# YoungSeng/QPGesture

Hardware: AMD Instinct MI355X
Metric: matched gesture frames/sec (GestureKNN) (higher is better)
Workload: dtype split-f16 products / f64 block sums + f64 re-evaluation; 1 GPU; 1 x 24 s clip (M=6 windows, Q=48 steps, 1440 frames each) per job vs speaker-10-class DB N_db=2048 windows (53248 candidates), shipped mode wavlm_feat(f32-bounded/f64-exact)+text(f32)+phase; n_db=2048, windows_per_clip=6, clips=1, clips_per_gpu=1, feature_dtype=f32, audio_precision=mixed, encode_batch=0, clips_in_flight=1, parallelism=single GPU, unsharded DB

## Files before the change

include/qpg.h:

```cpp
#ifndef QPG_H
#define QPG_H

#include <stddef.h>
#include <stdint.h>

#ifdef __cplusplus
extern "C" {
#endif

#define QPG_OK 0
#define QPG_EINVAL (-1)
#define QPG_EHIP (-2)
#define QPG_EUNSUP (-3)

typedef struct qpg_ctx qpg_ctx;

int qpg_version(void);
const char* qpg_build_id(void);
int qpg_ctx_create(int device, qpg_ctx** out);
int qpg_dev_kernarg(void);
int qpg_ctx_destroy(qpg_ctx* ctx);
#define QPG_OPT_GATE_DEDUP_FROM_CHAINS 0
#define QPG_OPT_TAKES_STAGES 1
#define QPG_OPT_COUNT 4
int qpg_ctx_set_option(qpg_ctx* ctx, int option, int value);
int qpg_ctx_get_option(qpg_ctx* ctx, int option, int* value);
int qpg_last_error(char* buf, size_t n);
int qpg_signal_i32(qpg_ctx*, void* stream, int32_t* dst, int32_t value);
int qpg_doorbell_wait(qpg_ctx*, void* stream, int32_t* counter, const int32_t* go, int32_t timeout_ms);


int qpg_wavlm_resample_f32(qpg_ctx*, void* stream, const float* x, int64_t N, int Tin, int F, int Tout, float* out);

int qpg_frame_norm2_f64(qpg_ctx*, void* stream, const float* x, int64_t rows, int F, double* out);

int qpg_audio_cand_norm2(qpg_ctx*, void* stream, const double* fn2, int N, int T, const int32_t* cand_t,
                         int G, int n_taps, int tap_stride, double* cn2);

int qpg_l2_normalize_rows_f32(qpg_ctx*, void* stream, const float* x, int64_t rows, int D, float* out);
int qpg_text_pack_queries_f32(qpg_ctx*, void* stream, const float* x, int M, int R, int D, const int32_t* q_win,
                              const int32_t* q_row, int Q, float* out);


int qpg_audio_pack_queries(qpg_ctx*, void* stream, const float* qbase, int M, int T, int F,
                           const int32_t* q_win, const int32_t* q_t, int Q, int n_taps, int tap_stride,
                           float* q32, double* qn2);

int qpg_audio_cosine_f64(qpg_ctx*, void* stream, const float* base, int N, int T, int F,
                         const int32_t* cand_t, int G, int n_taps, int tap_stride, const double* cn2,
                         const float* q32, const double* qn2, int Q, double* D, int64_t ldD);
int qpg_audio_cosine_f64_h(qpg_ctx*, void* stream, const void* base_f16, int N, int T, int F,
                           const int32_t* cand_t, int G, int n_taps, int tap_stride, const double* cn2,
                           const float* q32, const double* qn2, int Q, double* D, int64_t ldD);

#define QPG_AUDIO_MX_ERR 2.05e-6
int qpg_audio_cosine_mx(qpg_ctx*, void* stream, const float* base, int N, int T, int F, const int32_t* cand_t, int G,
                        int n_taps, int tap_stride, const double* cn2, const float* q32, const double* qn2, int Q,
                        void* D, int d_is_f32, int64_t ldD, int32_t* stats);

int qpg_audio_cosine_mx_h(qpg_ctx*, void* stream, const void* base_f16, int N, int T, int F, const int32_t* cand_t, int G,
                          int n_taps, int tap_stride, const double* cn2, const float* q32, const double* qn2, int Q,
                          void* D, int d_is_f32, int64_t ldD, int32_t* stats);

#define QPG_AUDIO_HL_ERR 1.3e-6
int qpg_audio_hl_supported(int T, int F, int G, int n_taps, int tap_stride, int cand_step);
int qpg_audio_pack_queries_hl(qpg_ctx*, void* stream, const float* qbase, int M, int T, int F, const int32_t* q_win,
                              const int32_t* q_t, int Q, int n_taps, int tap_stride, float* q32, double* qn2, void* image,
                              int64_t image_bytes);
int64_t qpg_audio_hl_db_bytes(int N, int F);
int64_t qpg_audio_hl_query_bytes(int Q, int F);
int qpg_audio_hl_pack_db(qpg_ctx*, void* stream, const float* base, int N, int T, int F, int G, int n_taps, int tap_stride,
                         int cand_step, void* image, int64_t image_bytes);
int qpg_audio_hl_pack_queries(qpg_ctx*, void* stream, const float* q32, int Q, int F, void* image, int64_t image_bytes);
int qpg_clip_pack_hl(qpg_ctx*, void* stream, const float* qbase, int M, int T, int F, const int32_t* q_win,
                     const int32_t* q_t, int Q, int n_taps, int tap_stride, float* q32, double* qn2, void* image,
                     int64_t image_bytes, const float* text_ctx, int Mt, int R, int Dt, const int32_t* tq_win,
                     const int32_t* tq_row, int Qt, float* qn_out, void* cols_image, int64_t cols_bytes);
int qpg_audio_cosine_hl(qpg_ctx*, void* stream, const void* db_image, int N, int F, int G, const double* cn2,
                        const void* q_image, const double* qn2, int Q, void* D, int d_is_f32, int64_t ldD, int32_t* stats);
int qpg_audio_hl1_supported(int T, int F, int G, int n_taps, int tap_stride, int cand_step);
int64_t qpg_audio_hl1_db_bytes(int N, int F);
int qpg_audio_hl1_pack_db(qpg_ctx*, void* stream, const void* base_f16, int N, int T, int F, int G, int n_taps,
                          int tap_stride, int cand_step, void* image, int64_t image_bytes);
int qpg_audio_cosine_hl1(qpg_ctx*, void* stream, const void* db_image, int N, int F, int G, const double* cn2,
                         const void* q_image, const double* qn2, int Q, void* D, int d_is_f32, int64_t ldD, int32_t* stats);
int qpg_probe_mfma_f16_tile(qpg_ctx*, void* stream, const void* a, const void* b, const float* c, int tiles, float* out);

int qpg_text_pack_candidates_f32(qpg_ctx*, void* stream, const float* x, int N, int R, int Dm,
                                 const int32_t* cand_r, int G, float* xt);

int qpg_text_cosine_f32(qpg_ctx*, void* stream, const float* xt, int64_t C, int Dm, const float* qn, int Q,
                        float* D, int64_t ldD);

int64_t qpg_text_percode_ws_bytes(int64_t C, int Q, int K, int tiles_per_chunk);
int qpg_text_percode_f32(qpg_ctx*, void* stream, const float* xt, int64_t C, int Dm, const int16_t* cand_code, int K,
                         const float* qn, int Q, int tiles_per_chunk, int32_t idx_base, float absent, void* ws,
                         int64_t ws_bytes, float* out_dist, int32_t* out_idx, int16_t* out_rank, int32_t* out_nn);
int qpg_text_pack_candidates_f16(qpg_ctx*, void* stream, const float* x, int N, int R, int Dm, const int32_t* cand_r,
                                 int G, void* xh, float* nrm);
int qpg_text_percode_f16(qpg_ctx*, void* stream, const void* xh, const float* nrm, int64_t C, int Dm,
                         const int16_t* cand_code, int K, const float* qn, int Q, int32_t idx_base, float absent,
                         void* ws, int64_t ws_bytes, float* out_dist, int32_t* out_idx, int16_t* out_rank,
                         int32_t* out_nn);

int64_t qpg_hl_rows_bytes(int64_t R, int D);
int64_t qpg_hl_cols_bytes(int Q, int D);
int qpg_hl_pack_rows(qpg_ctx*, void* stream, const float* xs, int64_t R, int D, void* image, int64_t image_bytes);
int qpg_hl_pack_cols(qpg_ctx*, void* stream, const float* qn, int Q, int D, void* image, int64_t image_bytes);
int qpg_hl_prepare_queries(qpg_ctx*, void* stream, const float* q, int Q, int D, float* qn_out, void* cols_image,
                           int64_t image_bytes, float* qperm_out);
int qpg_hl_gemm_distance(qpg_ctx*, void* stream, const void* rows_image, int64_t R, int D, const void* cols_image, int Q,
                         float* Dm, int64_t ldD, float* tile_min, int64_t ldT);
int qpg_hl_gemm_tilemin(qpg_ctx*, void* stream, const void* rows_image, int64_t R, int D, const void* cols_image, int Q,
                        float band, float* tile_min, uint16_t* tile_mask, int64_t ldT);
int qpg_hl_gemm_tilemin_h(qpg_ctx*, void* stream, const void* rows_image, int64_t R, int D, const void* cols_image, int Q,
                          float band, float* tile_min_t, uint16_t* tile_mask_t, int64_t ldQ);
int qpg_perm32_rows_f32(qpg_ctx*, void* stream, const float* x, int64_t R, int D, float* y);
int qpg_percode_select_bycode_f32(qpg_ctx*, void* stream, const float* tile_min_t, const uint16_t* tile_mask_t, int64_t ldQ,
                                  int Q, int64_t R, const int16_t* row_code, const int32_t* row_index,
                                  const int32_t* zero_row, const int32_t* code_tile, int K, float band,
                                  const float* qn_perm, const float* xs_perm, int D, float absent, float* out_dist,
                                  int32_t* out_idx, int16_t* out_rank, int32_t* out_nn, int32_t* stats, int32_t idx_base);
int qpg_percode_select_sorted_f32(qpg_ctx*, void* stream, const float* Dm, int64_t ldD, const float* tile_min,
                                  const uint16_t* tile_mask , int64_t ldT,
                                  int Q, int64_t R, const int16_t* row_code, const int32_t* row_index,
                                  const int32_t* zero_row, const int32_t* code_tile, int K, float band, const float* qn,
                                  const float* xs, int D, float absent, float* out_dist, int32_t* out_idx,
                                  int16_t* out_rank, int32_t* out_nn, int32_t* stats, int32_t idx_base, int q_block,
                                  int64_t block_stride);

int qpg_wavvq_lev_f32(qpg_ctx*, void* stream, const int32_t* sym_db, int N, int T, const int32_t* cand_t, int G,
                      const int32_t* tap_off, int n_taps, const int32_t* sym_q, int Mq, int Tq,
                      const int32_t* q_win, const int32_t* q_t, int Q, float* D, int64_t ldD);

int qpg_percode_select_f64(qpg_ctx*, void* stream, const double* D, int64_t ldD, int Q, const int16_t* cand_code,
                           int64_t C, int K, double absent, int32_t idx_base, double* out_dist, int32_t* out_idx,
                           int16_t* out_rank, int q_block, int64_t block_stride);
int qpg_percode_select_f32(qpg_ctx*, void* stream, const float* D, int64_t ldD, int Q, const int16_t* cand_code,
                           int64_t C, int K, float absent, int32_t idx_base, float* out_dist, int32_t* out_idx,
                           int16_t* out_rank, int q_block, int64_t block_stride);

int qpg_percode_select_guarded_f64(qpg_ctx*, void* stream, const double* D, int64_t ldD, int Q, const int16_t* cand_code,
                                   int64_t C, int K, double absent, int32_t idx_base, double* out_dist, int32_t* out_idx,
                                   int16_t* out_rank, int q_block, int64_t block_stride, const float* base, int T, int F,
                                   const int32_t* cand_t, int G, int n_taps, int tap_stride, const float* q32, double eps,
                                   int32_t* stats, int base_is_f16);

int64_t qpg_percode_select_exact_ws_bytes(int Q, int64_t C, int K);
int qpg_percode_select_exact_f64(qpg_ctx*, void* stream, const double* D, int64_t ldD, int Q, const int16_t* cand_code,
                                 int64_t C, int K, double absent, int32_t idx_base, double* out_dist, int32_t* out_idx,
                                 int16_t* out_rank, int q_block, int64_t block_stride, const float* base, int T, int F,
                                 const int32_t* cand_t, int G, int n_taps, int tap_stride, const float* q32, double eps,
                                 int32_t* stats, int base_is_f16, void* ws, int64_t ws_bytes);

int qpg_percode_select_mixed_f64(qpg_ctx*, void* stream, const void* D, int d_is_f32, int64_t ldD, int Q, const int16_t* cand_code,
                                 int64_t C, int K, double absent, int32_t idx_base, double* out_dist, int32_t* out_idx,
                                 int16_t* out_rank, int q_block, int64_t block_stride, const float* base, int T, int F,
                                 const int32_t* cand_t, int G, int n_taps, int tap_stride, const float* q32,
                                 const double* qn2, const double* cn2, double eps1, double eps2, int32_t* stats,
                                 void* ws, int64_t ws_bytes, int base_is_f16);
int64_t qpg_percode_select_mixed_ws_bytes(int Q, int K);
int64_t qpg_percode_select_mixed_ws_stride(int K);
int qpg_percode_select_mixed_f64_cut(qpg_ctx*, void* stream, const void* D, int d_is_f32, int64_t ldD, int Q,
                                     const int16_t* cand_code, int64_t C, int K, double absent, int32_t idx_base,
                                     double* out_dist, int32_t* out_idx, int16_t* out_rank, int q_block, int64_t block_stride,
                                     const float* base, int T, int F, const int32_t* cand_t, int G, int n_taps,
                                     int tap_stride, const float* q32, const double* qn2, const double* cn2, double eps1,
                                     double eps2, int32_t* stats, void* ws, int64_t ws_bytes, int base_is_f16,
                                     const int16_t* pos_rank_t, const int16_t* freq_rank, int top_n, int probe);

int64_t qpg_merge_mixed_ws_bytes(int Q, int K, int fl_cap);
int qpg_merge_mixed_phase1_f64(qpg_ctx*, void* stream, const void* recv, int W, int64_t src_stride, int64_t dist_off,
                               int64_t idx_off, int Q, int K, double absent, double eps1, int R, void* req,
                               int64_t req_stride, void* ws, int64_t ws_bytes, int32_t* stats, int fl_cap,
                               int64_t flag_off);
int qpg_shard_refine_f64(qpg_ctx*, void* stream, const void* req_recv, int W, int64_t req_stride, int R, int q_stride,
                         int64_t cand_base, const float* base, int base_is_f16, int T, int F, const int32_t* cand_t, int G,
                         int n_taps, int tap_stride, const float* q32, const double* qn2, const double* cn2, void* resp,
                         int64_t resp_stride, int reference_arithmetic, int32_t* stats, int Rq);
int qpg_flags_stamp(qpg_ctx*, void* stream, void* buf, int nblk, int64_t stride, int64_t off, const int32_t* stats);
int qpg_flags_gather(qpg_ctx*, void* stream, const void* buf, int nblk, int64_t stride, int64_t off, int32_t* stats);
int qpg_merge_mixed_phase2_f64(qpg_ctx*, void* stream, const void* recv, int W, int64_t src_stride, int64_t idx_off, int Q,
                               int K, double absent, const void* ws, int64_t ws_bytes, const void* resp_recv,
                               int64_t resp_stride, double* out_dist, int32_t* out_idx, int16_t* out_rank, int32_t* stats,
                               int fl_cap, double eps2);

int qpg_merge_select_f64(qpg_ctx*, void* stream, const void* recv, int W, int64_t src_stride, int64_t dist_off,
                         int64_t idx_off, int Q, int K, double absent, double* out_dist, int32_t* out_idx,
                         int16_t* out_rank, double eps2, int32_t* stats);
int qpg_merge_select_f32(qpg_ctx*, void* stream, const void* recv, int W, int64_t src_stride, int64_t dist_off,
                         int64_t idx_off, int Q, int K, float absent, float* out_dist, int32_t* out_idx,
                         int16_t* out_rank);

int qpg_rank_rows_f64(qpg_ctx*, void* stream, const double* d, int Q, int K, int16_t* out);
int qpg_rank_rows_f32(qpg_ctx*, void* stream, const float* d, int Q, int K, int16_t* out);


int qpg_l2_table_f32(qpg_ctx*, void* stream, const float* sig, int K, int Dm, float* out);

#define QPG_MODE_AUD_TXT 0
#define QPG_MODE_AUD 1
#define QPG_MODE_TXT 2
#define QPG_MODE_SERIAL_WALK 0x100
#define QPG_MODE_PREFUSED 0x200

int qpg_match_steps(qpg_ctx*, void* stream, const int16_t* aud_rank, const int32_t* aud_idx,
                    const int16_t* txt_rank, const int32_t* txt_idx, const int16_t* pos_rank,
                    const int16_t* freq_rank, const int32_t* code, int code_ld, const int32_t* aud_cidx,
                    const int32_t* aud_pslot, int Ga, const int32_t* txt_cidx, const int32_t* txt_pslot, int Gt,
                    const float* phase, int Tp, int mode, int M, int steps, int K, int seed_code,
                    const float* seed_phase, int32_t* gate_tables, int32_t* out_codes, float* out_phase,
                    int32_t* out_vote, int32_t* out_status, const int32_t* guard_flags);
int qpg_match_steps_batch(qpg_ctx*, void* stream, const int16_t* aud_rank, const int32_t* aud_idx, const int16_t* txt_rank,
                          const int32_t* txt_idx, const int16_t* pos_rank, const int16_t* freq_rank, const int32_t* code,
                          int code_ld, const int32_t* aud_cidx, const int32_t* aud_pslot, int Ga, const int32_t* txt_cidx,
                          const int32_t* txt_pslot, int Gt, const float* phase, int Tp, int mode, int M, int steps, int K,
                          int n_chains, const int32_t* seed_codes, const float* seed_phase, int32_t* gate_tables,
                          int32_t* out_codes, float* out_phase, int32_t* out_vote, int32_t* out_status,
                          int64_t status_stride, const int32_t* guard_flags);
#define QPG_TAKES_MAX 65536
size_t qpg_match_steps_takes_ws_bytes(int n_takes, int M, int steps);
int qpg_match_steps_takes(qpg_ctx*, void* stream, const int16_t* aud_rank, const int32_t* aud_idx, const int16_t* txt_rank,
// ... 187 lines not shown
```

qpgesture_amd/code_knn.py:

```python
import ctypes
from collections import namedtuple
from typing import NamedTuple, Optional

import numpy as np
import torch

from . import _lib
from .parallel import allreduce_max_, allreduce_min_index, exchange_bytes, shard_rows
from .sorted_rows import SortedRows

from .constant import (ABSENT_DIST, NUM_AUDIO_FEAT_FRAMES, STEP_SZ, WAVVQ_GROUP_SIZE, codebook_size, num_frames,
                       num_frames_code)

MODE_AUD_TXT, MODE_AUD, MODE_TXT = _lib.QPG_MODE_AUD_TXT, _lib.QPG_MODE_AUD, _lib.QPG_MODE_TXT
AUDIO_MX_ERR = _lib.QPG_AUDIO_MX_ERR
AUDIO_MX_BAND = 2.1 * AUDIO_MX_ERR
AUDIO_HL_ERR = _lib.QPG_AUDIO_HL_ERR
AUDIO_HL_BAND = 2.1 * AUDIO_HL_ERR

FLAG_LIST_OVERFLOW, FLAG_SMALL_NORMS, FLAG_REQUEST_OVERFLOW, FLAG_CROSS_SHARD_TIE = 1, 2, 4, 8
FLAG_TEXT_OVERFLOW = 16


_PIN_SENTINEL = -1234567
# ... 207 lines not shown
            pd = torch.empty((self.K, self.K), dtype=torch.float32, device=dev)
            _lib.call("qpg_l2_table_f32", dev, sig, self.K, sig.shape[1], pd)
            self.pos_dist = pd
            self.pos_rank = torch.empty((self.K, self.K), dtype=torch.int16, device=dev)
            _lib.call("qpg_rank_rows_f32", dev, pd, self.K, self.K, self.pos_rank)
        else:
            self.pos_rank = torch.as_tensor(np.asarray(pos_rank, np.int16), device=dev).contiguous()

        cnt = np.bincount(code.reshape(-1), minlength=self.K)[:self.K]
        self.freq_dist = np.where(cnt > 0, 1 - cnt / cnt.sum(), 1.0)
        self.pos_rank_t = self.pos_rank.t().contiguous()
        if freq_rank is None:
            fd = torch.from_numpy(self.freq_dist[None].copy()).to(dev)
            self.freq_rank = torch.empty((1, self.K), dtype=torch.int16, device=dev)
            _lib.call("qpg_rank_rows_f64", dev, fd, 1, self.K, self.freq_rank)
            self.freq_rank = self.freq_rank[0].contiguous()
        else:
            self.freq_rank = torch.as_tensor(np.asarray(freq_rank, np.int16), device=dev).contiguous()

    def save(self, path, key="", sources=None):
        from . import db_cache
        return db_cache.save(self, path, key, sources=sources)

    @classmethod
    def load(cls, path, device="cuda:0", key=None):
        from . import db_cache
        dev = torch.device(device)
        if dev.type != "cuda":
            raise RuntimeError("GestureDB needs a HIP device (got %s); there is no CPU path" % dev)
        _lib.load()
        db = db_cache.load(path, dev, key)
        if db is None:
            return None
        if db.hl_image is not None or db.txt_sorted is not None:
            from .selfcheck import mfma_bound_ok
            db.hl_bound_ok, db.hl_bound_report = mfma_bound_ok(dev)
            if not db.hl_bound_ok:
                db.hl_image = db.txt_sorted = None
        return db

    @staticmethod
    def _cand_code(code_local, cidx, dev):
        cc = np.ascontiguousarray(code_local[:, np.asarray(cidx, np.int64)].reshape(-1))
        cc = np.where((cc >= 0) & (cc < 32767), cc, -1).astype(np.int16)
        return torch.from_numpy(cc if cc.size else np.zeros((1,), np.int16)).to(dev)

    @property
    def idx_base(self):
        return self.lo


Knobs = namedtuple("Knobs", "audio_precision audio_kernel text_kernel tie_eps mixed_single_launch sharded_mixed "
                   "sharded_mixed_min_gflop force_sharded overlap_sweeps text_after_sweep audio_first fused_pack rank_cut "
                   "split_fuse split_fuse_max_steps host_ranks use_wavvq",
                   defaults=("mixed", "hl", "mfma", 1e-12, False, True, 20.0, False, True, True, None, True, True, True,
                             256, False, False))
DBFacts = namedtuple("DBFacts", "n_local N world K Ga F Dt feature_dtype hl_bound_ok has_hl_image has_txt_sorted hl_planes",
                     defaults=("f32", True, True, True, 2))


class AudioPlan(NamedTuple):
    path: str
    kernel: str
    band: float
    cut_top_n: int
    fused_rank: bool


class StepPlan(NamedTuple):
    audio: Optional[AudioPlan]
    text: Optional[str]
    sharded: bool
    exchange: Optional[str]
    clip_pack: bool
    split_fuse: bool
    overlap: bool
    order: Optional[str]


def plan_audio(kn, db, Q, want_rank=False, reduce=True, out_given=False, cut_top_n=0):
    C = db.n_local * db.Ga
    fused_rank = want_rank and db.world == 1
    local_final = fused_rank and reduce and not out_given
    shard_part = (db.world > 1 or kn.force_sharded) and not reduce and out_given
    gflop = 2e-9 * Q * (-(-db.N // db.world) * db.Ga) * NUM_AUDIO_FEAT_FRAMES * db.F
    guard = kn.tie_eps > 0 and C > 0
    half = db.feature_dtype == "f16"
    if (kn.audio_precision == "mixed" and guard and db.K <= 512 and db.hl_bound_ok and
            (local_final or (shard_part and kn.sharded_mixed and gflop >= kn.sharded_mixed_min_gflop))):
        hl = kn.audio_kernel == "hl" and db.has_hl_image
        kernel = ("hl" if db.hl_planes == 2 else "hl1") if hl else ("mx_h" if half else "mx")
        cut = cut_top_n if (cut_top_n in (1, 2) and local_final and not kn.mixed_single_launch) else 0
        return AudioPlan("mixed", kernel, AUDIO_HL_BAND if hl else AUDIO_MX_BAND, cut, fused_rank)
    path = "exact" if (kn.audio_precision == "exact" and guard) else ("guarded" if guard else "plain")
    return AudioPlan(path, "f64_h" if half else "f64", 0.0, 0, fused_rank)


def plan_text(kn, db, Q, reduce=True, out_given=False):
    mfma = (kn.text_kernel == "mfma" and db.has_txt_sorted and Q > 0 and kn.audio_precision != "exact" and
            ((not out_given and reduce and db.world == 1) or (out_given and not reduce)))
    return "mfma" if mfma else "valu"


def plan_step(kn, db, M, steps, mode=MODE_AUD_TXT, for_walk=False, owner_blocks=False):
    Q = M * steps
    sharded = db.world > 1 or kn.force_sharded
    audio = text = None
    if mode != MODE_TXT and not kn.use_wavvq:
        cut = 0
        if for_walk and kn.rank_cut and not sharded and not kn.host_ranks:
            cut = 1 if mode == MODE_AUD_TXT else 2
        audio = plan_audio(kn, db, Q, want_rank=not sharded, reduce=not sharded, out_given=sharded, cut_top_n=cut)
    if mode != MODE_AUD:
        text = plan_text(kn, db, Q, reduce=not sharded, out_given=sharded)
    split = (for_walk and mode == MODE_AUD_TXT and not sharded and not kn.host_ranks and kn.split_fuse and
             db.K % 16 == 0 and db.K <= 4096 and Q <= kn.split_fuse_max_steps)
    overlap = mode == MODE_AUD_TXT and kn.overlap_sweeps
    mfma_text = kn.text_kernel == "mfma" and db.has_txt_sorted and kn.audio_precision != "exact"
    clip_pack = (overlap and not kn.use_wavvq and mfma_text and audio.kernel in ("hl", "hl1") and db.Dt % 128 == 0 and
                 kn.fused_pack)
    audio_first = mfma_text if kn.audio_first is None else bool(kn.audio_first)
    after = overlap and kn.text_after_sweep and not audio_first and not kn.use_wavvq
    order = None
    if overlap:
        order = "audio_first" if audio_first else ("text_after_sweep" if after else "text_first")
    exchange = ("all_to_all" if owner_blocks else "all_gather") if sharded else None
    return StepPlan(audio, text, sharded, exchange, clip_pack, split, overlap, order)


class TakesPlan(NamedTuple):
    path: str
    reason: str


def plan_takes(kn, db, M, steps, n_takes, serial_walk=False):
    if db.world > 1 or kn.force_sharded:
        return TakesPlan("unsupported", "takes of a row-sharded database are not implemented (the merged tables would serve; "
                                        "nothing tests them)")
    if serial_walk:
        return TakesPlan("per_take", "the one-wave sequential walk was asked for (serial_walk)")
    K = db.K
    last_idx = min(steps * 4, num_frames_code) - 1
    if (last_idx // 4 != steps - 1 or M * steps > 2048 or 2 * steps * 2 * K * 2 > 64 * 1024 or (steps * 2 * K) % 8 or
            2 * K > 65536):
        return TakesPlan("per_take", "the tabulated walk does not take this geometry (steps = %d, K = %d, %d steps per clip)"
                         % (steps, K, M * steps))
    if not 1 <= n_takes <= _lib.QPG_TAKES_MAX:
        return TakesPlan("per_take", "n_takes outside [1, %d]" % _lib.QPG_TAKES_MAX)
    return TakesPlan("kernel", "")


AudioResult = namedtuple("AudioResult", "dist idx rank D q32 qn2 plan")


def _grown(buf, nbytes, dev, zero=False):
    if buf is not None and buf.numel() >= nbytes:
        return buf
    return (torch.zeros if zero else torch.empty)((nbytes,), dtype=torch.uint8, device=dev)


class CodeKNN:

    def __init__(self, db, use_wavlm=True, use_wavvq=False, use_phase=True, use_txt=True, rng=None):
        if use_wavlm == use_wavvq:
            raise ValueError("exactly one of use_wavlm / use_wavvq (GestureKNN.py:431-438)")
        if use_wavvq and not db.has_wavvq:
            raise ValueError("GestureDB was built without a wavvq track")
        self.db = db
        self.use_wavvq = use_wavvq
        if use_wavvq:
            self.step_sz, self.n_db_frm = db.vq_step, db.Tv
        else:
            self.step_sz, self.n_db_frm = db.step_sz, db.T
        self.n_db_seq = db.N
        self.use_phase, self.use_txt = use_phase, use_txt
        self.rng = rng if rng is not None else np.random
        self.overlap_sweeps = True
        self.text_after_sweep = True
        self.audio_first = None
        self.serial_walk = False
        self.tie_eps = 1e-12
        self._guard_stats = torch.zeros((4,), dtype=torch.int32, device=db.device)
        self.audio_precision = "mixed"
        self.audio_kernel = "hl"
        self.text_kernel = "mfma"
        self._txt_scratch = {}
        self.fallbacks = 0
        import os as _os
        self.fused_pack = _os.environ.get("QPG_FUSED_PACK", "1") != "0"
        self.rank_cut = _os.environ.get("QPG_RANK_CUT", "1") != "0"
        self.rank_cut_probe = 64
        self.mixed_single_launch = False
        self.split_fuse = True
        self.split_fuse_max_steps = 256
        self.sharded_mixed = True
        self.force_sharded = False
        self.sharded_mixed_min_gflop = 20.0
        self.mixed_requests = None
        self.host_ranks = False

        self._qpos, self._qcache, self._layouts, self._mm_cache, self._pinned_ints, self._plans = None, {}, {}, {}, {}, {}
        self._side_stream = self._side_gate = self._side_done = self._sweep_event = None
        self._mix_ws = self._exact_ws = self._hl_qimage = self._takes_ws = None
        self.kernel_events, self.kernel_events_every, self.kernel_event_pool, self._ev_calls = None, 1, None, 0
        self.text_fallbacks, self.tables, self._last_mix_Q = 0, None, 0
        self._last_audio_mixed = self._last_audio_exact = self._last_audio_hl = False
        self._last_text_mfma = self._last_rank_cut = False
        self._last_D_aud = self._last_q32 = self._last_qn2 = self._last_ints = self._last_gate_tables = None

    def _knobs(self):
        return Knobs(self.audio_precision, self.audio_kernel, self.text_kernel, self.tie_eps, self.mixed_single_launch,
                     self.sharded_mixed, self.sharded_mixed_min_gflop, self.force_sharded, self.overlap_sweeps,
                     self.text_after_sweep, self.audio_first, self.fused_pack, self.rank_cut, self.split_fuse,
                     self.split_fuse_max_steps, self.host_ranks, self.use_wavvq)

    def _facts(self):
        db = self.db
        return DBFacts(db.n_local, db.N, db.world, db.K, db.Ga, db.F, db.Dt, db.feature_dtype, db.hl_bound_ok,
                       db.hl_image is not None, db.txt_sorted is not None, db.hl_planes)

    def _audio_grid(self):
        db = self.db
        if self.use_wavvq:
            return db.vq_cidx, db.vq_pslot, db.Gv
        return db.aud_cidx, db.aud_pslot, db.Ga

    def query_positions(self):
        key = (self.n_db_frm, self.step_sz)
        if self._qpos is not None and self._qpos[0] == key:
            return self._qpos[1]
        pos, i = [], 0
        while i < self.n_db_frm:
            pos.append(i)
            i += STEP_SZ * self.step_sz
        self._qpos = (key, pos)
        return pos

    def init_code_phase(self):
        db = self.db
        i = self.rng.randint(0, self.n_db_seq)
        j = self.rng.randint(0, self.n_db_frm - int(num_frames / num_frames_code))
        code = int(db.code_host[i, j // num_frames_code])
        P = db.phase_host[i, j:j + 8]
        if P.shape[0] != 8:
            raise ValueError("init_code_phase drew frame %d: phase slice has %d rows, not 8 "
                             "(the reference fails on this draw too); use another seed" % (j, P.shape[0]))
        return code, np.concatenate((P[:, 0], P[:, 1]), axis=1).astype(np.float32)

    def _tables_out(self, Q, dtype, out, with_rank):
        K, dev = self.db.K, self.db.device
        dist, idx, qb, bs = out if out is not None else (torch.empty((Q, K), dtype=dtype, device=dev),
                                                         torch.empty((Q, K), dtype=torch.int32, device=dev), 0, 0)
        return dist, idx, (torch.empty((Q, K), dtype=torch.int16, device=dev) if with_rank else None), qb, bs

    def _select_plain(self, D, cand_code, C, G, out, with_rank):
        db, Q = self.db, D.shape[0]
        dist, idx, rank, qb, bs = self._tables_out(Q, D.dtype, out, with_rank)
        _lib.call("qpg_percode_select_f64" if D.dtype == torch.float64 else "qpg_percode_select_f32", db.device, D,
                  D.stride(0), Q, cand_code, C, db.K, float(ABSENT_DIST), db.idx_base * G, dist, idx, rank, qb, bs)
        return dist, idx, rank

    def _finish(self, dist, idx, rank, want_rank, reduce):
        if not reduce:
            return dist, idx
        dist, idx = self._reduce_min(dist, idx)
        if want_rank:
            return dist, idx, (rank if rank is not None else self.rank_rows(dist))
        return dist, idx

    def _sweep_timer(self):
        if self.kernel_events is None:
            return None
        if self.kernel_events_every > 1:
            self._ev_calls += 1
            if self._ev_calls % self.kernel_events_every:
                return None
        return (self.kernel_event_pool.pop() if self.kernel_event_pool else
                (torch.cuda.Event(enable_timing=True), torch.cuda.Event(enable_timing=True)))

    def sweep_audio(self, qbase, q_win, q_t, tap_stride=None, want_rank=False, reduce=True, out=None, prepacked=None,
                    cut_top_n=None):
        Q = int(q_win.shape[0]) if isinstance(q_win, torch.Tensor) else len(q_win)
        plan = plan_audio(self._knobs(), self._facts(), Q, want_rank, reduce, out is not None, cut_top_n or 0)
        r = self._sweep_audio(plan, qbase, q_win, q_t, tap_stride, out, prepacked)
        return self._finish(r.dist, r.idx, r.rank, want_rank, reduce)

    def _sweep_audio(self, plan, qbase, q_win, q_t, tap_stride=None, out=None, prepacked=None, sweep_event=None,
                     after_sweep=None):
        db, dev = self.db, self.db.device
        Q = int(q_win.shape[0]) if isinstance(q_win, torch.Tensor) else len(q_win)
        qbase = qbase.contiguous()
        M, T, F = qbase.shape
        ts = db.tap_stride if tap_stride is None else tap_stride
        if prepacked is not None:
            q32, qn2 = prepacked[0], prepacked[1]
        else:
            q32 = torch.empty((Q, NUM_AUDIO_FEAT_FRAMES * F), dtype=torch.float32, device=dev)
            qn2 = torch.empty((Q,), dtype=torch.float64, device=dev)
        C = db.n_local * db.Ga
        mixed, use_hl, half = plan.path == "mixed", plan.kernel in ("hl", "hl1"), db.feature_dtype == "f16"
        D = torch.empty((Q, max(C, 1)), dtype=torch.float32 if mixed else torch.float64, device=dev)
        timer = self._sweep_timer()
        sweep_fn = "qpg_audio_cosine_" + plan.kernel
        if use_hl:
            qi = self._hl_qimage = _grown(self._hl_qimage, int(_lib.load().qpg_audio_hl_query_bytes(Q, db.F)), dev)
            sweep_launch = _lib.prepare(sweep_fn, dev, db.hl_image, db.n_local, db.F, db.Ga, db.cn2, qi,
                                        qn2, Q, D, 1, D.stride(0), self._guard_stats)
            if prepacked is None:
                _lib.call("qpg_audio_pack_queries_hl", dev, qbase, M, T, F, _i32(q_win, dev), _i32(q_t, dev), Q,
                          NUM_AUDIO_FEAT_FRAMES, ts, q32, qn2, qi, qi.numel())
        else:
            assert prepacked is None, "the one-launch clip pack feeds the split-f16 sweep only"
            _lib.call("qpg_audio_pack_queries", dev, qbase, M, T, F, _i32(q_win, dev), _i32(q_t, dev), Q,
                      NUM_AUDIO_FEAT_FRAMES, ts, q32, qn2)
        if timer is not None:
            timer[0].record(torch.cuda.current_stream(dev))
        if use_hl:
            sweep_launch()
        else:
            strides = (1, D.stride(0), self._guard_stats) if mixed else (D.stride(0),)
            _lib.call(sweep_fn, dev, db.base, db.n_local, db.T, db.F, db.aud_t, db.Ga, NUM_AUDIO_FEAT_FRAMES,
                      db.tap_stride, db.cn2, q32, qn2, Q, D, *strides)
        if timer is not None:
            timer[1].record(torch.cuda.current_stream(dev))
            self.kernel_events.append(timer)
        if after_sweep is not None:
            after_sweep()
        if sweep_event is not None:
            sweep_event.record(torch.cuda.current_stream(dev))
        if plan.path == "plain":
            dist, idx, rank = self._select_plain(D, db.aud_cand_code, C, db.Ga, out, plan.fused_rank)
        else:
            dist, idx, rank, qb, bs = self._tables_out(Q, torch.float64, out, plan.fused_rank)
            tables = (Q, db.aud_cand_code, C, db.K, float(ABSENT_DIST), db.idx_base * db.Ga, dist, idx, rank, qb, bs)
            track = (db.base, db.T, db.F, db.aud_t, db.Ga, NUM_AUDIO_FEAT_FRAMES, db.tap_stride, q32)
        if mixed:
            ws = self._mix_ws = _grown(self._mix_ws, int(_lib.load().qpg_percode_select_mixed_ws_bytes(Q, db.K)), dev,
                                       zero=True)
            single = self.mixed_single_launch
            sel_args = (D, 1, D.stride(0), *tables, *track, qn2, db.cn2, plan.band, float(self.tie_eps),
                        self._guard_stats, None if single else ws, 0 if single else ws.numel(), int(half))
            try:
                if plan.cut_top_n:
                    _lib.call("qpg_percode_select_mixed_f64_cut", dev, *sel_args, db.pos_rank_t, db.freq_rank,
                              int(plan.cut_top_n), int(self.rank_cut_probe))
                else:
                    _lib.call("qpg_percode_select_mixed_f64", dev, *sel_args)
            except Exception:
                self._mix_ws = None
                raise
        elif plan.path == "exact":
            ws = self._exact_ws = _grown(self._exact_ws, int(_lib.load().qpg_percode_select_exact_ws_bytes(Q, C, db.K)),
                                         dev)
            _lib.call("qpg_percode_select_exact_f64", dev, D, D.stride(0), *tables, *track, float(self.tie_eps),
                      self._guard_stats, int(half), ws, ws.numel())
        elif plan.path == "guarded":
            _lib.call("qpg_percode_select_guarded_f64", dev, D, D.stride(0), *tables, *track, float(self.tie_eps),
                      self._guard_stats, int(half))
        self._last_audio_mixed, self._last_audio_exact, self._last_audio_hl = mixed, plan.path == "exact", use_hl
        self._last_rank_cut, self._last_D_aud, self._last_q32, self._last_qn2 = plan.cut_top_n > 0, D, q32, qn2
        if mixed:
            self._last_mix_Q = Q
        return AudioResult(dist, idx, rank, D, q32, qn2, plan)

    def sweep_text(self, queries, want_rank=False, reduce=True, normalised=False, out=None, cols_packed=False, kind=None):
        db, dev = self.db, self.db.device
        Q = queries.shape[0]
        if normalised:
            qn = queries
        else:
            qn = torch.empty_like(queries)
            _lib.call("qpg_l2_normalize_rows_f32", dev, queries, Q, db.Dt, qn)
        if kind is None:
            kind = plan_text(self._knobs(), self._facts(), Q, reduce, out is not None)
        self._last_text_mfma = kind == "mfma"
        if kind == "mfma":
            dist, idx, rank, qb, bs = self._tables_out(Q, torch.float32, out, want_rank and out is None)
            db.txt_sorted.select(qn, float(ABSENT_DIST), self._guard_stats, dist=dist, idx=idx, rank=rank,
                                 idx_base=db.idx_base * db.Gt, q_block=qb, block_stride=bs, scratch=self._txt_scratch,
                                 cols_packed=cols_packed)
        else:
            D = torch.empty((Q, max(db.Ct, 1)), dtype=torch.float32, device=dev)
            _lib.call("qpg_text_cosine_f32", dev, db.ctxt, db.Ct, db.Dt, qn, Q, D, D.stride(0))
            dist, idx, rank = self._select_plain(D, db.txt_cand_code, db.Ct, db.Gt, out, want_rank and db.world == 1)
        return self._finish(dist, idx, rank, want_rank, reduce)

    def sweep_audio_wavvq(self, test_wavvq, q_win, q_t, want_rank=False, reduce=True, out=None):
        db, dev = self.db, self.db.device
        tw = torch.as_tensor(test_wavvq).to(dev)
        sym_q = (tw[..., 0].to(torch.int64) * WAVVQ_GROUP_SIZE + tw[..., 1].to(torch.int64)).to(torch.int32).contiguous()
        Q = int(q_win.shape[0]) if isinstance(q_win, torch.Tensor) else len(q_win)
        C = db.n_local * db.Gv
        D = torch.empty((Q, max(C, 1)), dtype=torch.float32, device=dev)
        taps = (ctypes.c_int32 * len(db.vq_taps))(*db.vq_taps)
        _lib.call("qpg_wavvq_lev_f32", dev, db.vq_sym, db.n_local, db.Tv, db.vq_t, db.Gv, taps, len(db.vq_taps),
                  sym_q, sym_q.shape[0], sym_q.shape[1], _i32(q_win, dev), _i32(q_t, dev), Q, D, D.stride(0))
        dist, idx, rank = self._select_plain(D, db.vq_cand_code, C, db.Gv, out, want_rank and db.world == 1)
        self._last_D_aud = D
        return self._finish(dist, idx, rank, want_rank, reduce)

    def _reduce_min(self, dist, idx):
        if self.db.world == 1:
            return dist, idx
        return allreduce_min_index(dist, idx)

    def guard_stats(self):
        v = self._guard_stats.cpu().numpy()
        return int(v[0]), bool(v[1])

    def mixed_stats(self):
        v = self._guard_stats.cpu().numpy()
        return {"tier1_pairs": int(v[2]), "tier2_pairs": int(v[0]), "flags": int(v[1])}

    def tier1_list_lengths(self):
        ws, Q = self._mix_ws, self._last_mix_Q
        if ws is None or not Q:
            return np.zeros((0,), np.int64)
        K = self.db.K
        stride = int(_lib.load().qpg_percode_select_mixed_ws_stride(K))
        w = ws[:Q * stride].view(Q, stride)[:, 24 * K:24 * K + 4].contiguous().view(torch.int32)
        return w.cpu().numpy().reshape(-1).astype(np.int64)

    def clear_flags(self):
        self._guard_stats[1:2].zero_()

    @staticmethod
    def numpy_ranks(dist, idx=None, integer=False):
        d = dist.detach().cpu().numpy()
        present = None if idx is None else (idx.detach().cpu().numpy() >= 0)
        out = np.empty(d.shape, np.int16)
        for r_, row in enumerate(d):
            full = present is not None and bool(present[r_].all())
            if full and integer:
# ... 67 lines not shown
        dev = self.db.device
        if self._side_stream is None:
            self._side_stream = torch.cuda.Stream(dev)
            self._side_gate, self._side_done = torch.cuda.Event(), torch.cuda.Event()
            self._sweep_event = torch.cuda.Event()
        if dev.index is None or dev.index == torch.cuda.current_device():
            self._side_gate.record()
        else:
            self._side_gate.record(torch.cuda.current_stream(dev))
        self._side_stream.wait_event(self._side_gate)
        return self._side_stream

    def _clip_pack(self, test_interp, test_context, q_win, q_t, q_row, Q):
        db, dev = self.db, self.db.device
        q32 = torch.empty((Q, NUM_AUDIO_FEAT_FRAMES * db.F), dtype=torch.float32, device=dev)
        qn2 = torch.empty((Q,), dtype=torch.float64, device=dev)
        qi = self._hl_qimage = _grown(self._hl_qimage, int(_lib.load().qpg_audio_hl_query_bytes(Q, db.F)), dev)
        qn = torch.empty((Q, db.Dt), dtype=torch.float32, device=dev)
        cols = db.txt_sorted.cols_buffer(Q, self._txt_scratch)
        tc, ti = test_context.contiguous(), test_interp.contiguous()
        _lib.call("qpg_clip_pack_hl", dev, ti, ti.shape[0], db.T, db.F, q_win, q_t, Q, NUM_AUDIO_FEAT_FRAMES,
                  db.tap_stride, q32, qn2, qi, qi.numel(), tc, tc.shape[0], tc.shape[1], db.Dt, q_win, q_row, Q, qn, cols,
                  cols.numel())
        return q32, qn2, qn

    def sweep_tables(self, test_interp, test_context, n_windows, mode=MODE_AUD_TXT, owner_blocks=False, for_walk=False,
                     after_sweep=None):
        db, dev = self.db, self.db.device
        M, steps = n_windows, self.n_steps()
        if test_interp.shape[0] < M or (mode != MODE_AUD and test_context.shape[0] < M):
            raise IndexError("n_windows=%d but the test arrays hold %d audio / %d context windows"
                             % (M, test_interp.shape[0], test_context.shape[0]))
        want = (db.Tv, 2) if self.use_wavvq else (db.T, db.F)
        if tuple(test_interp.shape[1:]) != want:
            raise ValueError("test audio windows have shape %s, database expects %s"
                             % (tuple(test_interp.shape[1:]), want))
        q_win, q_t, q_row = self._query_index(M)
        Q = M * steps
        key = (self._knobs(), self._facts(), M, steps, mode, for_walk, owner_blocks)
        plan = self._plans.get(key)
        if plan is None:
            plan = self._plans[key] = plan_step(*key)
        sharded = plan.sharded
        T = dict(aud_d=None, aud_idx=None, aud_rank=None, txt_d=None, txt_idx=None, txt_rank=None)
        gtab = torch.empty((3, max(M, 1) * steps, db.K), dtype=torch.int32, device=dev) if plan.split_fuse else None
        lay = self._layout(Q, owner_blocks, mode) if sharded else None
        side = self._fork_side() if plan.overlap else None
        packed = None
        if plan.clip_pack:
            packed = self._clip_pack(test_interp, test_context, q_win, q_t, q_row, Q)
            self._side_gate.record(torch.cuda.current_stream(dev))
            side.wait_event(self._side_gate)

        def keep(p_, g, r):
            T[p_ + "_d"], T[p_ + "_idx"], T[p_ + "_rank"] = r[0], r[1], (None if sharded else r[2])
            if gtab is not None:
                _lib.call("qpg_fuse_best_ranked", dev, r[2], r[1], db.pos_rank, db.freq_rank, Q, db.K, gtab[g])

        def text_pack():
            tc = test_context.contiguous()
            qn = torch.empty((Q, db.Dt), dtype=torch.float32, device=dev)
            _lib.call("qpg_text_pack_queries_f32", dev, tc, tc.shape[0], tc.shape[1], db.Dt, q_win, q_row, Q, qn)
            return qn

        def text_side(qn=None):
            if packed is not None:
                qn = packed[2]
            elif qn is None:
                qn = text_pack()
            keep("txt", 1, self.sweep_text(qn, want_rank=not sharded, reduce=not sharded, normalised=True,
                                           out=lay.views("txt") if sharded else None, cols_packed=packed is not None,
                                           kind=plan.text))

        if plan.order == "text_first":
            with torch.cuda.stream(side):
                text_side()
        aud = None
        if mode != MODE_TXT:
            out = lay.views("aud") if sharded else None
            if self.use_wavvq:
                r = self.sweep_audio_wavvq(test_interp, q_win, q_t, want_rank=not sharded, reduce=not sharded, out=out)
            else:
                aud = self._sweep_audio(plan.audio, test_interp, q_win, q_t, out=out, prepacked=packed,
                                        sweep_event=self._sweep_event if plan.order == "text_after_sweep" else None,
                                        after_sweep=after_sweep)
                r = self._finish(aud.dist, aud.idx, aud.rank, not sharded, not sharded)
            keep("aud", 0, r)
        if plan.order == "text_after_sweep":
            with torch.cuda.stream(side):
                qn_early = None if packed is not None else text_pack()
                side.wait_event(self._sweep_event)
                text_side(qn_early)
        elif plan.order == "audio_first":
            with torch.cuda.stream(side):
                text_side()
        if plan.overlap:
            self._side_done.record(side)
            torch.cuda.current_stream(dev).wait_event(self._side_done)
        elif mode != MODE_AUD:
            text_side()
        if sharded:
            self._merge_shards(lay, owner_blocks, T, aud)
        if self.host_ranks:
            for p_ in ("aud", "txt"):
                if T[p_ + "_d"] is not None:
                    T[p_ + "_rank"] = self.numpy_ranks(T[p_ + "_d"], T[p_ + "_idx"],
                                                       integer=(p_ == "aud" and self.use_wavvq))
        if gtab is not None:
            T["gate_tables"] = gtab
        return T

    def _layout(self, Q, owner_blocks, mode):
        parts = tuple(p_ for p_, off in (("aud", MODE_TXT), ("txt", MODE_AUD)) if mode != off)
        key = (Q, self.db.world if owner_blocks else 1, parts, not self.use_wavvq)
        if key not in self._layouts:
            self._layouts[key] = ExchangeLayout(key[0], self.db.K, key[1], parts, key[3], self.db.device)
        return self._layouts[key]

    def _merge_shards(self, lay, owner_blocks, T, aud):
        db, dev = self.db, self.db.device
        _lib.call("qpg_flags_stamp", dev, lay.send, lay.nblk, lay.block_bytes, lay.off["flags"], self._guard_stats)
        recv = exchange_bytes(lay.send, db.world, owner_blocks)
        src_stride = lay.block_bytes if owner_blocks else lay.send.numel()
        gathered = False
        for p_ in lay.parts:
            d = torch.empty((lay.Qb, db.K), dtype=lay.dtype[p_], device=dev)
            ix = torch.empty((lay.Qb, db.K), dtype=torch.int32, device=dev)
            rk = torch.empty((lay.Qb, db.K), dtype=torch.int16, device=dev)
            wavlm_aud = p_ == "aud" and aud is not None
            if wavlm_aud and aud.plan.path in ("mixed", "exact"):
                self._merge_mixed(recv, src_stride, lay, owner_blocks, d, ix, rk, aud.q32, aud.qn2, aud.plan)
                gathered = True
            elif lay.dtype[p_] == torch.float64:
                guard = wavlm_aud and self.tie_eps > 0
                _lib.call("qpg_merge_select_f64", dev, recv, db.world, src_stride, lay.off[p_ + "_d"],
                          lay.off[p_ + "_i"], lay.Qb, db.K, float(ABSENT_DIST), d, ix, rk,
                          float(self.tie_eps) if guard else 0.0, self._guard_stats if guard else None)
            else:
# ... 237 lines not shown
```

qpgesture_amd/csrc/qpg_common.h:

```cpp
#pragma once
#include <hip/hip_runtime.h>
#include <stdint.h>
#include <stdio.h>
#include <string.h>

#include "../../include/qpg.h"

struct qpg_ctx {
  int device;
  int n_cu;
  float* zeros;
  bool select_lds_raised;
  int opt[QPG_OPT_COUNT];
};

#ifdef QPG_DEBUG_HOOKS
#define QPG_HOOK_VAR(type, name, value) static type name = value
#else
#define QPG_HOOK_VAR(type, name, value) static constexpr type name = value
#endif

void qpg_set_error(const char* fmt, ...);

#define QPG_REQUIRE(cond, ...)      \
  do {                              \
    if (!(cond)) {                  \
      qpg_set_error(__VA_ARGS__);   \
      return QPG_EINVAL;            \
    }                               \
  } while (0)

#define QPG_LAUNCH_CHECK(name)                                                \
  do {                                                                        \
    hipError_t e_ = hipGetLastError();                                        \
    if (e_ != hipSuccess) {                                                   \
      qpg_set_error("%s: launch failed: %s", name, hipGetErrorString(e_));    \
      return QPG_EHIP;                                                        \
    }                                                                         \
  } while (0)

static inline hipStream_t qpg_stream(void* s) { return reinterpret_cast<hipStream_t>(s); }

typedef double f64x4 __attribute__((ext_vector_type(4)));
typedef float f32x4 __attribute__((ext_vector_type(4)));
typedef float f32x16 __attribute__((ext_vector_type(16)));

#pragma clang fp contract(off)
__device__ __forceinline__ float f_mul(float a, float b) { return a * b; }
__device__ __forceinline__ float f_add(float a, float b) { return a + b; }
__device__ __forceinline__ float f_sub(float a, float b) { return a - b; }
__device__ __forceinline__ float f_div(float a, float b) { return a / b; }
__device__ __forceinline__ float f_sqrt(float a) { return __builtin_sqrtf(a); }
__device__ __forceinline__ double f_mul(double a, double b) { return a * b; }
__device__ __forceinline__ double f_add(double a, double b) { return a + b; }
__device__ __forceinline__ double f_sub(double a, double b) { return a - b; }
__device__ __forceinline__ double f_div(double a, double b) { return a / b; }

__device__ __forceinline__ double cosine_from_dot(double dot, double qn2, double cn2) {
  const double tiny = 10.0 * 2.220446049250313e-16;
  double nq = sqrt(qn2), nc = sqrt(cn2);
  bool zq = nq < tiny, zc = nc < tiny;
  if (zq || zc) {
    double a = zq ? qn2 : 1.0, b = zc ? cn2 : 1.0;
    double cross = dot / ((zq ? 1.0 : nq) * (zc ? 1.0 : nc));
    return 0.5 * (a + b - 2.0 * cross);
// ... 146 lines not shown
```

qpgesture_amd/csrc/qpg_core.hip:

```cpp
#include <stdarg.h>

#include "qpg_common.h"
#include <stdlib.h>

static thread_local char g_err[512] = "";

void qpg_set_error(const char* fmt, ...) {
  va_list ap;
  va_start(ap, fmt);
  vsnprintf(g_err, sizeof(g_err), fmt, ap);
  va_end(ap);
}

extern "C" int qpg_version(void) { return 109; }

#ifndef QPG_BUILD_ID
#define QPG_BUILD_ID "unstamped"
#endif
static const char g_build_id[] = "QPG_BUILD_ID=" QPG_BUILD_ID;
extern "C" const char* qpg_build_id(void) { return g_build_id + 13; }

extern "C" int qpg_dev_kernarg(void) {
  const char* e = getenv("HIP_FORCE_DEV_KERNARG");
  return (e && e[0] == '1') ? 1 : 0;
}

extern "C" int qpg_last_error(char* buf, size_t n) {
  if (!buf || n == 0) return QPG_EINVAL;
  strncpy(buf, g_err, n - 1);
  buf[n - 1] = 0;
  return QPG_OK;
}

extern "C" int qpg_ctx_create(int device, qpg_ctx** out) {
  QPG_REQUIRE(out != nullptr, "qpg_ctx_create: out is null");
  int n = 0;
  if (hipGetDeviceCount(&n) != hipSuccess || device < 0 || device >= n) {
    qpg_set_error("qpg_ctx_create: no HIP device %d (count %d)", device, n);
    return QPG_EHIP;
  }
  hipDeviceProp_t p;
  if (hipGetDeviceProperties(&p, device) != hipSuccess) {
    qpg_set_error("qpg_ctx_create: hipGetDeviceProperties failed");
    return QPG_EHIP;
  }
  qpg_ctx* c = new qpg_ctx;
  c->device = device;
  c->n_cu = p.multiProcessorCount;
  c->zeros = nullptr;
  c->select_lds_raised = false;
  for (int i = 0; i < QPG_OPT_COUNT; ++i) c->opt[i] = 0;
  c->opt[QPG_OPT_GATE_DEDUP_FROM_CHAINS] = 1;
  c->opt[QPG_OPT_TAKES_STAGES] = 7;
  int prev = 0;
  (void)hipGetDevice(&prev);
  const bool ok = hipSetDevice(device) == hipSuccess && hipMalloc(reinterpret_cast<void**>(&c->zeros), 4096) == hipSuccess &&
                  hipMemset(c->zeros, 0, 4096) == hipSuccess;
  (void)hipSetDevice(prev);
  if (!ok) {
    qpg_set_error("qpg_ctx_create: could not allocate the context's zero page on device %d", device);
    delete c;
    return QPG_EHIP;
  }
  *out = c;
  return QPG_OK;
}

extern "C" int qpg_ctx_set_option(qpg_ctx* ctx, int option, int value) {
  QPG_REQUIRE(ctx != nullptr, "qpg_ctx_set_option: null context");
  QPG_REQUIRE(option >= 0 && option < QPG_OPT_COUNT, "qpg_ctx_set_option: unknown option %d", option);
  if (option == QPG_OPT_GATE_DEDUP_FROM_CHAINS) QPG_REQUIRE(value >= 0, "qpg_ctx_set_option: gate_dedup_from_chains >= 0");
  ctx->opt[option] = value;
  return QPG_OK;
}

extern "C" int qpg_ctx_get_option(qpg_ctx* ctx, int option, int* value) {
  QPG_REQUIRE(ctx != nullptr && value != nullptr, "qpg_ctx_get_option: null pointer");
  QPG_REQUIRE(option >= 0 && option < QPG_OPT_COUNT, "qpg_ctx_get_option: unknown option %d", option);
  *value = ctx->opt[option];
  return QPG_OK;
}

extern "C" int qpg_ctx_destroy(qpg_ctx* ctx) {
  if (ctx && ctx->zeros) (void)hipFree(ctx->zeros);
  delete ctx;
  return QPG_OK;
}

__global__ void signal_i32_kernel(int32_t* dst, int32_t value) {
  __hip_atomic_store(dst, value, __ATOMIC_RELEASE, __HIP_MEMORY_SCOPE_SYSTEM);
}

extern "C" int qpg_signal_i32(qpg_ctx* ctx, void* stream, int32_t* dst, int32_t value) {
  QPG_REQUIRE(ctx && dst && (reinterpret_cast<uintptr_t>(dst) % 4) == 0, "qpg_signal_i32: null or misaligned destination");
  hipLaunchKernelGGL(signal_i32_kernel, dim3(1), dim3(1), 0, qpg_stream(stream), dst, value);
  QPG_LAUNCH_CHECK("signal_i32_kernel");
  return QPG_OK;
}

__global__ void doorbell_wait_kernel(int32_t* __restrict__ counter, const int32_t* __restrict__ go, int32_t timeout_ms) {
  const int32_t seq = atomicAdd(counter, 1) + 1;
  const long long t0 = wall_clock64();
  const long long limit = (long long)timeout_ms * 100000ll;
  while (__hip_atomic_load(go, __ATOMIC_RELAXED, __HIP_MEMORY_SCOPE_SYSTEM) - seq < 0) {
    if (wall_clock64() - t0 > limit) break;
    __builtin_amdgcn_s_sleep(16);
// ... 167 lines not shown
```

qpgesture_amd/csrc/qpg_select.hip:

```cpp
#include "qpg_common.h"

__device__ __forceinline__ unsigned long long order_key(double d) {
  unsigned long long b = (unsigned long long)__double_as_longlong(d);
  return (b >> 63) ? ~b : (b | 0x8000000000000000ull);
}
__device__ __forceinline__ double key_value(unsigned long long k, double) {
  unsigned long long b = (k >> 63) ? (k & 0x7fffffffffffffffull) : ~k;
  return __longlong_as_double((long long)b);
}
__device__ __forceinline__ unsigned int order_key(float d) {
  unsigned int b = __float_as_uint(d);
  return (b >> 31) ? ~b : (b | 0x80000000u);
}
__device__ __forceinline__ float key_value(unsigned int k, float) {
  unsigned int b = (k >> 31) ? (k & 0x7fffffffu) : ~k;
  return __uint_as_float(b);
}

template <typename T, typename KeyT, bool PACKED>
__global__ __launch_bounds__(1024) void percode_select_kernel(const T* __restrict__ D, int64_t ldD,
                                                              const int16_t* __restrict__ cand_code, int64_t C, int K,
                                                              T absent, int32_t idx_base, T* __restrict__ out_dist,
                                                              int32_t* __restrict__ out_idx,
                                                              int16_t* __restrict__ out_rank, int q_block,
                                                              int64_t block_stride) {
  extern __shared__ __attribute__((aligned(16))) unsigned char smem[];
  unsigned long long* best = reinterpret_cast<unsigned long long*>(smem);
  unsigned int* besti = reinterpret_cast<unsigned int*>(smem + 8 * (size_t)K);
  T* v = reinterpret_cast<T*>(smem + 12 * (size_t)rank_sort_pow2(K));
  constexpr int VEC = 16 / sizeof(T);
  typedef T vecT __attribute__((ext_vector_type(VEC)));
  typedef int16_t vecC __attribute__((ext_vector_type(VEC)));
  const int q = blockIdx.x;
  if (q_block > 0) {
    const int64_t shift = (int64_t)(q / q_block) * block_stride;
    const int64_t rowoff = (int64_t)(q % q_block) * K - (int64_t)q * K;
    out_dist = reinterpret_cast<T*>(reinterpret_cast<unsigned char*>(out_dist) + shift) + rowoff;
    out_idx = reinterpret_cast<int32_t*>(reinterpret_cast<unsigned char*>(out_idx) + shift) + rowoff;
  }
  const T* row = D + (int64_t)q * ldD;
  for (int k = threadIdx.x; k < K; k += blockDim.x) {
    best[k] = ~0ull;
    besti[k] = 0xffffffffu;
  }
  __syncthreads();
  const bool vec_ok = (ldD % VEC) == 0 && (reinterpret_cast<uintptr_t>(D) % 16) == 0 &&
                      (reinterpret_cast<uintptr_t>(cand_code) % (2 * VEC)) == 0;
  const int64_t Cv = vec_ok ? (C / VEC) * VEC : 0;
  for (int64_t c = (int64_t)threadIdx.x * VEC; c < Cv; c += (int64_t)blockDim.x * VEC) {
    const vecT d = *reinterpret_cast<const vecT*>(row + c);
    const vecC cd = *reinterpret_cast<const vecC*>(cand_code + c);
#pragma unroll
    for (int e = 0; e < VEC; ++e) {
// ... 50 lines not shown
                     [&](int k, int r) { out_rank[(int64_t)q * K + k] = (int16_t)r; });
}

template <typename T, typename F>
__device__ __forceinline__ void block_stable_ranks(const T* v, int K, int* cnt, F&& emit) {
  const int tid = threadIdx.x;
  if (K <= 512 && K >= 64 && (int)blockDim.x >= 256) {
    __shared__ unsigned long long rank_skey[512];
    __shared__ int rank_scode[512];
    block_sorted_ranks(v, K, rank_skey, rank_scode, emit);
    return;
  }
  const int P = (int)blockDim.x >= 2 * K ? (int)blockDim.x / K : 1;
  if (P == 1) {
    for (int k = tid; k < K; k += blockDim.x) {
      const T x = v[k];
      int r = 0;
#pragma unroll 8
      for (int o = 0; o < K; ++o) {
        const T y = v[o];
        r += (y < x) || (y == x && o < k);
      }
      emit(k, r);
    }
    return;
  }
  for (int k = tid; k < K; k += blockDim.x) cnt[k] = 0;
  __syncthreads();
  if (tid < P * K) {
    const int k = tid % K, part = tid / K;
    const int o0 = (int)((int64_t)part * K / P), o1 = (int)((int64_t)(part + 1) * K / P);
    const T x = v[k];
    int r = 0;
#pragma unroll 8
    for (int o = o0; o < o1; ++o) {
      const T y = v[o];
      r += (y < x) || (y == x && o < k);
    }
    atomicAdd(&cnt[k], r);
  }
  __syncthreads();
  for (int k = tid; k < K; k += blockDim.x) emit(k, cnt[k]);
}

struct GuardArgs {
  const float* base;
  int half;
  const float* q32;
  const int32_t* cand_t;
  int T, F, G, n_taps, tap_stride;
  double eps;
  int32_t* stats;
};
struct RankCut {
  const int16_t* pos_t;
  const int16_t* freq;
  int top_n;
  int probe;
};
#define GUARD_LIST 256
typedef _Float16 g16x4 __attribute__((ext_vector_type(4)));
__device__ __forceinline__ float guard_val(const GuardArgs& A, int64_t off) {
  return A.half ? (float)reinterpret_cast<const _Float16*>(A.base)[off] : A.base[off];
}
__device__ __forceinline__ f32x4 guard_val4(const GuardArgs& A, int64_t off) {
  if (A.half) {
    const g16x4 h = *reinterpret_cast<const g16x4*>(reinterpret_cast<const _Float16*>(A.base) + off);
    return (f32x4){(float)h[0], (float)h[1], (float)h[2], (float)h[3]};
  }
  return *reinterpret_cast<const f32x4*>(A.base + off);
}

__device__ __forceinline__ double refine_pair_f64(const GuardArgs& A, int q, int64_t c_local, int sub) {
  const int D = A.n_taps * A.F;
  const int j = (int)(c_local / A.G), g = (int)(c_local - (int64_t)j * A.G);
  const int t0 = A.cand_t[g];
  const float* qrow = A.q32 + (int64_t)q * D;
  const int64_t crow = (int64_t)j * A.T * A.F;
  auto cval = [&](int e) -> double {
    const int tap = e / A.F, f = e - tap * A.F;
    const int t = t0 + tap * A.tap_stride;
    return t < A.T ? (double)guard_val(A, crow + (int64_t)t * A.F + f) : 0.0;
  };
  const int l = sub & 1;
  const bool is_c = sub >= 2;
  auto chain = [&](auto val) -> double {
    double acc = 0.0;
    const int nfull = D / 8;
    for (int gq = 0; gq < nfull; ++gq) {
#pragma unroll
      for (int u = 3; u >= 0; --u) {
        const double v = val(8 * gq + 2 * u + l);
        acc = f_add(f_mul(v, v), acc);
      }
    }
    for (int i = nfull * 8; i < D; i += 2) {
      const double v = (i + l < D) ? val(i + l) : 0.0;
      acc = f_add(f_mul(v, v), acc);
    }
    return acc;
  };
  const double a1 = is_c ? chain(cval) : chain([&](int e) -> double { return (double)qrow[e]; });
  const double o1 = __shfl_xor(a1, 1, 64);
  double n = sqrt(l == 0 ? f_add(a1, o1) : f_add(o1, a1));
  if (n < 10.0 * 2.220446049250313e-16) n = 1.0;
  const double n_other = __shfl_xor(n, 2, 64);
// ... 393 lines not shown
#pragma unroll
    for (int u = 0; u < UN; ++u)
#pragma unroll
      for (int e = 0; e < 4; ++e) {
        const int code = cd[u][e];
        if ((unsigned)code >= (unsigned)K) continue;
        unsigned int o = old[u][e];
        if (key[u][e] < o) o = atomicMin(&best32[code], key[u][e]);
        const unsigned int lo = o < key[u][e] ? o : key[u][e];
        if ((double)d[u][e] <= (double)key_value(lo, 0.f) + eps1) {
          const int pp = atomicAdd(&n_pot, 1);
          if (pp < MIX_SPOT) {
            pc[pp] = (int)(b + (int64_t)u * blockDim.x * 4 + e);
            pd[pp] = d[u][e];
            pk[pp] = (int16_t)code;
          }
        }
      }
  }
  for (int64_t c = cv + tid; c < c1; c += blockDim.x) visit(c, row[c], cand_code[c]);
  __syncthreads();
  SEL_STAMP(1);
  MixStream m = mix_stream_of(ws, q, K);
  if (MIX_INV_ATOMIC) {
    for (int k = tid; k < K; k += blockDim.x)
      if (best32[k] != 0xffffffffu) atomicMax(&m.inv[k], ~best32[k]);
  } else {
    for (int k = tid; k < K; k += blockDim.x) m.inv[(size_t)sl * K + k] = ~best32[k];
  }
  SEL_STAMP(2);
  const int np = n_pot;
  if (np > MIX_SPOT) {
    if (tid == 0) m.cnt[sl] = -1;
    return;
  }
  const int seg = sl * MIX_SPOT;
  for (int e = tid; e < np; e += blockDim.x) {
    if (!((double)pd[e] <= (double)key_value(best32[pk[e]], 0.f) + eps1)) continue;
    const int pos = seg + atomicAdd(&n_keep, 1);
    m.pot_c[pos] = pc[e];
    m.pot_d[pos] = pd[e];
    m.pot_k[pos] = pk[e];
  }
  __syncthreads();
  if (tid == 0) m.cnt[sl] = n_keep;
  SEL_STAMP(3);
}

template <typename DT>
__global__ __launch_bounds__(1024) void percode_select_mixed_f64_kernel(
    const DT* __restrict__ D, int64_t ldD, const int16_t* __restrict__ cand_code, int64_t C, int K, double absent,
    int32_t idx_base, double* __restrict__ out_dist, int32_t* __restrict__ out_idx, int16_t* __restrict__ out_rank,
    int q_block, int64_t block_stride, GuardArgs A, double eps1, const double* __restrict__ cn2,
    const double* __restrict__ qn2, int use_qlds, int phase, unsigned char* __restrict__ ws, int pre, RankCut RC) {
  extern __shared__ __attribute__((aligned(16))) unsigned char smem[];
  unsigned long long* best = reinterpret_cast<unsigned long long*>(smem);
  double* v = reinterpret_cast<double*>(smem + 8 * (size_t)K);
  unsigned int* besti = reinterpret_cast<unsigned int*>(smem + 16 * (size_t)K);
  unsigned int* near_ = besti + K;
  int* s_code = reinterpret_cast<int*>(near_ + K);
  unsigned char* refd = reinterpret_cast<unsigned char*>(s_code + K);
  unsigned char* tail = smem + 32 * (size_t)K;
  double* l_d = reinterpret_cast<double*>(tail);
  int* l_c = reinterpret_cast<int*>(tail + 8 * MIX_LIST);
  int* l_k = l_c + MIX_LIST;
  int* l2 = l_k + MIX_LIST;
  int* ctl = l2 + MIX_LIST2;
  int* p_c = ctl + 8;
  int16_t* p_k = reinterpret_cast<int16_t*>(p_c + MIX_LIST);
  int* rk = reinterpret_cast<int*>(p_k + MIX_LIST);
  int* pot_c = rk + K;
  int16_t* pot_k = reinterpret_cast<int16_t*>(pot_c + MIX_POT);
  float* qlds = reinterpret_cast<float*>(pot_k + MIX_POT);
  const int q = blockIdx.x, tid = threadIdx.x, lane = tid & 63, wv = tid >> 6, nwv = blockDim.x >> 6;
  const DT* row = D + (int64_t)q * ldD;
  if (q_block > 0) {
    const int64_t shift = (int64_t)(q / q_block) * block_stride;
    const int64_t rowoff = (int64_t)(q % q_block) * K - (int64_t)q * K;
    out_dist = reinterpret_cast<double*>(reinterpret_cast<unsigned char*>(out_dist) + shift) + rowoff;
    out_idx = reinterpret_cast<int32_t*>(reinterpret_cast<unsigned char*>(out_idx) + shift) + rowoff;
  }
  unsigned char* wq = ws ? mix_query_base(ws, q, K) : nullptr;
  for (int k = tid; k < K; k += blockDim.x) {
    best[k] = ~0ull;
    besti[k] = 0xffffffffu;
    near_[k] = 0;
    refd[k] = 0;
  }
  if (tid < 8) ctl[tid] = 0;
  __syncthreads();
  SEL_STAMP(0);
  unsigned long long* skey = reinterpret_cast<unsigned long long*>(p_c);
  int* scode = reinterpret_cast<int*>(skey + 512);
  auto rank_pass = [&](bool store) {
    block_sorted_ranks(v, K, skey, scode, [&](int k, int r) {
      if (store && out_rank) out_rank[(int64_t)q * K + k] = (int16_t)r;
      s_code[r] = k;
    });
  };
  int n = 0;
  bool order_parked = false;
  if (phase != 2) {
  constexpr int VE = 16 / (int)sizeof(DT);
  typedef DT vecD __attribute__((ext_vector_type(VE)));
  typedef int16_t vecC __attribute__((ext_vector_type(VE)));
  const bool vec_ok = (ldD % VE) == 0 && (reinterpret_cast<uintptr_t>(D) % 16) == 0 &&
                      (reinterpret_cast<uintptr_t>(cand_code) % (2 * VE)) == 0;
  const int64_t Cv = vec_ok ? (C / VE) * VE : 0;
  constexpr bool K32 = sizeof(DT) == 4;
  unsigned int* best32 = reinterpret_cast<unsigned int*>(s_code);
  const bool streamed = K32 && pre;
  MixStream ms = {};
  if (streamed) ms = mix_stream_of(ws, q, K);
  if (K32 && !streamed) {
    for (int k = tid; k < K; k += blockDim.x) best32[k] = 0xffffffffu;
    __syncthreads();
  }
  auto pass1 = [&](int64_t c, DT dv, int cd) {
    if ((unsigned)cd >= (unsigned)K) return;
    const double d = (double)dv;
    double lo;
    if constexpr (K32) {
      const unsigned int key = order_key((float)dv);
      unsigned int old = *reinterpret_cast<volatile unsigned int*>(&best32[cd]);
      if (key < old) old = atomicMin(&best32[cd], key);
      lo = (double)key_value(old < key ? old : key, 0.f);
    } else {
      const unsigned long long key = (unsigned long long)order_key(d);
      unsigned long long old = *reinterpret_cast<volatile unsigned long long*>(&best[cd]);
      if (key < old) old = atomicMin(&best[cd], key);
      lo = key_value(old < key ? old : key, 0.0);
    }
    if (d <= lo + eps1) {
      const int pp = atomicAdd(&ctl[4], 1);
      if (pp < MIX_POT) {
        pot_c[pp] = (int)c;
        pot_k[pp] = (int16_t)cd;
      }
    }
  };
  if (!streamed) {
#pragma unroll 4
    for (int64_t c = (int64_t)tid * VE; c < Cv; c += (int64_t)blockDim.x * VE) {
      const vecD d = *reinterpret_cast<const vecD*>(row + c);
      const vecC cd = *reinterpret_cast<const vecC*>(cand_code + c);
#pragma unroll
      for (int e = 0; e < VE; ++e) pass1(c + e, d[e], cd[e]);
    }
    for (int64_t c = Cv + tid; c < C; c += blockDim.x) pass1(c, row[c], cand_code[c]);
    __syncthreads();
  }
  int g_pot = 0;
// ... 404 lines not shown
        __syncthreads();
        if (tid == 0) atomicAdd(&A.stats[0], n2);
      }
    }
    for (int e = tid; e < n; e += blockDim.x)
      if ((unsigned long long)order_key(l_d[e]) == best[l_k[e]])
        atomicMin(&besti[l_k[e]], (unsigned int)(l_c[e] + idx_base));
    __syncthreads();
    for (int k = tid; k < K; k += blockDim.x)
      if (near_[k] >= 2) {
        if (best[k] != ~0ull) v[k] = key_value(best[k], 0.0);
        else besti[k] = (unsigned int)rk[k];
      }
    if (tid == 0) atomicAdd(&A.stats[2], n);
    __syncthreads();
  }
  for (int k = tid; k < K; k += blockDim.x) {
    const bool have = besti[k] != 0xffffffffu;
    out_dist[(int64_t)q * K + k] = v[k];
    out_idx[(int64_t)q * K + k] = have ? (int32_t)besti[k] : -1;
  }
  SEL_STAMP(8);
  if (!out_rank) return;
  if (tid == 0) ctl[2] = 0;
  __syncthreads();
  bool repaired = false;
  if (phase == 2 && RC.pos_t && reinterpret_cast<const int*>(wq + 24 * (size_t)K)[1] == 1) {
    const int16_t* w_order = reinterpret_cast<const int16_t*>(wq + mix_park_order_off(K));
    for (int r = tid; r < K; r += blockDim.x) s_code[r] = w_order[r];
    __syncthreads();
    for (int round = 0; round < 24 && !repaired; ++round) {
      if (tid == 0) ctl[5] = 0;
      __syncthreads();
#pragma unroll
      for (int parity = 0; parity < 2; ++parity) {
        for (int r = 2 * tid + parity; r + 1 < K; r += 2 * blockDim.x) {
          const int ka = s_code[r], kb = s_code[r + 1];
          if (rank_gt(rank_sort_key(v[ka]), ka, rank_sort_key(v[kb]), kb)) {
            s_code[r] = kb;
            s_code[r + 1] = ka;
            ctl[5] = 1;
          }
        }
        __syncthreads();
      }
      repaired = ctl[5] == 0;
      __syncthreads();
    }
    if (repaired)
      for (int r = tid; r < K; r += blockDim.x) out_rank[(int64_t)q * K + s_code[r]] = (int16_t)r;
  }
  if (!repaired) rank_pass(true);
  SEL_STAMP(9);
  if (A.eps <= 0.0) return;
  __syncthreads();
  for (int r = tid; r + 1 < K; r += blockDim.x) {
    const int ka = s_code[r], kb = s_code[r + 1];
    if (besti[ka] == 0xffffffffu || besti[kb] == 0xffffffffu) continue;
    if (phase == 2 && RC.pos_t &&
        !(reinterpret_cast<const unsigned char*>(pot_c)[ka] && reinterpret_cast<const unsigned char*>(pot_c)[kb]))
      continue;
    if (v[kb] - v[ka] < A.eps) {
#pragma unroll
      for (int h = 0; h < 2; ++h) {
        const int k = h ? kb : ka;
        if (atomicExch(&near_[k], 0xffffffffu) == 0xffffffffu || refd[k]) continue;
        const int pos = atomicAdd(&ctl[2], 1);
        if (pos < MIX_LIST2) {
          l2[pos] = k;
        }
      }
    }
  }
  __syncthreads();
  int n3 = ctl[2];
  SEL_STAMP(10);
  if (n3 == 0) return;
  if (n3 > MIX_LIST2) {
    n3 = MIX_LIST2;
    if (tid == 0) atomicOr(&A.stats[1], 1);
  }
  for (int i0 = 0; i0 < n3; i0 += blockDim.x / 4) {
    const int i = i0 + (tid >> 2);
    const int k = l2[i < n3 ? i : 0];
    const double dr = refine_pair_f64(A, q, (int64_t)(besti[k] - (unsigned int)idx_base), tid & 3);
    if (i < n3 && (tid & 3) == 0) {
      v[k] = dr;
      out_dist[(int64_t)q * K + k] = dr;
    }
  }
  if (tid == 0) atomicAdd(&A.stats[0], n3);
  __syncthreads();
  SEL_STAMP(11);
  rank_pass(true);
  SEL_STAMP(12);
}

extern "C" int64_t qpg_percode_select_mixed_ws_bytes(int Q, int K) {
  return (Q <= 0 || K <= 0) ? 0 : (int64_t)((size_t)Q * mix_ws_stride(K));
}
extern "C" int64_t qpg_percode_select_mixed_ws_stride(int K) {
  return K <= 0 ? 0 : (int64_t)mix_ws_stride(K);
}

static int select_mixed_impl(const char* name, qpg_ctx* ctx, void* stream, const void* D, int d_is_f32, int64_t ldD, int Q,
                             const int16_t* cand_code, int64_t C, int K, double absent,
                             int32_t idx_base, double* out_dist, int32_t* out_idx, int16_t* out_rank,
                             int q_block, int64_t block_stride, const float* base, int T, int F,
                             const int32_t* cand_t, int G, int n_taps, int tap_stride,
                             const float* q32, const double* qn2, const double* cn2, double eps1,
                             double eps2, int32_t* stats, void* ws, int64_t ws_bytes, int base_is_f16,
                             const RankCut* cut = nullptr) {
  QPG_REQUIRE(ctx && D && (cand_code || C == 0) && out_dist && out_idx && base && cand_t && q32 && qn2 && cn2 && stats,
              "%s: null pointer", name);
  QPG_REQUIRE(Q >= 0 && C >= 0 && K > 0 && K <= 512 && ldD >= C && C + (int64_t)idx_base < 0x7fffffffll,
              "%s: bad size (K <= 512)", name);
  QPG_REQUIRE(T > 0 && F > 0 && (F % 4) == 0 && G > 0 && n_taps > 0 && tap_stride > 0 && C % G == 0 &&
                  eps1 >= 2.0 * QPG_AUDIO_HL_ERR && eps2 >= 0.0 && eps2 < eps1,
              "%s: bad geometry (F %% 4 == 0) or eps (eps1 >= 2 x the sweep's error bound - at least %g -, 0 <= eps2 < eps1)",
              name, 2.0 * (double)QPG_AUDIO_HL_ERR);
  QPG_REQUIRE(q_block >= 0 && (q_block == 0 || (!out_rank && Q % q_block == 0 && block_stride % 8 == 0)),
              "%s: block layout needs Q %% q_block == 0, an 8-byte multiple stride and no rank output", name);
  if (Q == 0) return QPG_OK;
  GuardArgs A;
  A.base = base; A.half = base_is_f16; A.q32 = q32; A.cand_t = cand_t; A.T = T; A.F = F; A.G = G; A.n_taps = n_taps;
  A.tap_stride = tap_stride; A.eps = eps2; A.stats = stats;
  const int use_qlds = (n_taps == 6 && F == 1024) ? 1 : 0;
  const size_t sh2 = 32 * (size_t)K + 16 * MIX_LIST + 4 * MIX_LIST2 + 32 + 6 * MIX_LIST + 4 * (size_t)K;
  size_t sh2c = sh2;
  const RankCut RCnone = {nullptr, nullptr, 1, 0};
  const size_t sh1 = sh2 + 6 * MIX_POT;
  const size_t sh = sh1 + (use_qlds ? (size_t)n_taps * F * 4 : 0);
  if (!ctx->select_lds_raised) {
    if (hipFuncSetAttribute(reinterpret_cast<const void*>(percode_select_mixed_f64_kernel<double>),
                            hipFuncAttributeMaxDynamicSharedMemorySize, 128 * 1024) != hipSuccess ||
        hipFuncSetAttribute(reinterpret_cast<const void*>(percode_select_mixed_f64_kernel<float>),
                            hipFuncAttributeMaxDynamicSharedMemorySize, 128 * 1024) != hipSuccess) {
      qpg_set_error("%s: cannot raise the dynamic LDS limit", name);
      return QPG_EHIP;
    }
    ctx->select_lds_raised = true;
  }
  unsigned char* w = static_cast<unsigned char*>(ws);
  if (ws)
    QPG_REQUIRE(ws_bytes >= qpg_percode_select_mixed_ws_bytes(Q, K) && (reinterpret_cast<uintptr_t>(ws) % 16) == 0,
                "%s: workspace too small or misaligned (qpg_percode_select_mixed_ws_bytes)", name);
#define SEL_MIX_LAUNCH(DT, SH, PHASE, PRE)                                                                                  \
  hipLaunchKernelGGL((percode_select_mixed_f64_kernel<DT>), dim3(Q), dim3(1024), SH, qpg_stream(stream),               \
                     static_cast<const DT*>(D), ldD, cand_code, C, K, absent, idx_base, out_dist, out_idx, out_rank,   \
                     q_block, block_stride, A, eps1, cn2, qn2, use_qlds, PHASE, w, PRE, RCv)
  RankCut RCv = RCnone;
  if (!ws) {
    if (d_is_f32) SEL_MIX_LAUNCH(float, sh, 0, 0); else SEL_MIX_LAUNCH(double, sh, 0, 0);
    QPG_LAUNCH_CHECK("percode_select_mixed_f64_kernel");
    return QPG_OK;
  }
  if (d_is_f32) {
    const size_t shs = 4 * (size_t)K + 10 * (size_t)MIX_SPOT;
    hipLaunchKernelGGL(mixed_stream_kernel, dim3(Q, MIX_SPLIT), dim3(1024), shs, qpg_stream(stream),
                       static_cast<const float*>(D), ldD, cand_code, C, K, eps1, w);
    QPG_LAUNCH_CHECK("mixed_stream_kernel");
    if (cut && cut->pos_t && out_rank) {
      RCv = *cut;
      sh2c = sh2 + 12 * (size_t)rank_sort_pow2(K) + 8 * (size_t)((K + 7) / 8 * 8) + 17 * 8 + 64 * (8 + 8 + 4) +
             16 * (size_t)K;
    }
    SEL_MIX_LAUNCH(float, sh2c, 1, 1);
  } else {
    SEL_MIX_LAUNCH(double, sh1, 1, 0);
  }
  QPG_LAUNCH_CHECK("percode_select_mixed_f64_kernel (lists)");
  const int rb = Q >= 512 ? 8 : (Q >= 128 ? 16 : 64);
  hipLaunchKernelGGL((select_refine_kernel<4>), dim3(Q, rb), dim3(256), 0, qpg_stream(stream), A, K, cn2, qn2, w, use_qlds);
  QPG_LAUNCH_CHECK("select_refine_kernel");
  if (d_is_f32) SEL_MIX_LAUNCH(float, sh2c, 2, 0); else SEL_MIX_LAUNCH(double, sh2, 2, 0);
  QPG_LAUNCH_CHECK("percode_select_mixed_f64_kernel (merge)");
#undef SEL_MIX_LAUNCH
  return QPG_OK;
}

extern "C" int qpg_percode_select_mixed_f64(qpg_ctx* ctx, void* stream, const void* D, int d_is_f32, int64_t ldD, int Q,
                                            const int16_t* cand_code, int64_t C, int K, double absent,
                                            int32_t idx_base, double* out_dist, int32_t* out_idx, int16_t* out_rank,
                                            int q_block, int64_t block_stride, const float* base, int T, int F,
                                            const int32_t* cand_t, int G, int n_taps, int tap_stride,
                                            const float* q32, const double* qn2, const double* cn2, double eps1,
                                            double eps2, int32_t* stats, void* ws, int64_t ws_bytes, int base_is_f16) {
  return select_mixed_impl("qpg_percode_select_mixed_f64", ctx, stream, D, d_is_f32, ldD, Q, cand_code, C, K, absent, idx_base,
                           out_dist, out_idx, out_rank, q_block, block_stride, base, T, F, cand_t, G, n_taps, tap_stride, q32,
                           qn2, cn2, eps1, eps2, stats, ws, ws_bytes, base_is_f16);
}

extern "C" int qpg_percode_select_mixed_f64_cut(qpg_ctx* ctx, void* stream, const void* D, int d_is_f32, int64_t ldD, int Q,
                                                const int16_t* cand_code, int64_t C, int K, double absent,
                                                int32_t idx_base, double* out_dist, int32_t* out_idx, int16_t* out_rank,
                                                int q_block, int64_t block_stride, const float* base, int T, int F,
                                                const int32_t* cand_t, int G, int n_taps, int tap_stride,
                                                const float* q32, const double* qn2, const double* cn2, double eps1,
                                                double eps2, int32_t* stats, void* ws, int64_t ws_bytes, int base_is_f16,
                                                const int16_t* pos_rank_t, const int16_t* freq_rank, int top_n, int probe) {
  const char* name = "qpg_percode_select_mixed_f64_cut";
  QPG_REQUIRE(pos_rank_t && freq_rank && out_rank && ws && d_is_f32 && q_block == 0 && (top_n == 1 || top_n == 2) &&
                  probe >= 0,
              "%s: needs the rank tables, out_rank, an f32 matrix, a workspace, no block layout, top_n 1 or 2", name);
  RankCut rc = {pos_rank_t, freq_rank, top_n, probe > 0 ? probe : 64};
  return select_mixed_impl(name, ctx, stream, D, d_is_f32, ldD, Q, cand_code, C, K, absent, idx_base, out_dist, out_idx,
                           out_rank, q_block, block_stride, base, T, F, cand_t, G, n_taps, tap_stride, q32, qn2, cn2, eps1, eps2,
                           stats, ws, ws_bytes, base_is_f16, &rc);
}

template <typename T, typename KeyT, bool PACKED>
static int percode_select(const char* name, qpg_ctx* ctx, void* stream, const T* D, int64_t ldD, int Q,
                          const int16_t* cand_code, int64_t C, int K, T absent, int32_t idx_base, T* out_dist,
                          int32_t* out_idx, int16_t* out_rank, int q_block, int64_t block_stride) {
  QPG_REQUIRE(ctx && D && (cand_code || C == 0) && out_dist && out_idx, "%s: null pointer", name);
  QPG_REQUIRE(Q >= 0 && C >= 0 && K > 0 && K <= 2048 && ldD >= C && C + (int64_t)idx_base < 0x7fffffffll,
              "%s: bad size (K <= 2048, candidate indices must stay below 2^31)", name);
  QPG_REQUIRE(q_block >= 0 && (q_block == 0 || (!out_rank && Q % q_block == 0 && block_stride % 8 == 0)),
              "%s: block layout needs Q %% q_block == 0, an 8-byte multiple stride and no rank output", name);
  if (Q == 0) return QPG_OK;
  const size_t sh = 12 * (size_t)rank_sort_pow2(K) + (size_t)K * sizeof(T);
  hipLaunchKernelGGL((percode_select_kernel<T, KeyT, PACKED>), dim3(Q), dim3(1024), sh, qpg_stream(stream), D, ldD,
                     cand_code, C, K, absent, idx_base, out_dist, out_idx, out_rank, q_block, block_stride);
  QPG_LAUNCH_CHECK(name);
  return QPG_OK;
}

extern "C" int qpg_percode_select_f64(qpg_ctx* ctx, void* stream, const double* D, int64_t ldD, int Q,
                                      const int16_t* cand_code, int64_t C, int K, double absent, int32_t idx_base,
                                      double* out_dist, int32_t* out_idx, int16_t* out_rank, int q_block,
                                      int64_t block_stride) {
  return percode_select<double, unsigned long long, false>("qpg_percode_select_f64", ctx, stream, D, ldD, Q, cand_code,
                                                           C, K, absent, idx_base, out_dist, out_idx, out_rank, q_block,
                                                           block_stride);
}
extern "C" int qpg_percode_select_f32(qpg_ctx* ctx, void* stream, const float* D, int64_t ldD, int Q,
                                      const int16_t* cand_code, int64_t C, int K, float absent, int32_t idx_base,
                                      float* out_dist, int32_t* out_idx, int16_t* out_rank, int q_block,
                                      int64_t block_stride) {
  return percode_select<float, unsigned int, true>("qpg_percode_select_f32", ctx, stream, D, ldD, Q, cand_code, C, K,
                                                   absent, idx_base, out_dist, out_idx, out_rank, q_block, block_stride);
}

struct ExactWs {
  double* wmin;
  double* list_d;
  int32_t* widx;
  unsigned int* near_;
  int* list_c;
  int* cnt;
};
__host__ static size_t exact_ws_layout(int Q, int64_t C, int K, unsigned char* b, ExactWs* w) {
  size_t o = 0;
  const size_t QK = (size_t)Q * K, QC = (size_t)Q * (size_t)C;
  if (w) w->wmin = reinterpret_cast<double*>(b + o);
  o += QK * 8;
  if (w) w->list_d = reinterpret_cast<double*>(b + o);
  o += QC * 8;
  if (w) w->widx = reinterpret_cast<int32_t*>(b + o);
  o += QK * 4;
  if (w) w->near_ = reinterpret_cast<unsigned int*>(b + o);
// ... 737 lines not shown
```

qpgesture_amd/csrc/qpg_sorted.hip:

```cpp
#include "qpg_common.h"

__device__ __forceinline__ unsigned int okey32(float d) {
  const unsigned int b = __float_as_uint(d);
  return (b >> 31) ? ~b : (b | 0x80000000u);
}
__device__ __forceinline__ float okey32_value(unsigned int k) {
  return __uint_as_float((k >> 31) ? (k & 0x7fffffffu) : ~k);
}

#define SORT_SPLIT 8
#define SORT_LIST 2048
#define SORT_TILES 1024
#define SORT_THREADS 256

__global__ __launch_bounds__(SORT_THREADS) void percode_select_sorted_kernel(
    const float* __restrict__ Dm, int64_t ldD, const float* __restrict__ tmin, const uint16_t* __restrict__ tmask,
    int64_t ldT, int64_t R, const int16_t* __restrict__ row_code, const int32_t* __restrict__ row_index, const int32_t* __restrict__ zero_row,
    const int32_t* __restrict__ code_tile, int K, float band, const float* __restrict__ qn, const float* __restrict__ xs,
    int Dd, float absent, float* __restrict__ out_dist, int32_t* __restrict__ out_idx, int32_t* __restrict__ stats,
    int32_t idx_base, int q_block, int64_t block_stride) {
  extern __shared__ __attribute__((aligned(16))) unsigned char smem[];
  const int S = gridDim.y, s = blockIdx.y;
  const int k0 = (int)((int64_t)s * K / S), k1 = (int)((int64_t)(s + 1) * K / S), KL = k1 - k0;
  const int KLmax = ((K + S - 1) / S + 4) & ~3;
  unsigned long long* ebest = reinterpret_cast<unsigned long long*>(smem);
  unsigned int* best = reinterpret_cast<unsigned int*>(ebest + KLmax);
  int* list = reinterpret_cast<int*>(best + KLmax);
  int* tl = list + SORT_LIST;
  float* qrow = reinterpret_cast<float*>(tl + SORT_TILES);
  __shared__ int n_list, n_tiles;
  const int q = blockIdx.x, tid = threadIdx.x;
  const float* row = Dm ? Dm + (int64_t)q * ldD : nullptr;
  const float* trow = tmin + (int64_t)q * ldT;
  const uint16_t* mrow = tmask ? tmask + (int64_t)q * ldT : nullptr;
  const int t0 = code_tile[k0], t1 = code_tile[k1];
  for (int k = tid; k < KL; k += blockDim.x) {
    ebest[k] = ~0ull;
    best[k] = (zero_row && zero_row[k0 + k] >= 0) ? okey32(0.5f) : 0xffffffffu;
  }
  for (int i = tid; i < Dd / 4; i += blockDim.x)
    reinterpret_cast<f32x4*>(qrow)[i] = reinterpret_cast<const f32x4*>(qn + (int64_t)q * Dd)[i];
  if (tid == 0) {
    n_list = 0;
    n_tiles = 0;
  }
  __syncthreads();
  for (int t = t0 + tid; t < t1; t += blockDim.x) {
    const int code = (row_code[(int64_t)t * 16] & 0x1fff) - k0;
    if ((unsigned)code < (unsigned)KL) atomicMin(&best[code], okey32(trow[t]));
  }
  __syncthreads();
  if (band >= 0.f) {
    for (int t = t0 + tid; t < t1; t += blockDim.x) {
// ... 29 lines not shown
  }
  __syncthreads();
  int n = n_list;
  if (n > SORT_LIST) {
    n = SORT_LIST;
    if (tid == 0 && stats) atomicOr(&stats[1], 16);
  }
  for (int e = tid; e < n; e += blockDim.x) {
    const int r = list[e];
    const bool z = r >= (int)R;
    const f32x4* xp = reinterpret_cast<const f32x4*>(xs + (int64_t)(z ? (int)R : r) * Dd);
    const f32x4* qp = reinterpret_cast<const f32x4*>(qrow);
    float a0 = 0.f, a1 = 0.f, a2 = 0.f, a3 = 0.f;
    for (int g0 = 0; g0 < Dd / 16; g0 += 4) {
      f32x4 xv[16];
#pragma unroll
      for (int i = 0; i < 16; ++i) xv[i] = (g0 * 4 + i) < Dd / 4 ? xp[g0 * 4 + i] : (f32x4){0.f, 0.f, 0.f, 0.f};
#pragma unroll
      for (int gg = 0; gg < 4; ++gg) {
        if (g0 + gg >= Dd / 16) break;
#pragma unroll
        for (int u = 3; u >= 0; --u) {
          const f32x4 x = xv[gg * 4 + u], qq = qp[(g0 + gg) * 4 + u];
          const float d0 = f_sub(qq.x, x.x), d1 = f_sub(qq.y, x.y), d2 = f_sub(qq.z, x.z), d3 = f_sub(qq.w, x.w);
          a0 = f_add(f_mul(d0, d0), a0);
          a1 = f_add(f_mul(d1, d1), a1);
          a2 = f_add(f_mul(d2, d2), a2);
          a3 = f_add(f_mul(d3, d3), a3);
        }
      }
    }
    const float dist = f_mul(0.5f, f_add(f_add(a0, a1), f_add(a2, a3)));
    const int cd = z ? r - (int)R : (row_code[r] & 0x1fff);
    const int oi = z ? zero_row[cd] : row_index[r];
    atomicMin(&ebest[cd - k0], ((unsigned long long)okey32(dist) << 32) | (unsigned int)oi);
  }
  __syncthreads();
  if (q_block > 0) {
    const int64_t shift = (int64_t)(q / q_block) * block_stride;
    const int64_t rowoff = (int64_t)(q % q_block) * K - (int64_t)q * K;
    out_dist = reinterpret_cast<float*>(reinterpret_cast<unsigned char*>(out_dist) + shift) + rowoff;
    out_idx = reinterpret_cast<int32_t*>(reinterpret_cast<unsigned char*>(out_idx) + shift) + rowoff;
  }
  for (int k = tid; k < KL; k += blockDim.x) {
    const unsigned long long kv = ebest[k];
    const bool have = kv != ~0ull;
    out_dist[(int64_t)q * K + k0 + k] = have ? okey32_value((unsigned int)(kv >> 32)) : absent;
    out_idx[(int64_t)q * K + k0 + k] = have ? (int32_t)(kv & 0xffffffffu) + idx_base : -1;
  }
}

__global__ __launch_bounds__(256) void sorted_finish_kernel(const float* __restrict__ dist, const int32_t* __restrict__ idx,
                                                             int K, int16_t* __restrict__ out_rank,
                                                             int32_t* __restrict__ out_nn) {
  extern __shared__ __attribute__((aligned(16))) unsigned char smem[];
  unsigned long long* skey = reinterpret_cast<unsigned long long*>(smem);
  int* scode = reinterpret_cast<int*>(skey + rank_sort_pow2(K));
  float* v = reinterpret_cast<float*>(scode + rank_sort_pow2(K));
  __shared__ unsigned long long nn_key;
  const int q = blockIdx.x, tid = threadIdx.x, lane = tid & 63;
  if (tid == 0) nn_key = ~0ull;
  unsigned long long mine = ~0ull;
  for (int k = tid; k < K; k += blockDim.x) {
    const float dv = dist[(int64_t)q * K + k];
    const int iv = idx[(int64_t)q * K + k];
    v[k] = dv;
    if (iv >= 0) {
      const unsigned long long kv = ((unsigned long long)okey32(dv) << 32) | (unsigned int)iv;
      if (kv < mine) mine = kv;
    }
  }
  __syncthreads();
  if (out_nn) {
    for (int o = 32; o > 0; o >>= 1) {
      const unsigned long long other = __shfl_xor(mine, o, 64);
      mine = other < mine ? other : mine;
    }
    if (lane == 0 && mine != ~0ull) atomicMin(&nn_key, mine);
    __syncthreads();
    if (tid == 0) out_nn[q] = nn_key != ~0ull ? (int32_t)(nn_key & 0xffffffffu) : -1;
  }
  if (!out_rank) return;
  block_sorted_ranks(v, K, skey, scode, [&](int k, int r) { out_rank[(int64_t)q * K + k] = (int16_t)r; });
}

extern "C" int qpg_percode_select_sorted_f32(qpg_ctx* ctx, void* stream, const float* Dm, int64_t ldD, const float* tile_min,
                                             const uint16_t* tile_mask, int64_t ldT, int Q, int64_t R,
                                             const int16_t* row_code,
                                             const int32_t* row_index, const int32_t* zero_row, const int32_t* code_tile,
                                             int K, float band, const float* qn, const float* xs, int Dd, float absent,
                                             float* out_dist, int32_t* out_idx, int16_t* out_rank, int32_t* out_nn,
                                             int32_t* stats, int32_t idx_base, int q_block, int64_t block_stride) {
  const char* name = "qpg_percode_select_sorted_f32";
  QPG_REQUIRE(ctx && (Dm || tile_mask) && tile_min && row_code && row_index && code_tile && qn && xs && out_dist && out_idx,
              "%s: null pointer", name);
  QPG_REQUIRE(Q >= 0 && R > 0 && (R % 16) == 0 && R < 0x7fffffffll - 0x2000 && (!Dm || ldD >= R) && ldT >= R / 16 && K > 0 &&
                  K <= 2048 && K <= 0x1fff && Dd > 0 && (Dd % 16) == 0 && (reinterpret_cast<uintptr_t>(xs) % 16) == 0 &&
                  (reinterpret_cast<uintptr_t>(qn) % 16) == 0,
              "%s: bad size / alignment (R %% 16 == 0, D %% 16 == 0, K <= 2048)", name);
  QPG_REQUIRE(q_block >= 0 && idx_base >= 0 &&
                  (q_block == 0 || (!out_rank && !out_nn && Q % q_block == 0 && block_stride % 8 == 0)),
              "%s: block layout needs Q %% q_block == 0, an 8-byte multiple stride and no rank / nn output", name);
  if (Q == 0) return QPG_OK;
  const int S = K >= 32 * SORT_SPLIT ? SORT_SPLIT : (K >= 32 ? K / 32 : 1);
  const int KLmax = ((K + S - 1) / S + 4) & ~3;
  const size_t sh = 12 * (size_t)KLmax + 4 * (size_t)SORT_LIST + 4 * (size_t)SORT_TILES + 4 * (size_t)Dd;
  QPG_REQUIRE(sh <= 64 * 1024, "%s: K / D too large for the LDS tables", name);
  hipLaunchKernelGGL(percode_select_sorted_kernel, dim3(Q, S), dim3(SORT_THREADS), sh, qpg_stream(stream), Dm, ldD, tile_min,
                     tile_mask, ldT, R, row_code, row_index, zero_row, code_tile, K, band, qn, xs, Dd, absent, out_dist, out_idx, stats,
                     idx_base, q_block, block_stride);
  QPG_LAUNCH_CHECK("percode_select_sorted_kernel");
  if (out_rank || out_nn) {
    hipLaunchKernelGGL(sorted_finish_kernel, dim3(Q), dim3(256), 12 * (size_t)rank_sort_pow2(K) + 4 * (size_t)K, qpg_stream(stream),
                       (const float*)out_dist, (const int32_t*)out_idx, K, out_rank, out_nn);
    QPG_LAUNCH_CHECK("sorted_finish_kernel");
  }
  return QPG_OK;
}

__global__ __launch_bounds__(256) void perm32_kernel(const float* __restrict__ x, int64_t n32, float* __restrict__ y) {
  for (int64_t i = (int64_t)blockIdx.x * blockDim.x + threadIdx.x; i < n32; i += (int64_t)gridDim.x * blockDim.x) {
    const f32x4* p = reinterpret_cast<const f32x4*>(x) + i * 8;
    f32x4 u[8];
#pragma unroll
    for (int v = 0; v < 8; ++v) u[v] = p[v];
    f32x4* o = reinterpret_cast<f32x4*>(y) + i * 8;
#pragma unroll
    for (int k = 0; k < 4; ++k) {
      o[2 * k] = (f32x4){u[3][k], u[2][k], u[1][k], u[0][k]};
      o[2 * k + 1] = (f32x4){u[7][k], u[6][k], u[5][k], u[4][k]};
    }
  }
}

extern "C" int qpg_perm32_rows_f32(qpg_ctx* ctx, void* stream, const float* x, int64_t R, int D, float* y) {
  QPG_REQUIRE(ctx && x && y && x != y && R >= 0 && D > 0 && (D % 32) == 0 && (reinterpret_cast<uintptr_t>(x) % 16) == 0 &&
                  (reinterpret_cast<uintptr_t>(y) % 16) == 0,
              "qpg_perm32_rows_f32: bad argument (D %% 32 == 0, 16-byte aligned, out of place)");
  const int64_t n32 = R * (D / 32);
  if (n32 == 0) return QPG_OK;
  const int64_t nb = (n32 + 255) / 256;
  hipLaunchKernelGGL(perm32_kernel, dim3((unsigned)(nb < 16384 ? nb : 16384)), dim3(256), 0, qpg_stream(stream), x, n32, y);
  QPG_LAUNCH_CHECK("perm32_kernel");
  return QPG_OK;
}

#define BYC_THREADS 512
#define BYC_QMAX 2048
#define BYC_LIST 1024

template <int PT>
__global__ __launch_bounds__(BYC_THREADS) void percode_select_bycode_kernel(
    const float* __restrict__ tmin_t, const uint16_t* __restrict__ tmask_t, int64_t ldQ, int Q, int64_t R,
    const int16_t* __restrict__ row_code, const int32_t* __restrict__ row_index, const int32_t* __restrict__ zero_row,
    const int32_t* __restrict__ code_tile, int K, float band, const float* __restrict__ qp, const float* __restrict__ xsp,
    int Dd, float absent, float* __restrict__ out_dist, int32_t* __restrict__ out_idx, int32_t* __restrict__ stats,
    int32_t idx_base) {
  extern __shared__ __attribute__((aligned(16))) unsigned char smem[];
  const int rowb = Dd * 4;
  float* rows0 = reinterpret_cast<float*>(smem);
  unsigned long long* ebest = reinterpret_cast<unsigned long long*>(smem + (size_t)17 * rowb);
  float* cmin = reinterpret_cast<float*>(ebest + Q);
  int* list_q = reinterpret_cast<int*>(cmin + Q);
  int* list_r = list_q + BYC_LIST;
  __shared__ int n_list[2];
  const int code = blockIdx.x, tid = threadIdx.x;
  const int t0 = code_tile[code], t1 = code_tile[code + 1], nt = t1 - t0;
  const int zr = zero_row ? zero_row[code] : -1;
  const int nv = Dd / 4;
  for (int q = tid; q < Q; q += BYC_THREADS) {
// ... 100 lines not shown
#pragma unroll
        for (int i = 0; i < 8; ++i) {
          const bool in = g0 + i < G32;
          qq[2 * i] = in ? qv[(g0 + i) * 8] : (f32x4){0.f, 0.f, 0.f, 0.f};
          qq[2 * i + 1] = in ? qv[(g0 + i) * 8 + 1] : (f32x4){0.f, 0.f, 0.f, 0.f};
        }
#pragma unroll
        for (int i = 0; i < 16; ++i) {
          if (g0 + (i >> 1) >= G32) break;
          const f32x4 xv = xp[(g0 + (i >> 1)) * 8 + (i & 1)];
#pragma unroll
          for (int j = 0; j < 4; ++j) {
            const float d = f_sub(qq[i][j], xv[j]);
            a = f_add(f_mul(d, d), a);
          }
        }
      }
      const float s01 = f_add(a, __shfl_xor(a, 1, 64));
      const float s = f_add(s01, __shfl_xor(s01, 2, 64));
      if (on && k4 == 0) {
        const float dist = f_mul(0.5f, s);
        const int oi = r == 16 ? zr : row_index[(int64_t)(t0 + t) * 16 + r];
        atomicMin(&ebest[q], ((unsigned long long)okey32(dist) << 32) | (unsigned int)oi);
      }
    }
    __syncthreads();
    if (t + 1 < nt) commit();
  }
  if (nt == 0 && zr >= 0 && band >= 0.f) {
    for (int q = tid; q < Q; q += BYC_THREADS) {
      const float* qr = qp + (int64_t)q * Dd;
      float a0 = 0.f, a1 = 0.f, a2 = 0.f, a3 = 0.f;
      for (int G = 0; G < G32; ++G)
        for (int j = 0; j < 8; ++j) {
          const float d0 = qr[G * 32 + j], d1 = qr[G * 32 + 8 + j], d2 = qr[G * 32 + 16 + j], d3 = qr[G * 32 + 24 + j];
          a0 = f_add(f_mul(d0, d0), a0);
          a1 = f_add(f_mul(d1, d1), a1);
          a2 = f_add(f_mul(d2, d2), a2);
          a3 = f_add(f_mul(d3, d3), a3);
        }
      const float dist = f_mul(0.5f, f_add(f_add(a0, a1), f_add(a2, a3)));
      ebest[q] = ((unsigned long long)okey32(dist) << 32) | (unsigned int)zr;
    }
    __syncthreads();
  }
  for (int q = tid; q < Q; q += BYC_THREADS) {
    const unsigned long long kv = ebest[q];
    const bool have = kv != ~0ull;
    out_dist[(int64_t)q * K + code] = have ? okey32_value((unsigned int)(kv >> 32)) : absent;
    out_idx[(int64_t)q * K + code] = have ? (int32_t)(kv & 0xffffffffu) + idx_base : -1;
  }
}

extern "C" int qpg_percode_select_bycode_f32(qpg_ctx* ctx, void* stream, const float* tile_min_t, const uint16_t* tile_mask_t,
                                             int64_t ldQ, int Q, int64_t R, const int16_t* row_code,
                                             const int32_t* row_index, const int32_t* zero_row, const int32_t* code_tile,
                                             int K, float band, const float* qn_perm, const float* xs_perm, int Dd,
                                             float absent, float* out_dist, int32_t* out_idx, int16_t* out_rank,
                                             int32_t* out_nn, int32_t* stats, int32_t idx_base) {
  const char* name = "qpg_percode_select_bycode_f32";
  QPG_REQUIRE(ctx && tile_min_t && tile_mask_t && row_code && row_index && code_tile && qn_perm && xs_perm && out_dist && out_idx,
              "%s: null pointer", name);
  QPG_REQUIRE(Q >= 0 && ldQ >= Q && R > 0 && (R % 16) == 0 && R < 0x7fffffffll - 0x2000 && K > 0 && K <= 0x1fff && Dd > 0 &&
                  (Dd % 128) == 0 && Dd <= 1024 && (reinterpret_cast<uintptr_t>(xs_perm) % 16) == 0 &&
                  (reinterpret_cast<uintptr_t>(qn_perm) % 16) == 0 && idx_base >= 0,
              "%s: bad size / alignment (R %% 16 == 0, D %% 128 == 0, D <= 1024)", name);
  if (Q == 0) return QPG_OK;
  static bool raised = false;
  if (!raised) {
    bool ok = true;
#define BYC_RAISE(PT_) ok = ok && hipFuncSetAttribute(reinterpret_cast<const void*>(percode_select_bycode_kernel<PT_>), \
                                                      hipFuncAttributeMaxDynamicSharedMemorySize, 96 * 1024) == hipSuccess
    BYC_RAISE(1); BYC_RAISE(2); BYC_RAISE(3); BYC_RAISE(4); BYC_RAISE(5); BYC_RAISE(6); BYC_RAISE(7); BYC_RAISE(8);
#undef BYC_RAISE
    if (!ok) {
      qpg_set_error("%s: cannot raise the dynamic LDS limit", name);
      return QPG_EHIP;
    }
    raised = true;
  }
  for (int qa = 0; qa < Q; qa += BYC_QMAX) {
    const int qn = Q - qa < BYC_QMAX ? Q - qa : BYC_QMAX;
    const size_t sh = (size_t)17 * Dd * 4 + 12 * (size_t)qn + 8 * (size_t)BYC_LIST;
    QPG_REQUIRE(sh <= 96 * 1024, "%s: LDS tables too large", name);
#define BYC_GO(PT_) hipLaunchKernelGGL(percode_select_bycode_kernel<PT_>, dim3(K), dim3(BYC_THREADS), sh, qpg_stream(stream), \
                                       tile_min_t + qa, tile_mask_t + qa, ldQ, qn, R, row_code, row_index, zero_row, code_tile, K, \
                                       band, qn_perm + (int64_t)qa * Dd, xs_perm, Dd, absent, out_dist + (int64_t)qa * K,           \
                                       out_idx + (int64_t)qa * K, stats, idx_base)
    switch (Dd / 128) {
      case 1: BYC_GO(1); break;
      case 2: BYC_GO(2); break;
      case 3: BYC_GO(3); break;
      case 4: BYC_GO(4); break;
      case 5: BYC_GO(5); break;
      case 6: BYC_GO(6); break;
      case 7: BYC_GO(7); break;
      default: BYC_GO(8); break;
    }
#undef BYC_GO
    QPG_LAUNCH_CHECK("percode_select_bycode_kernel");
  }
  if (out_rank || out_nn) {
    hipLaunchKernelGGL(sorted_finish_kernel, dim3(Q), dim3(256), 12 * (size_t)rank_sort_pow2(K) + 4 * (size_t)K, qpg_stream(stream),
                       (const float*)out_dist, (const int32_t*)out_idx, K, out_rank, out_nn);
    QPG_LAUNCH_CHECK("sorted_finish_kernel");
  }
  return QPG_OK;
}
```

qpgesture_amd/csrc/qpg_tail.hip:

```cpp
#include "qpg_common.h"
#include <type_traits>

__global__ __launch_bounds__(256) void l2_table_kernel(const float* __restrict__ sig, int K, int Dm,
                                                       float* __restrict__ out) {
  const int p = blockIdx.x;
  for (int c = threadIdx.x; c < K; c += blockDim.x) {
    double s = 0.0;
    for (int e = 0; e < Dm; ++e) {
      const float d = f_sub(sig[(int64_t)p * Dm + e], sig[(int64_t)c * Dm + e]);
      s += (double)d * (double)d;
    }
    out[(int64_t)p * K + c] = (c == p) ? __builtin_inff() : (float)sqrt(s);
  }
}

extern "C" int qpg_l2_table_f32(qpg_ctx* ctx, void* stream, const float* sig, int K, int Dm, float* out) {
  QPG_REQUIRE(ctx && sig && out && K > 0 && Dm > 0, "qpg_l2_table_f32: bad argument");
  hipLaunchKernelGGL(l2_table_kernel, dim3(K), dim3(256), 0, qpg_stream(stream), sig, K, Dm, out);
  QPG_LAUNCH_CHECK("l2_table_kernel");
  return QPG_OK;
}

__device__ __forceinline__ float lane4_sum(float v, int l) {
  const float o1 = __shfl_xor(v, 1, 64);
  const float pair = (l & 1) ? f_add(o1, v) : f_add(v, o1);
  const float o2 = __shfl_xor(pair, 2, 64);
  return (l & 2) ? f_add(o2, pair) : f_add(pair, o2);
}

__device__ __forceinline__ float einsum_sq_128(const float* v, int l) {
  float a = 0.f;
#pragma unroll
  for (int g = 0; g < 8; ++g) {
#pragma unroll
    for (int u = 3; u >= 0; --u) {
      const float x = v[g * 16 + u * 4 + l];
      a = f_add(f_mul(x, x), a);
    }
  }
  return lane4_sum(a, l);
}

struct ArgMin {
  double v;
  int i;
};
__device__ __forceinline__ ArgMin amin(ArgMin a, ArgMin b) {
  return (b.v < a.v || (b.v == a.v && b.i < a.i)) ? b : a;
}
__device__ __forceinline__ ArgMin wave_argmin(ArgMin m) {
#pragma unroll
  for (int o = 32; o > 0; o >>= 1) {
    ArgMin t{__shfl_xor(m.v, o, 64), __shfl_xor(m.i, o, 64)};
    m = amin(m, t);
  }
  return m;
}

#define QPG_KMAX_PER_LANE 16

__global__ __launch_bounds__(256) void fuse_best_kernel(const int16_t* __restrict__ rank0,
                                                        const int32_t* __restrict__ idx0,
                                                        const int16_t* __restrict__ rank1,
                                                        const int32_t* __restrict__ idx1,
                                                        const int16_t* __restrict__ pos_rank,
                                                        const int16_t* __restrict__ freq_rank, int Q, int K, int mode,
                                                        int32_t* __restrict__ T0, int32_t* __restrict__ T1) {
  const int lane = threadIdx.x & 63;
  const int64_t task = (int64_t)blockIdx.x * 4 + (threadIdx.x >> 6);
  if (task >= (int64_t)Q * K) return;
  const int q = (int)(task / K), p = (int)(task - (int64_t)q * K);
  if (mode == 0) {
    const int16_t* ra = rank0 + (int64_t)q * K;
    const int16_t* rt = rank1 + (int64_t)q * K;
    ArgMin ma{__builtin_inf(), 0x7fffffff}, mt{__builtin_inf(), 0x7fffffff};
#pragma unroll
    for (int i = 0; i < QPG_KMAX_PER_LANE; ++i) {
      const int c = lane + 64 * i;
      if (c < K) {
        const double pos_score = (double)pos_rank[(int64_t)p * K + c] + (double)freq_rank[c] * 0.05;
        ma = amin(ma, ArgMin{pos_score + (double)ra[c], c});
        mt = amin(mt, ArgMin{pos_score + (double)rt[c], c});
      }
    }
    ma = wave_argmin(ma);
    mt = wave_argmin(mt);
    if (lane == 0) {
      T0[task] = idx0[(int64_t)q * K + ma.i];
      T1[task] = idx1[(int64_t)q * K + mt.i];
    }
    return;
  }
  const int16_t* rk = (mode == 1 ? rank0 : rank1) + (int64_t)q * K;
  const int32_t* ix = (mode == 1 ? idx0 : idx1) + (int64_t)q * K;
  ArgMin m{__builtin_inf(), 0x7fffffff};
  double vals[QPG_KMAX_PER_LANE];
#pragma unroll
  for (int i = 0; i < QPG_KMAX_PER_LANE; ++i) {
    const int c = lane + 64 * i;
    vals[i] = __builtin_inf();
    if (c < K) {
      const double pos_score = (double)pos_rank[(int64_t)p * K + c] + (double)freq_rank[c] * 0.05;
// ... 280 lines not shown
        const int l = lane & 3, grp = lane >> 2;
        const float* v = (grp & 1) ? vb[grp >> 1] : va[grp >> 1];
        float n = f_sqrt(einsum_sq_128_t(v, l));
        if (n < eps10) n = 1.f;
        if (l == 0) nrm[grp] = n;
      }
      __syncthreads();
#pragma unroll
      for (int k = 0; k < 2; ++k) {
        const float na = nrm[2 * k], nb = nrm[2 * k + 1];
        const float2 xa = reinterpret_cast<const float2*>(va[k])[lane], xb = reinterpret_cast<const float2*>(vb[k])[lane];
        float2 d;
        d.x = f_sub(f_div(xa.x, na), f_div(xb.x, nb));
        d.y = f_sub(f_div(xa.y, na), f_div(xb.y, nb));
        reinterpret_cast<float2*>(va[k])[lane] = d;
      }
      __syncthreads();
      if (lane < 8) {
        const int l = lane & 3, k = lane >> 2;
        const float sc = f_mul(0.5f, einsum_sq_128_t(va[k], l));
        if (l == 0) score[k] = sc;
      }
      __syncthreads();
      const int fi = (score[1] < score[0]) ? 1 : 0;
      prev = fi ? cur[1].tail : cur[0].tail;
      reinterpret_cast<float2*>(A.out_phase + ((int64_t)w * A.steps + s) * 128)[lane] = prev;
      const int wpay = fi ? cur[1].pay : cur[0].pay;
      if (lane < A.step_codes) wincodes[s * A.step_codes + lane] = wpay;
      if (lane == 0) A.out_vote[w * A.steps + s] = fi;
      prev_code = __shfl(wpay, A.step_codes - 1, 64);
      if (spec) {
        cur[0] = fi ? nxt[1][0] : nxt[0][0];
        cur[1] = fi ? nxt[1][1] : nxt[0][1];
      }
    }
    __syncthreads();
    if (lane < A.codes_per_window) A.out_codes[(int64_t)w * A.codes_per_window + lane] = wincodes[lane];
    prev_code = wincodes[last_idx];
  }
  __threadfence_system();
  __syncthreads();
  if (lane == 0) {
    A.out_status[0] = bad;
    __threadfence_system();
    A.out_status[1] = A.guard_flags ? A.guard_flags[0] : 0;
  }
}


struct GateGeom {
  int s_last, off_last;
};

__device__ __forceinline__ const float* cand_block(const TailArgs& A, int which, int ci, int* pay_base) {
  const int G = which ? A.G1 : A.G0;
  const int cc = ci < 0 ? 0 : ci;
  const int j = cc / G, g = cc - j * G;
  const int ps = (which ? A.pslot1 : A.pslot0)[g];
  *pay_base = j * A.code_ld + (which ? A.cidx1 : A.cidx0)[g];
  return A.phase + ((int64_t)j * A.Tp + ps) * 16;
}

__device__ __forceinline__ unsigned int gate_eval(const TailArgs& A, int q, int p, const float* prev, int lane) {
  const int K = A.K;
  const int k = (lane >> 2) & 1, l = lane & 3;
  const int ck = (k ? A.T1 : A.T0)[(int64_t)q * K + p];
  int pb_unused;
  const float* head = cand_block(A, k, ck, &pb_unused);
  float xa[32], xb[32];
  float sa = 0.f, sb = 0.f;
#pragma unroll
  for (int g = 0; g < 8; ++g) {
#pragma unroll
    for (int u = 3; u >= 0; --u) {
      const int e = g * 16 + u * 4 + l;
      const float va = e < 80 ? prev[48 + e] : head[e - 80];
      const float vb = e < 48 ? prev[80 + e] : head[e - 48];
      xa[g * 4 + u] = va;
      xb[g * 4 + u] = vb;
      sa = f_add(f_mul(va, va), sa);
      sb = f_add(f_mul(vb, vb), sb);
    }
  }
  const float eps10 = 10.f * 1.1920928955078125e-07f;
  float na = f_sqrt(lane4_sum(sa, l)), nb = f_sqrt(lane4_sum(sb, l));
  if (na < eps10) na = 1.f;
  if (nb < eps10) nb = 1.f;
  float sd = 0.f;
#pragma unroll
  for (int g = 0; g < 8; ++g) {
#pragma unroll
    for (int u = 3; u >= 0; --u) {
      const float d = f_sub(f_div(xa[g * 4 + u], na), f_div(xb[g * 4 + u], nb));
      sd = f_add(f_mul(d, d), sd);
    }
  }
  const float score = f_mul(0.5f, lane4_sum(sd, l));
  const float other = __shfl_xor(score, 4, 64);
  const float s0 = k ? other : score, s1 = k ? score : other;
  const int fi = (s1 < s0) ? 1 : 0;
  return (unsigned int)((p << 1) | fi);
}

__device__ __forceinline__ const float* gate_prev(const TailArgs& A, const GateGeom& geo, int s, int kp, int ci, int* p) {
  int pb;
  const float* prev = cand_block(A, kp, ci, &pb) + 384;
  *p = A.code[pb + (s == 0 ? geo.off_last : A.step_codes - 1)];
  return prev;
}

__global__ __launch_bounds__(256) void gate_table_kernel(TailArgs A, GateGeom geo, uint16_t* __restrict__ Gt) {
  const int K = A.K, Qc = A.M * A.steps, Q = Qc * A.n_chains;
  const int lane = threadIdx.x & 63;
  const int64_t task = ((int64_t)blockIdx.x * 256 + threadIdx.x) >> 3;
  const int64_t n_task = (int64_t)Q * 2 * K;
  const bool live = task < n_task;
  const int q = live ? (int)(task / (2 * K)) : 0;
  const int sigma = live ? (int)(task - (int64_t)q * 2 * K) : 0;
  const int chain = q / Qc;
  const bool first = q == chain * Qc;
  if (first && sigma != 0) return;
  const int s = q % A.steps;
  int p;
  const float* prev;
  if (first) {
    p = A.seed_codes ? A.seed_codes[chain] : A.seed_code;
    prev = A.seed_phase + (int64_t)chain * 128;
  } else {
    const int pp = sigma >> 1, kp = sigma & 1;
    const int ci = (kp ? A.T1 : A.T0)[(int64_t)(q - 1) * K + pp];
    prev = gate_prev(A, geo, s, kp, ci, &p);
  }
  const unsigned int g = gate_eval(A, q, p, prev, lane);
  if (live && (lane & 7) == 0) Gt[task] = (uint16_t)g;
}

#define GD_SLOTS 2048
#define GD_THREADS 1024
__global__ __launch_bounds__(GD_THREADS) void gate_table_dedup_kernel(TailArgs A, GateGeom geo, uint16_t* __restrict__ Gt) {
  __shared__ int key[GD_SLOTS];
  __shared__ unsigned short val[GD_SLOTS];
  __shared__ unsigned short ulist[GD_SLOTS];
  __shared__ int n_u;
  const int K = A.K, Qc = A.M * A.steps, tid = threadIdx.x, lane = tid & 63;
  const int q = blockIdx.x, chain = q / Qc, s = q % A.steps;
  uint16_t* out = Gt + (int64_t)q * 2 * K;
  if (q == chain * Qc) {
    if (tid < 8) {
      const int p = A.seed_codes ? A.seed_codes[chain] : A.seed_code;
      const unsigned int g = gate_eval(A, q, p, A.seed_phase + (int64_t)chain * 128, lane);
      if (tid == 0) out[0] = (uint16_t)g;
    }
    return;
  }
  for (int i = tid; i < GD_SLOTS; i += GD_THREADS) key[i] = 0;
  if (tid == 0) n_u = 0;
  __syncthreads();
  constexpr int PER = 2 * 512 / GD_THREADS;
  int slot[PER];
#pragma unroll
  for (int u = 0; u < PER; ++u) {
    const int sigma = u * GD_THREADS + tid;
    slot[u] = -1;
    if (sigma < 2 * K) {
      const int pp = sigma >> 1, kp = sigma & 1;
      const int ci = (kp ? A.T1 : A.T0)[(int64_t)(q - 1) * K + pp];
      const int kv = (((ci < 0 ? 0 : ci) << 1) | kp) + 1;
      unsigned int h = ((unsigned int)kv * 2654435761u) >> 21;
      for (;;) {
        const int old = atomicCAS(&key[h], 0, kv);
        if (old == 0) {
          ulist[atomicAdd(&n_u, 1)] = (unsigned short)h;
          break;
        }
        if (old == kv) break;
        h = (h + 1) & (GD_SLOTS - 1);
      }
      slot[u] = (int)h;
    }
  }
  __syncthreads();
  const int nu = n_u;
  for (int u = tid >> 3; u < nu; u += GD_THREADS >> 3) {
    const int h = ulist[u], kv = key[h] - 1;
    int p;
    const float* prev = gate_prev(A, geo, s, kv & 1, kv >> 1, &p);
    const unsigned int g = gate_eval(A, q, p, prev, lane);
    if ((lane & 7) == 0) val[h] = (unsigned short)g;
  }
  __syncthreads();
#pragma unroll
  for (int u = 0; u < PER; ++u)
    if (slot[u] >= 0) out[u * GD_THREADS + tid] = val[slot[u]];
}

#define QPG_CHASE_QMAX 2048
__global__ __launch_bounds__(1024) void gate_chase_kernel(TailArgs A, const uint16_t* __restrict__ Gt) {
  extern __shared__ __attribute__((aligned(16))) uint16_t gl[];
  __shared__ uint16_t sig[QPG_CHASE_QMAX];
  __shared__ int bad_s;
  const int K = A.K, Q = A.M * A.steps, tid = threadIdx.x, nt = blockDim.x;
  const int per_w = A.steps * 2 * K;
  const int chain = blockIdx.x;
  const int64_t q0 = (int64_t)chain * Q;
  Gt += q0 * 2 * K;
  A.T0 += q0 * K;
  A.T1 += q0 * K;
  A.out_phase += q0 * 128;
  A.out_vote += q0;
  A.out_codes += (int64_t)chain * A.M * A.codes_per_window;
  A.out_status += (int64_t)chain * A.status_stride;
  if (tid == 0) bad_s = 0;
  int sigma = 0;
  auto stage = [&](int w, int first, int step) {
    const int4* src = reinterpret_cast<const int4*>(Gt + (int64_t)w * per_w);
    int4* dst = reinterpret_cast<int4*>(gl + (size_t)(w & 1) * per_w);
    for (int v = first; v < per_w / 8; v += step) dst[v] = src[v];
  };
  stage(0, tid, nt);
  __syncthreads();
  for (int w = 0; w < A.M; ++w) {
    if (tid >= 64 && w + 1 < A.M) stage(w + 1, tid - 64, nt - 64);
    if (tid == 0) {
      const uint16_t* g = gl + (size_t)(w & 1) * per_w;
      for (int s = 0; s < A.steps; ++s) {
        sigma = (w == 0 && s == 0) ? g[0] : g[s * 2 * K + sigma];
        sig[w * A.steps + s] = (uint16_t)sigma;
      }
    }
    __syncthreads();
  }
  for (int i = tid; i < Q * 32; i += nt) {
    const int q = i >> 5, v = i & 31;
    const int sg = sig[q], p = sg >> 1, fi = sg & 1;
    const int ci = (fi ? A.T1 : A.T0)[(int64_t)q * K + p];
    int pb;
    const float* blk = cand_block(A, fi, ci, &pb) + 384;
    reinterpret_cast<f32x4*>(A.out_phase + (int64_t)q * 128)[v] = reinterpret_cast<const f32x4*>(blk)[v];
    if (v == 0) {
      A.out_vote[q] = fi;
      if (A.T0[(int64_t)q * K + p] < 0 || A.T1[(int64_t)q * K + p] < 0) bad_s = 1;
    }
  }
  for (int i = tid; i < A.M * A.codes_per_window; i += nt) {
    const int w = i / A.codes_per_window, c = i - w * A.codes_per_window;
    const int q = w * A.steps + c / A.step_codes;
    const int sg = sig[q], p = sg >> 1, fi = sg & 1;
    const int ci = (fi ? A.T1 : A.T0)[(int64_t)q * K + p];
    int pb;
    cand_block(A, fi, ci, &pb);
    A.out_codes[i] = A.code[pb + c % A.step_codes];
  }
  __threadfence_system();
  __syncthreads();
  if (tid == 0) {
    A.out_status[0] = bad_s;
    __threadfence_system();
    A.out_status[1] = A.guard_flags ? A.guard_flags[0] : 0;
  }
}

#define QPG_TAKES_PER_BLOCK 64
__host__ __device__ __forceinline__ int64_t takes_trail_off(int n_takes) { return ((int64_t)n_takes + 7) & ~(int64_t)7; }

__global__ __launch_bounds__(256) void takes_step0_kernel(TailArgs A, int n_takes, uint16_t* __restrict__ step0) {
  const int lane = threadIdx.x & 63;
  const int task = (int)(((int64_t)blockIdx.x * 256 + threadIdx.x) >> 3);
  const bool live = task < n_takes;
  const int take = live ? task : n_takes - 1;
  int p = A.seed_codes[take];
  p = p < 0 ? 0 : (p >= A.K ? A.K - 1 : p);
  const unsigned int g = gate_eval(A, 0, p, A.seed_phase + (int64_t)take * 128, lane);
  if (live && (lane & 7) == 0) step0[take] = (uint16_t)g;
}

__global__ __launch_bounds__(1024) void gate_chase_takes_kernel(int M, int steps, int K, int n_takes,
                                                                const uint16_t* __restrict__ Gt,
                                                                const uint16_t* __restrict__ step0,
                                                                uint16_t* __restrict__ trail) {
  extern __shared__ __attribute__((aligned(16))) uint16_t gl[];
  const int tid = threadIdx.x, nt = blockDim.x;
  const int per_w = steps * 2 * K;
  const int take = blockIdx.x * QPG_TAKES_PER_BLOCK + tid;
  const bool chaser = tid < QPG_TAKES_PER_BLOCK && take < n_takes;
  auto stage = [&](int w, int first, int step) {
    const int4* src = reinterpret_cast<const int4*>(Gt + (int64_t)w * per_w);
    int4* dst = reinterpret_cast<int4*>(gl + (size_t)(w & 1) * per_w);
    for (int v = first; v < per_w / 8; v += step) dst[v] = src[v];
  };
  stage(0, tid, nt);
  __syncthreads();
  int sigma = chaser ? step0[take] : 0;
  for (int w = 0; w < M; ++w) {
    if (tid >= 64 && w + 1 < M) stage(w + 1, tid - 64, nt - 64);
    if (chaser) {
      const uint16_t* g = gl + (size_t)(w & 1) * per_w;
      for (int s = 0; s < steps; ++s) {
        if (w | s) sigma = g[s * 2 * K + sigma];
        trail[(int64_t)(w * steps + s) * n_takes + take] = (uint16_t)sigma;
      }
    }
    __syncthreads();
  }
// ... 123 lines not shown
  }
  QPG_LAUNCH_CHECK("fuse_best_kernel");
  TailArgs A;
  A.T0 = T0; A.T1 = T1; A.code = code; A.code_ld = code_ld;
  const bool txt0 = (mode == QPG_MODE_TXT), txt1 = (mode != QPG_MODE_AUD);
  A.cidx0 = txt0 ? txt_cidx : aud_cidx; A.pslot0 = txt0 ? txt_pslot : aud_pslot; A.G0 = txt0 ? Gt : Ga;
  A.cidx1 = txt1 ? txt_cidx : aud_cidx; A.pslot1 = txt1 ? txt_pslot : aud_pslot; A.G1 = txt1 ? Gt : Ga;
  A.phase = phase; A.Tp = Tp; A.M = M; A.steps = steps; A.step_codes = 4;
  A.codes_per_window = (steps * 4 < 30) ? steps * 4 : 30;
  A.K = K; A.seed_code = seed_code; A.seed_phase = seed_phase; A.seed_codes = seed_codes; A.n_chains = n_chains;
  A.status_stride = status_stride;
  A.out_codes = out_codes; A.out_phase = out_phase; A.out_vote = out_vote; A.out_status = out_status;
  A.guard_flags = guard_flags;
  const size_t lds_g = (size_t)2 * steps * 2 * K * sizeof(uint16_t);
  if (!tabulated) {
    QPG_REQUIRE(n_chains == 1, "qpg_match_steps_batch: the sequential walk takes one chain per call");
    hipLaunchKernelGGL(match_walk_kernel, dim3(1), dim3(64), lds, qpg_stream(stream), A);
    QPG_LAUNCH_CHECK("match_walk_kernel");
    return QPG_OK;
  }
  uint16_t* gtab = reinterpret_cast<uint16_t*>(gate_tables + (int64_t)2 * Q * K);
  const int64_t lanes = (int64_t)Q * 2 * K * 8;
  const int dedup_from = ctx->opt[QPG_OPT_GATE_DEDUP_FROM_CHAINS];
  if (dedup_from > 0 && n_chains >= dedup_from && K <= 512) {
    hipLaunchKernelGGL(gate_table_dedup_kernel, dim3((unsigned)Q), dim3(GD_THREADS), 0, qpg_stream(stream), A, geo, gtab);
    QPG_LAUNCH_CHECK("gate_table_dedup_kernel");
  } else {
    hipLaunchKernelGGL(gate_table_kernel, dim3((unsigned)((lanes + 255) / 256)), dim3(256), 0, qpg_stream(stream), A,
                       geo, gtab);
    QPG_LAUNCH_CHECK("gate_table_kernel");
  }
  if (n_takes > 0) {
    uint16_t* step0 = reinterpret_cast<uint16_t*>(takes_ws);
    uint16_t* trail = step0 + takes_trail_off(n_takes);
    const int stages = ctx->opt[QPG_OPT_TAKES_STAGES];
    if (stages & 1) {
      hipLaunchKernelGGL(takes_step0_kernel, dim3((unsigned)(((int64_t)n_takes * 8 + 255) / 256)), dim3(256), 0,
                         qpg_stream(stream), A, n_takes, step0);
      QPG_LAUNCH_CHECK("takes_step0_kernel");
    }
    if (stages & 2) {
      hipLaunchKernelGGL(gate_chase_takes_kernel,
                         dim3((unsigned)((n_takes + QPG_TAKES_PER_BLOCK - 1) / QPG_TAKES_PER_BLOCK)), dim3(1024), lds_g,
                         qpg_stream(stream), M, steps, K, n_takes, (const uint16_t*)gtab, (const uint16_t*)step0, trail);
      QPG_LAUNCH_CHECK("gate_chase_takes_kernel");
    }
    if (stages & 4) {
      hipLaunchKernelGGL(takes_epilogue_kernel, dim3((unsigned)n_takes), dim3(256), 0, qpg_stream(stream), A, n_takes,
                         (const uint16_t*)trail);
      QPG_LAUNCH_CHECK("takes_epilogue_kernel");
    }
    return QPG_OK;
  }
  hipLaunchKernelGGL(gate_chase_kernel, dim3(n_chains), dim3(1024), lds_g, qpg_stream(stream), A, (const uint16_t*)gtab);
  QPG_LAUNCH_CHECK("gate_chase_kernel");
  return QPG_OK;
}

extern "C" int qpg_match_steps(qpg_ctx* ctx, void* stream, const int16_t* aud_rank, const int32_t* aud_idx,
                               const int16_t* txt_rank, const int32_t* txt_idx, const int16_t* pos_rank,
                               const int16_t* freq_rank, const int32_t* code, int code_ld, const int32_t* aud_cidx,
                               const int32_t* aud_pslot, int Ga, const int32_t* txt_cidx, const int32_t* txt_pslot,
                               int Gt, const float* phase, int Tp, int mode, int M, int steps, int K, int seed_code,
                               const float* seed_phase, int32_t* gate_tables, int32_t* out_codes, float* out_phase,
                               int32_t* out_vote, int32_t* out_status, const int32_t* guard_flags) {
  return match_steps_impl(ctx, stream, aud_rank, aud_idx, txt_rank, txt_idx, pos_rank, freq_rank, code, code_ld, aud_cidx,
                          aud_pslot, Ga, txt_cidx, txt_pslot, Gt, phase, Tp, mode, M, steps, K, seed_code, seed_phase,
                          gate_tables, out_codes, out_phase, out_vote, out_status, guard_flags, 1, nullptr, 2);
}

extern "C" int qpg_match_steps_batch(qpg_ctx* ctx, void* stream, const int16_t* aud_rank, const int32_t* aud_idx,
                                     const int16_t* txt_rank, const int32_t* txt_idx, const int16_t* pos_rank,
                                     const int16_t* freq_rank, const int32_t* code, int code_ld, const int32_t* aud_cidx,
                                     const int32_t* aud_pslot, int Ga, const int32_t* txt_cidx, const int32_t* txt_pslot,
                                     int Gt, const float* phase, int Tp, int mode, int M, int steps, int K,
                                     int n_chains, const int32_t* seed_codes, const float* seed_phase,
                                     int32_t* gate_tables, int32_t* out_codes, float* out_phase, int32_t* out_vote,
                                     int32_t* out_status, int64_t status_stride, const int32_t* guard_flags) {
  QPG_REQUIRE(M > 0 && seed_codes, "qpg_match_steps_batch: M > 0 and device seed codes");
  return match_steps_impl(ctx, stream, aud_rank, aud_idx, txt_rank, txt_idx, pos_rank, freq_rank, code, code_ld, aud_cidx,
                          aud_pslot, Ga, txt_cidx, txt_pslot, Gt, phase, Tp, mode, M, steps, K, 0, seed_phase, gate_tables,
                          out_codes, out_phase, out_vote, out_status, guard_flags, n_chains, seed_codes, status_stride);
}

extern "C" size_t qpg_match_steps_takes_ws_bytes(int n_takes, int M, int steps) {
  if (n_takes < 1 || M < 1 || steps < 1) return 0;
  return sizeof(uint16_t) * (size_t)(takes_trail_off(n_takes) + (int64_t)M * steps * n_takes);
}

extern "C" int qpg_match_steps_takes(qpg_ctx* ctx, void* stream, const int16_t* aud_rank, const int32_t* aud_idx,
                                     const int16_t* txt_rank, const int32_t* txt_idx, const int16_t* pos_rank,
                                     const int16_t* freq_rank, const int32_t* code, int code_ld, const int32_t* aud_cidx,
                                     const int32_t* aud_pslot, int Ga, const int32_t* txt_cidx, const int32_t* txt_pslot,
                                     int Gt, const float* phase, int Tp, int mode, int M, int steps, int K,
                                     int n_takes, const int32_t* seed_codes, const float* seed_phase,
                                     int32_t* gate_tables, int32_t* out_codes, float* out_phase, int32_t* out_vote,
                                     int32_t* out_status, int64_t status_stride, const int32_t* guard_flags,
                                     void* workspace, size_t workspace_bytes) {
  QPG_REQUIRE(M > 0 && seed_codes && n_takes >= 1 && n_takes <= QPG_TAKES_MAX && status_stride >= 2,
              "qpg_match_steps_takes: M > 0, 1 <= n_takes <= %d, device seed codes and a status stride >= 2", QPG_TAKES_MAX);
  return match_steps_impl(ctx, stream, aud_rank, aud_idx, txt_rank, txt_idx, pos_rank, freq_rank, code, code_ld, aud_cidx,
                          aud_pslot, Ga, txt_cidx, txt_pslot, Gt, phase, Tp, mode, M, steps, K, 0, seed_phase, gate_tables,
                          out_codes, out_phase, out_vote, out_status, guard_flags, 1, seed_codes, status_stride, n_takes,
                          workspace, workspace_bytes);
}
```

qpgesture_amd/sorted_rows.py:

```python
import torch

from . import _lib

U32 = 2.0 ** -24
HL_GEMM_ERR = _lib.QPG_AUDIO_HL_ERR


def gemm32_err(d):
    n = d / 32
    kappa = 40.0 + 2.0 * max(0.0, n - 16)
    return kappa * U32 + 5.2e-7


def gemm_h_err(d):
    return 2.0 ** -10 + 2.0 ** -22 + (gemm32_err(d) - 5.2e-7) + 1.2e-7 + 1e-9


def prefilter_band_h(d):
    eps1 = ((d / 4 + 2) / 2 + 2) * U32
    e_sk = 0.5 * (8 * eps1 + 4 * (d / 4 + 3) * U32)
    return 2.1 * (gemm_h_err(d) + 2 * eps1 + e_sk)


def prefilter_band(d):
# ... 11 lines not shown
        valid = (cmt >= 0) & (cmt < K)
        zero = xn.double().square().sum(1) < 0.5
        zr = torch.full((K,), 0x7fffffff, dtype=torch.int64, device=dev)
        zi = torch.nonzero(valid & zero).reshape(-1)
        if zi.numel():
            zr.scatter_reduce_(0, cmt[zi], zi, "amin")
        self.zero_row = torch.where(zr == 0x7fffffff, torch.full_like(zr, -1), zr).to(torch.int32).contiguous()
        self.n_zero_rows = int(zi.numel())
        keep = torch.nonzero(valid & ~zero).reshape(-1)
        keep = keep[self._first_of_duplicates(xn, cmt, keep)]
        self.n_rows_kept = int(keep.numel())
        order = keep[torch.sort(cmt[keep], stable=True).indices]
        cd = cmt[order]
        cnt = torch.bincount(cd, minlength=K)
        pad_cnt = (cnt + 15) // 16 * 16
        start = torch.cumsum(pad_cnt, 0) - pad_cnt
        Rs = int(pad_cnt.sum().item())
        R = max((Rs + 63) // 64 * 64, 64)
        first = (torch.cumsum(cnt, 0) - cnt)
        within = torch.arange(order.numel(), device=dev) - first[cd]
        pos = start[cd] + within
        row_index = torch.full((R,), -1, dtype=torch.int32, device=dev)
        row_index[pos] = order.to(torch.int32)
        seg_code = torch.repeat_interleave(torch.arange(K, device=dev), pad_cnt)
        seg_code = torch.cat((seg_code, torch.full((R - Rs,), 0x1fff, device=dev, dtype=seg_code.dtype)))
        self.row_code = torch.where(row_index >= 0, seg_code, seg_code | 0x4000).to(torch.int16).contiguous()
        self.xs = torch.zeros((R + 1, d), dtype=torch.float32, device=dev)
        if order.numel():
            src = order[first.clamp(max=order.numel() - 1)[seg_code[:Rs]]]
            self.xs[:Rs] = xn[src]
            self.xs[pos] = xn[order]
        lib = _lib.load()
        self.image = torch.empty((int(lib.qpg_hl_rows_bytes(R, d)),), dtype=torch.uint8, device=dev)
        _lib.call("qpg_hl_pack_rows", dev, self.xs, R, d, self.image, self.image.numel())
        self.R, self.d, self.K, self.row_index, self.device = R, d, K, row_index, dev
        self.code_tile = torch.cat((torch.zeros((1,), dtype=torch.int64, device=dev),
                                    torch.cumsum(pad_cnt, 0) // 16)).to(torch.int32).contiguous()
        self.band = float(prefilter_band(d))
        self.use_masks = True
        self.by_code = False
        self.by_code_min_q = 256
        self.band_h = float(prefilter_band_h(d))
        self._xs_perm = None

    def xs_perm(self):
        if self._xs_perm is None:
            self._xs_perm = torch.empty_like(self.xs)
            _lib.call("qpg_perm32_rows_f32", self.device, self.xs, self.R + 1, self.d, self._xs_perm)
        return self._xs_perm

    def uses_by_code(self, Q, q_block=0):
        return bool(self.by_code and Q >= self.by_code_min_q and self.d % 128 == 0 and q_block == 0 and self.use_masks)

    def _select_by_code(self, qn, absent, stats, dist, idx, nn, rank, idx_base, sc, cols_packed, raw=None):
        dev = self.device
        Q = (raw if qn is None else qn).shape[0]
        nt, ldq = self.R // 16, (Q + 15) // 16 * 16
        if sc.get("tmin_t") is None or sc["tmin_t"].shape != (nt, ldq):
            sc["tmin_t"] = torch.empty((nt, ldq), dtype=torch.float32, device=dev)
            sc["tmask_t"] = torch.empty((nt, ldq), dtype=torch.int16, device=dev)
        if sc.get("qperm") is None or tuple(sc["qperm"].shape) != (Q, self.d):
            sc["qperm"] = torch.empty((Q, self.d), dtype=torch.float32, device=dev)
        if raw is not None:
            _lib.call("qpg_hl_prepare_queries", dev, raw, Q, self.d, None, sc["cols"], sc["cols"].numel(), sc["qperm"])
        else:
            if not cols_packed:
                _lib.call("qpg_hl_pack_cols", dev, qn, Q, self.d, sc["cols"], sc["cols"].numel())
            _lib.call("qpg_perm32_rows_f32", dev, qn, Q, self.d, sc["qperm"])
        _lib.call("qpg_hl_gemm_tilemin_h", dev, self.image, self.R, self.d, sc["cols"], Q, self.band_h, sc["tmin_t"],
                  sc["tmask_t"], ldq)
        _lib.call("qpg_percode_select_bycode_f32", dev, sc["tmin_t"], sc["tmask_t"], ldq, Q, self.R, self.row_code,
                  self.row_index, self.zero_row, self.code_tile, self.K, self.band_h, sc["qperm"], self.xs_perm(), self.d,
                  absent, dist, idx, rank, nn, stats, int(idx_base))
        return dist, idx, nn

    @staticmethod
    def _first_of_duplicates(xn, codes, keep):
        if keep.numel() == 0:
            return torch.ones((0,), dtype=torch.bool, device=keep.device)
        rows = xn[keep]
        bits = rows.contiguous().view(torch.int32).to(torch.int64)
        g = torch.Generator(device="cpu").manual_seed(0x5eed)
        w = (torch.randint(1, 2 ** 31 - 1, (rows.shape[1],), generator=g, dtype=torch.int64) * 2 + 1).to(rows.device)
        h = (bits * w).sum(1)
        key_order = torch.argsort(h, stable=True)
        key_order = key_order[torch.argsort(codes[keep][key_order], stable=True)]
        ck, hk = codes[keep][key_order], h[key_order]
        new_group = torch.ones_like(ck, dtype=torch.bool)
        new_group[1:] = (ck[1:] != ck[:-1]) | (hk[1:] != hk[:-1])
        first = torch.cummax(torch.where(new_group, torch.arange(ck.numel(), device=ck.device),
                                         torch.zeros_like(ck)), 0).values
        same = (rows[key_order] == rows[key_order[first]]).all(1)
        drop_sorted = same & ~new_group
        mask = torch.ones((keep.numel(),), dtype=torch.bool, device=keep.device)
        mask[key_order[drop_sorted]] = False
        return mask

    def cols_buffer(self, Q, scratch):
        nb = int(_lib.load().qpg_hl_cols_bytes(Q, self.d))
        if scratch.get("cols") is None or scratch["cols"].numel() < nb:
            scratch["cols"] = torch.empty((nb,), dtype=torch.uint8, device=self.device)
        return scratch["cols"]

    def select_raw(self, q, absent, stats, dist=None, idx=None, nn=None, rank=None, idx_base=0, scratch=None):
        dev, Q = self.device, q.shape[0]
        if not self.uses_by_code(Q):
            raise ValueError("select_raw: this batch does not take the by-code path (normalise and call select)")
        sc = scratch if scratch is not None else {}
        nb = int(_lib.load().qpg_hl_cols_bytes(Q, self.d))
        if sc.get("cols") is None or sc["cols"].numel() < nb:
            sc["cols"] = torch.empty((nb,), dtype=torch.uint8, device=dev)
        if dist is None:
            dist = torch.empty((Q, self.K), dtype=torch.float32, device=dev)
            idx = torch.empty((Q, self.K), dtype=torch.int32, device=dev)
        return self._select_by_code(None, absent, stats, dist, idx, nn, rank, idx_base, sc, False, raw=q.contiguous())

    def select(self, qn, absent, stats, dist=None, idx=None, nn=None, rank=None, idx_base=0, q_block=0, block_stride=0,
               scratch=None, cols_packed=False):
        dev, Q = self.device, qn.shape[0]
        lib = _lib.load()
        nb = int(lib.qpg_hl_cols_bytes(Q, self.d))
        sc = scratch if scratch is not None else {}
        if sc.get("cols") is None or sc["cols"].numel() < nb:
            sc["cols"] = torch.empty((nb,), dtype=torch.uint8, device=dev)
        nt = self.R // 16
        if self.uses_by_code(Q, q_block):
            if dist is None:
                dist = torch.empty((Q, self.K), dtype=torch.float32, device=dev)
                idx = torch.empty((Q, self.K), dtype=torch.int32, device=dev)
            return self._select_by_code(qn, absent, stats, dist, idx, nn, rank, idx_base, sc, cols_packed)
        if sc.get("tmin") is None or sc["tmin"].shape[0] < Q or sc["tmin"].shape[1] != nt:
            sc["tmin"] = torch.empty((Q, nt), dtype=torch.float32, device=dev)
            sc["tmask"] = torch.empty((Q, nt), dtype=torch.int16, device=dev)
            sc["Dm"] = None
        cols, tmin, tmask = sc["cols"], sc["tmin"], sc["tmask"]
        if dist is None:
            dist = torch.empty((Q, self.K), dtype=torch.float32, device=dev)
            idx = torch.empty((Q, self.K), dtype=torch.int32, device=dev)
        if not cols_packed:
            _lib.call("qpg_hl_pack_cols", dev, qn, Q, self.d, cols, cols.numel())
        if self.use_masks:
            _lib.call("qpg_hl_gemm_tilemin", dev, self.image, self.R, self.d, cols, Q, self.band, tmin, tmask, nt)
            Dm = None
        else:
            if sc.get("Dm") is None or sc["Dm"].shape[0] < Q:
                sc["Dm"] = torch.empty((Q, self.R), dtype=torch.float32, device=dev)
            Dm = sc["Dm"]
            _lib.call("qpg_hl_gemm_distance", dev, self.image, self.R, self.d, cols, Q, Dm, self.R, tmin, nt)
        _lib.call("qpg_percode_select_sorted_f32", dev, Dm, self.R, tmin, tmask if self.use_masks else None, nt, Q, self.R,
                  self.row_code, self.row_index, self.zero_row, self.code_tile, self.K, self.band, qn, self.xs, self.d,
                  absent, dist, idx, rank, nn, stats, int(idx_base), int(q_block), int(block_stride))
        return dist, idx, nn
```

Before: 6.035 million frames/s.

## Fold rank fusion into select kernels and stage gate-chase tables in one pass

Moves the per-query best-ranked fusion (formerly a separate qpg_fuse_best_ranked launch per modality) into the tail of the mixed audio select and the text sorted/by-code select kernels, computed from the block's LDS rank ordering. This removes two extra kernel launches and the re-read of rank/index arrays. The gate-chase kernel can also load all windows' gate tables into LDS at once, raising the dynamic LDS limit if needed, instead of double-buffering window by window. The costs are more LDS and register pressure in the select kernels and a larger LDS footprint for the chase kernel, which may lower occupancy.

After: 5.928 million frames/s, median of 2. No clear change (-1.8%).

```diff
diff --git a/include/qpg.h b/include/qpg.h
--- a/include/qpg.h
+++ b/include/qpg.h
@@ -22,6 +22,7 @@
 int qpg_ctx_destroy(qpg_ctx* ctx);
 #define QPG_OPT_GATE_DEDUP_FROM_CHAINS 0
 #define QPG_OPT_TAKES_STAGES 1
+#define QPG_OPT_CHASE_ONE_PASS 2
 #define QPG_OPT_COUNT 4
 int qpg_ctx_set_option(qpg_ctx* ctx, int option, int value);
 int qpg_ctx_get_option(qpg_ctx* ctx, int option, int* value);
@@ -128,6 +129,20 @@
                                   const float* xs, int D, float absent, float* out_dist, int32_t* out_idx,
                                   int16_t* out_rank, int32_t* out_nn, int32_t* stats, int32_t idx_base, int q_block,
                                   int64_t block_stride);
+int qpg_percode_select_sorted_fused_f32(qpg_ctx*, void* stream, const float* Dm, int64_t ldD, const float* tile_min,
+                                        const uint16_t* tile_mask, int64_t ldT, int Q, int64_t R,
+                                        const int16_t* row_code, const int32_t* row_index, const int32_t* zero_row,
+                                        const int32_t* code_tile, int K, float band, const float* qn, const float* xs,
+                                        int D, float absent, float* out_dist, int32_t* out_idx, int16_t* out_rank,
+                                        int32_t* out_nn, int32_t* stats, int32_t idx_base, const int16_t* pos_rank_t,
+                                        const int16_t* freq_rank, int32_t* fuse_T);
+int qpg_percode_select_bycode_fused_f32(qpg_ctx*, void* stream, const float* tile_min_t, const uint16_t* tile_mask_t,
+                                        int64_t ldQ, int Q, int64_t R, const int16_t* row_code, const int32_t* row_index,
+                                        const int32_t* zero_row, const int32_t* code_tile, int K, float band,
+                                        const float* qn_perm, const float* xs_perm, int D, float absent, float* out_dist,
+                                        int32_t* out_idx, int16_t* out_rank, int32_t* out_nn, int32_t* stats,
+                                        int32_t idx_base, const int16_t* pos_rank_t, const int16_t* freq_rank,
+                                        int32_t* fuse_T);
 
 int qpg_wavvq_lev_f32(qpg_ctx*, void* stream, const int32_t* sym_db, int N, int T, const int32_t* cand_t, int G,
                       const int32_t* tap_off, int n_taps, const int32_t* sym_q, int Mq, int Tq,
@@ -168,6 +183,13 @@
                                      int tap_stride, const float* q32, const double* qn2, const double* cn2, double eps1,
                                      double eps2, int32_t* stats, void* ws, int64_t ws_bytes, int base_is_f16,
                                      const int16_t* pos_rank_t, const int16_t* freq_rank, int top_n, int probe);
+int qpg_percode_select_mixed_f64_fused(qpg_ctx*, void* stream, const void* D, int d_is_f32, int64_t ldD, int Q,
+                                       const int16_t* cand_code, int64_t C, int K, double absent, int32_t idx_base,
+                                       double* out_dist, int32_t* out_idx, int16_t* out_rank, const float* base, int T,
+                                       int F, const int32_t* cand_t, int G, int n_taps, int tap_stride, const float* q32,
+                                       const double* qn2, const double* cn2, double eps1, double eps2, int32_t* stats,
+                                       void* ws, int64_t ws_bytes, int base_is_f16, const int16_t* pos_rank_t,
+                                       const int16_t* freq_rank, int top_n, int probe, int32_t* fuse_T);
 
 int64_t qpg_merge_mixed_ws_bytes(int Q, int K, int fl_cap);
 int qpg_merge_mixed_phase1_f64(qpg_ctx*, void* stream, const void* recv, int W, int64_t src_stride, int64_t dist_off,
diff --git a/qpgesture_amd/code_knn.py b/qpgesture_amd/code_knn.py
--- a/qpgesture_amd/code_knn.py
+++ b/qpgesture_amd/code_knn.py
@@ -283,9 +283,9 @@
 
 Knobs = namedtuple("Knobs", "audio_precision audio_kernel text_kernel tie_eps mixed_single_launch sharded_mixed "
                    "sharded_mixed_min_gflop force_sharded overlap_sweeps text_after_sweep audio_first fused_pack rank_cut "
-                   "split_fuse split_fuse_max_steps host_ranks use_wavvq",
+                   "split_fuse split_fuse_max_steps host_ranks use_wavvq fold_fuse",
                    defaults=("mixed", "hl", "mfma", 1e-12, False, True, 20.0, False, True, True, None, True, True, True,
-                             256, False, False))
+                             256, False, False, True))
 DBFacts = namedtuple("DBFacts", "n_local N world K Ga F Dt feature_dtype hl_bound_ok has_hl_image has_txt_sorted hl_planes",
                      defaults=("f32", True, True, True, 2))
 
@@ -298,7 +298,7 @@
     fused_rank: bool
 
 
-class StepPlan(NamedTuple):
+class _StepPlanTuple(NamedTuple):
     audio: Optional[AudioPlan]
     text: Optional[str]
     sharded: bool
@@ -307,6 +307,14 @@
     split_fuse: bool
     overlap: bool
     order: Optional[str]
+
+
+class StepPlan(_StepPlanTuple):
+
+    def __new__(cls, *members, fold_fuse=False):
+        self = super().__new__(cls, *members)
+        self.fold_fuse = bool(fold_fuse)
+        return self
 
 
 def plan_audio(kn, db, Q, want_rank=False, reduce=True, out_given=False, cut_top_n=0):
@@ -356,7 +364,9 @@
     if overlap:
         order = "audio_first" if audio_first else ("text_after_sweep" if after else "text_first")
     exchange = ("all_to_all" if owner_blocks else "all_gather") if sharded else None
-    return StepPlan(audio, text, sharded, exchange, clip_pack, split, overlap, order)
+    fold = bool(split and kn.fold_fuse and audio is not None and audio.path == "mixed" and audio.kernel in ("hl", "hl1") and
+                text == "mfma" and db.K <= 512)
+    return StepPlan(audio, text, sharded, exchange, clip_pack, split, overlap, order, fold_fuse=fold)
 
 
 class TakesPlan(NamedTuple):
@@ -424,6 +434,7 @@
         self.mixed_single_launch = False
         self.split_fuse = True
         self.split_fuse_max_steps = 256
+        self.fold_fuse = True
         self.sharded_mixed = True
         self.force_sharded = False
         self.sharded_mixed_min_gflop = 20.0
@@ -443,7 +454,7 @@
         return Knobs(self.audio_precision, self.audio_kernel, self.text_kernel, self.tie_eps, self.mixed_single_launch,
                      self.sharded_mixed, self.sharded_mixed_min_gflop, self.force_sharded, self.overlap_sweeps,
                      self.text_after_sweep, self.audio_first, self.fused_pack, self.rank_cut, self.split_fuse,
-                     self.split_fuse_max_steps, self.host_ranks, self.use_wavvq)
+                     self.split_fuse_max_steps, self.host_ranks, self.use_wavvq, self.fold_fuse)
 
     def _facts(self):
         db = self.db
@@ -517,8 +528,10 @@
         return self._finish(r.dist, r.idx, r.rank, want_rank, reduce)
 
     def _sweep_audio(self, plan, qbase, q_win, q_t, tap_stride=None, out=None, prepacked=None, sweep_event=None,
-                     after_sweep=None):
+                     after_sweep=None, fuse_T=None):
         db, dev = self.db, self.db.device
+        if fuse_T is not None and plan.path != "mixed":
+            raise ValueError("the folded rank fusion is the mixed select's")
         Q = int(q_win.shape[0]) if isinstance(q_win, torch.Tensor) else len(q_win)
         qbase = qbase.contiguous()
         M, T, F = qbase.shape
@@ -572,7 +585,11 @@
             sel_args = (D, 1, D.stride(0), *tables, *track, qn2, db.cn2, plan.band, float(self.tie_eps),
                         self._guard_stats, None if single else ws, 0 if single else ws.numel(), int(half))
             try:
-                if plan.cut_top_n:
+                if fuse_T is not None:
+                    fused_args = sel_args[:12] + sel_args[14:]
+                    _lib.call("qpg_percode_select_mixed_f64_fused", dev, *fused_args, db.pos_rank_t, db.freq_rank,
+                              int(plan.cut_top_n), int(self.rank_cut_probe), fuse_T)
+                elif plan.cut_top_n:
                     _lib.call("qpg_percode_select_mixed_f64_cut", dev, *sel_args, db.pos_rank_t, db.freq_rank,
                               int(plan.cut_top_n), int(self.rank_cut_probe))
                 else:
@@ -594,7 +611,8 @@
             self._last_mix_Q = Q
         return AudioResult(dist, idx, rank, D, q32, qn2, plan)
 
-    def sweep_text(self, queries, want_rank=False, reduce=True, normalised=False, out=None, cols_packed=False, kind=None):
+    def sweep_text(self, queries, want_rank=False, reduce=True, normalised=False, out=None, cols_packed=False, kind=None,
+                   fuse_T=None):
         db, dev = self.db, self.db.device
         Q = queries.shape[0]
         if normalised:
@@ -605,11 +623,14 @@
         if kind is None:
             kind = plan_text(self._knobs(), self._facts(), Q, reduce, out is not None)
         self._last_text_mfma = kind == "mfma"
+        if fuse_T is not None and not (kind == "mfma" and want_rank and out is None):
+            raise ValueError("the folded rank fusion is the text prefilter's select with ranks")
         if kind == "mfma":
             dist, idx, rank, qb, bs = self._tables_out(Q, torch.float32, out, want_rank and out is None)
             db.txt_sorted.select(qn, float(ABSENT_DIST), self._guard_stats, dist=dist, idx=idx, rank=rank,
                                  idx_base=db.idx_base * db.Gt, q_block=qb, block_stride=bs, scratch=self._txt_scratch,
-                                 cols_packed=cols_packed)
+                                 cols_packed=cols_packed,
+                                 fuse=None if fuse_T is None else (db.pos_rank_t, db.freq_rank, fuse_T))
         else:
             D = torch.empty((Q, max(db.Ct, 1)), dtype=torch.float32, device=dev)
             _lib.call("qpg_text_cosine_f32", dev, db.ctxt, db.Ct, db.Dt, qn, Q, D, D.stride(0))
@@ -783,9 +804,11 @@
             self._side_gate.record(torch.cuda.current_stream(dev))
             side.wait_event(self._side_gate)
 
+        fold = plan.fold_fuse
+
         def keep(p_, g, r):
             T[p_ + "_d"], T[p_ + "_idx"], T[p_ + "_rank"] = r[0], r[1], (None if sharded else r[2])
-            if gtab is not None:
+            if gtab is not None and not fold:
                 _lib.call("qpg_fuse_best_ranked", dev, r[2], r[1], db.pos_rank, db.freq_rank, Q, db.K, gtab[g])
 
         def text_pack():
@@ -801,7 +824,7 @@
                 qn = text_pack()
             keep("txt", 1, self.sweep_text(qn, want_rank=not sharded, reduce=not sharded, normalised=True,
                                            out=lay.views("txt") if sharded else None, cols_packed=packed is not None,
-                                           kind=plan.text))
+                                           kind=plan.text, fuse_T=gtab[1] if fold else None))
 
         if plan.order == "text_first":
             with torch.cuda.stream(side):
@@ -814,7 +837,7 @@
             else:
                 aud = self._sweep_audio(plan.audio, test_interp, q_win, q_t, out=out, prepacked=packed,
                                         sweep_event=self._sweep_event if plan.order == "text_after_sweep" else None,
-                                        after_sweep=after_sweep)
+                                        after_sweep=after_sweep, fuse_T=gtab[0] if fold else None)
                 r = self._finish(aud.dist, aud.idx, aud.rank, not sharded, not sharded)
             keep("aud", 0, r)
         if plan.order == "text_after_sweep":
diff --git a/qpgesture_amd/csrc/qpg_common.h b/qpgesture_amd/csrc/qpg_common.h
--- a/qpgesture_amd/csrc/qpg_common.h
+++ b/qpgesture_amd/csrc/qpg_common.h
@@ -11,6 +11,7 @@
   int n_cu;
   float* zeros;
   bool select_lds_raised;
+  int64_t chase_lds_max;
   int opt[QPG_OPT_COUNT];
 };
 
diff --git a/qpgesture_amd/csrc/qpg_core.hip b/qpgesture_amd/csrc/qpg_core.hip
--- a/qpgesture_amd/csrc/qpg_core.hip
+++ b/qpgesture_amd/csrc/qpg_core.hip
@@ -49,9 +49,11 @@
   c->n_cu = p.multiProcessorCount;
   c->zeros = nullptr;
   c->select_lds_raised = false;
+  c->chase_lds_max = 0;
   for (int i = 0; i < QPG_OPT_COUNT; ++i) c->opt[i] = 0;
   c->opt[QPG_OPT_GATE_DEDUP_FROM_CHAINS] = 1;
   c->opt[QPG_OPT_TAKES_STAGES] = 7;
+  c->opt[QPG_OPT_CHASE_ONE_PASS] = 1;
   int prev = 0;
   (void)hipGetDevice(&prev);
   const bool ok = hipSetDevice(device) == hipSuccess && hipMalloc(reinterpret_cast<void**>(&c->zeros), 4096) == hipSuccess &&
diff --git a/qpgesture_amd/csrc/qpg_fuse.h b/qpgesture_amd/csrc/qpg_fuse.h
--- /dev/null
+++ b/qpgesture_amd/csrc/qpg_fuse.h
@@ -0,0 +1,57 @@
+#pragma once
+#include "qpg_common.h"
+
+struct ArgMin {
+  double v;
+  int i;
+};
+__device__ __forceinline__ ArgMin amin(ArgMin a, ArgMin b) {
+  return (b.v < a.v || (b.v == a.v && b.i < a.i)) ? b : a;
+}
+
+template <int PP, int B>
+__device__ __forceinline__ void block_fuse_best_ranked(const int* code_at_rank, const int32_t* row_idx,
+                                                       const int16_t* __restrict__ pos_rank_t,
+                                                       const int16_t* __restrict__ freq_rank, int K,
+                                                       int32_t* __restrict__ T_row) {
+  const int tid = threadIdx.x, nt = blockDim.x;
+  if ((tid & ~63) >= K) return;
+  int pc[PP];
+  bool live[PP];
+  ArgMin m[PP];
+#pragma unroll
+  for (int u = 0; u < PP; ++u) {
+    const int p = tid + u * nt;
+    live[u] = p < K;
+    pc[u] = live[u] ? p : 0;
+    m[u] = ArgMin{__builtin_inf(), 0x7fffffff};
+  }
+  for (int base = 0; base < K; base += B) {
+    bool open = false;
+#pragma unroll
+    for (int u = 0; u < PP; ++u) open = open || (live[u] && !((double)base > m[u].v));
+    if (!__any(open)) break;
+    int c[B];
+    int fv[B], pv[PP][B];
+#pragma unroll
+    for (int j = 0; j < B; ++j) {
+      const int r = base + j < K ? base + j : K - 1;
+      const int cr = __builtin_amdgcn_readfirstlane(code_at_rank[r]);
+      c[j] = cr < 0 ? 0 : (cr < K ? cr : K - 1);
+      fv[j] = freq_rank[c[j]];
+#pragma unroll
+      for (int u = 0; u < PP; ++u) pv[u][j] = pos_rank_t[c[j] * K + pc[u]];
+    }
+#pragma unroll
+    for (int j = 0; j < B; ++j) {
+      if (base + j < K) {
+#pragma unroll
+        for (int u = 0; u < PP; ++u)
+          m[u] = amin(m[u], ArgMin{((double)pv[u][j] + (double)fv[j] * 0.05) + (double)(base + j), c[j]});
+      }
+    }
+  }
+#pragma unroll
+  for (int u = 0; u < PP; ++u)
+    if (live[u]) T_row[pc[u]] = row_idx[m[u].i];
+}
diff --git a/qpgesture_amd/csrc/qpg_select.hip b/qpgesture_amd/csrc/qpg_select.hip
--- a/qpgesture_amd/csrc/qpg_select.hip
+++ b/qpgesture_amd/csrc/qpg_select.hip
@@ -1,4 +1,5 @@
 #include "qpg_common.h"
+#include "qpg_fuse.h"
 
 __device__ __forceinline__ unsigned long long order_key(double d) {
   unsigned long long b = (unsigned long long)__double_as_longlong(d);
@@ -155,6 +156,12 @@
   double eps;
   int32_t* stats;
 };
+struct FuseOut {
+  const int16_t* pos_t;
+  const int16_t* freq;
+  int32_t* T;
+};
+
 struct RankCut {
   const int16_t* pos_t;
   const int16_t* freq;
@@ -654,7 +661,8 @@
     const DT* __restrict__ D, int64_t ldD, const int16_t* __restrict__ cand_code, int64_t C, int K, double absent,
     int32_t idx_base, double* __restrict__ out_dist, int32_t* __restrict__ out_idx, int16_t* __restrict__ out_rank,
     int q_block, int64_t block_stride, GuardArgs A, double eps1, const double* __restrict__ cn2,
-    const double* __restrict__ qn2, int use_qlds, int phase, unsigned char* __restrict__ ws, int pre, RankCut RC) {
+    const double* __restrict__ qn2, int use_qlds, int phase, unsigned char* __restrict__ ws, int pre, RankCut RC,
+    FuseOut FO) {
   extern __shared__ __attribute__((aligned(16))) unsigned char smem[];
   unsigned long long* best = reinterpret_cast<unsigned long long*>(smem);
   double* v = reinterpret_cast<double*>(smem + 8 * (size_t)K);
@@ -700,6 +708,12 @@
       s_code[r] = k;
     });
   };
+  auto fuse_row = [&]() {
+    if (!FO.T) return;
+    __syncthreads();
+    block_fuse_best_ranked<1, 16>(s_code, reinterpret_cast<const int32_t*>(besti), FO.pos_t, FO.freq, K,
+                                  FO.T + (int64_t)q * K);
+  };
   int n = 0;
   bool order_parked = false;
   if (phase != 2) {
@@ -1210,7 +1224,10 @@
   }
   if (!repaired) rank_pass(true);
   SEL_STAMP(9);
-  if (A.eps <= 0.0) return;
+  if (A.eps <= 0.0) {
+    fuse_row();
+    return;
+  }
   __syncthreads();
   for (int r = tid; r + 1 < K; r += blockDim.x) {
     const int ka = s_code[r], kb = s_code[r + 1];
@@ -1233,7 +1250,10 @@
   __syncthreads();
   int n3 = ctl[2];
   SEL_STAMP(10);
-  if (n3 == 0) return;
+  if (n3 == 0) {
+    fuse_row();
+    return;
+  }
   if (n3 > MIX_LIST2) {
     n3 = MIX_LIST2;
     if (tid == 0) atomicOr(&A.stats[1], 1);
@@ -1252,6 +1272,7 @@
   SEL_STAMP(11);
   rank_pass(true);
   SEL_STAMP(12);
+  fuse_row();
 }
 
 extern "C" int64_t qpg_percode_select_mixed_ws_bytes(int Q, int K) {
@@ -1268,7 +1289,7 @@
                              const int32_t* cand_t, int G, int n_taps, int tap_stride,
                              const float* q32, const double* qn2, const double* cn2, double eps1,
                              double eps2, int32_t* stats, void* ws, int64_t ws_bytes, int base_is_f16,
-                             const RankCut* cut = nullptr) {
+                             const RankCut* cut = nullptr, const FuseOut* fuse = nullptr) {
   QPG_REQUIRE(ctx && D && (cand_code || C == 0) && out_dist && out_idx && base && cand_t && q32 && qn2 && cn2 && stats,
               "%s: null pointer", name);
   QPG_REQUIRE(Q >= 0 && C >= 0 && K > 0 && K <= 512 && ldD >= C && C + (int64_t)idx_base < 0x7fffffffll,
@@ -1306,8 +1327,11 @@
 #define SEL_MIX_LAUNCH(DT, SH, PHASE, PRE)                                                                                  \
   hipLaunchKernelGGL((percode_select_mixed_f64_kernel<DT>), dim3(Q), dim3(1024), SH, qpg_stream(stream),               \
                      static_cast<const DT*>(D), ldD, cand_code, C, K, absent, idx_base, out_dist, out_idx, out_rank,   \
-                     q_block, block_stride, A, eps1, cn2, qn2, use_qlds, PHASE, w, PRE, RCv)
+                     q_block, block_stride, A, eps1, cn2, qn2, use_qlds, PHASE, w, PRE, RCv,                       \
+                     (PHASE) == 1 ? FOnone : FOv)
   RankCut RCv = RCnone;
+  const FuseOut FOnone = {nullptr, nullptr, nullptr};
+  const FuseOut FOv = fuse ? *fuse : FOnone;
   if (!ws) {
     if (d_is_f32) SEL_MIX_LAUNCH(float, sh, 0, 0); else SEL_MIX_LAUNCH(double, sh, 0, 0);
     QPG_LAUNCH_CHECK("percode_select_mixed_f64_kernel");
@@ -1365,6 +1389,25 @@
   return select_mixed_impl(name, ctx, stream, D, d_is_f32, ldD, Q, cand_code, C, K, absent, idx_base, out_dist, out_idx,
                            out_rank, q_block, block_stride, base, T, F, cand_t, G, n_taps, tap_stride, q32, qn2, cn2, eps1, eps2,
                            stats, ws, ws_bytes, base_is_f16, &rc);
+}
+
+extern "C" int qpg_percode_select_mixed_f64_fused(qpg_ctx* ctx, void* stream, const void* D, int d_is_f32, int64_t ldD, int Q,
+                                                  const int16_t* cand_code, int64_t C, int K, double absent,
+                                                  int32_t idx_base, double* out_dist, int32_t* out_idx, int16_t* out_rank,
+                                                  const float* base, int T, int F, const int32_t* cand_t, int G, int n_taps,
+                                                  int tap_stride, const float* q32, const double* qn2, const double* cn2,
+                                                  double eps1, double eps2, int32_t* stats, void* ws, int64_t ws_bytes,
+                                                  int base_is_f16, const int16_t* pos_rank_t, const int16_t* freq_rank,
+                                                  int top_n, int probe, int32_t* fuse_T) {
+  const char* name = "qpg_percode_select_mixed_f64_fused";
+  QPG_REQUIRE(pos_rank_t && freq_rank && out_rank && fuse_T && top_n >= 0 && top_n <= 2 && probe >= 0 &&
+                  (top_n == 0 || (ws && d_is_f32)),
+              "%s: needs the rank tables, out_rank, fuse_T, top_n 0 .. 2 (the cut: an f32 matrix and a workspace)", name);
+  const RankCut rc = {pos_rank_t, freq_rank, top_n, probe > 0 ? probe : 64};
+  const FuseOut fo = {pos_rank_t, freq_rank, fuse_T};
+  return select_mixed_impl(name, ctx, stream, D, d_is_f32, ldD, Q, cand_code, C, K, absent, idx_base, out_dist, out_idx,
+                           out_rank, 0, 0, base, T, F, cand_t, G, n_taps, tap_stride, q32, qn2, cn2, eps1, eps2, stats, ws,
+                           ws_bytes, base_is_f16, top_n ? &rc : nullptr, &fo);
 }
 
 template <typename T, typename KeyT, bool PACKED>
diff --git a/qpgesture_amd/csrc/qpg_sorted.hip b/qpgesture_amd/csrc/qpg_sorted.hip
--- a/qpgesture_amd/csrc/qpg_sorted.hip
+++ b/qpgesture_amd/csrc/qpg_sorted.hip
@@ -1,4 +1,5 @@
 #include "qpg_common.h"
+#include "qpg_fuse.h"
 
 __device__ __forceinline__ unsigned int okey32(float d) {
   const unsigned int b = __float_as_uint(d);
@@ -134,11 +135,16 @@
 
 __global__ __launch_bounds__(256) void sorted_finish_kernel(const float* __restrict__ dist, const int32_t* __restrict__ idx,
                                                              int K, int16_t* __restrict__ out_rank,
-                                                             int32_t* __restrict__ out_nn) {
+                                                             int32_t* __restrict__ out_nn,
+                                                             const int16_t* __restrict__ pos_rank_t,
+                                                             const int16_t* __restrict__ freq_rank,
+                                                             int32_t* __restrict__ fuse_T) {
   extern __shared__ __attribute__((aligned(16))) unsigned char smem[];
   unsigned long long* skey = reinterpret_cast<unsigned long long*>(smem);
   int* scode = reinterpret_cast<int*>(skey + rank_sort_pow2(K));
   float* v = reinterpret_cast<float*>(scode + rank_sort_pow2(K));
+  int* by_rank = reinterpret_cast<int*>(v + K);
+  int* s_idx = by_rank + K;
   __shared__ unsigned long long nn_key;
   const int q = blockIdx.x, tid = threadIdx.x, lane = tid & 63;
   if (tid == 0) nn_key = ~0ull;
@@ -147,6 +153,7 @@
     const float dv = dist[(int64_t)q * K + k];
     const int iv = idx[(int64_t)q * K + k];
     v[k] = dv;
+    if (fuse_T) s_idx[k] = iv;
     if (iv >= 0) {
       const unsigned long long kv = ((unsigned long long)okey32(dv) << 32) | (unsigned int)iv;
       if (kv < mine) mine = kv;
@@ -163,17 +170,22 @@
     if (tid == 0) out_nn[q] = nn_key != ~0ull ? (int32_t)(nn_key & 0xffffffffu) : -1;
   }
   if (!out_rank) return;
-  block_sorted_ranks(v, K, skey, scode, [&](int k, int r) { out_rank[(int64_t)q * K + k] = (int16_t)r; });
-}
-
-extern "C" int qpg_percode_select_sorted_f32(qpg_ctx* ctx, void* stream, const float* Dm, int64_t ldD, const float* tile_min,
-                                             const uint16_t* tile_mask, int64_t ldT, int Q, int64_t R,
-                                             const int16_t* row_code,
-                                             const int32_t* row_index, const int32_t* zero_row, const int32_t* code_tile,
-                                             int K, float band, const float* qn, const float* xs, int Dd, float absent,
-                                             float* out_dist, int32_t* out_idx, int16_t* out_rank, int32_t* out_nn,
-                                             int32_t* stats, int32_t idx_base, int q_block, int64_t block_stride) {
-  const char* name = "qpg_percode_select_sorted_f32";
+  block_sorted_ranks(v, K, skey, scode, [&](int k, int r) {
+    out_rank[(int64_t)q * K + k] = (int16_t)r;
+    if (fuse_T) by_rank[r] = k;
+  });
+  if (!fuse_T) return;
+  __syncthreads();
+  block_fuse_best_ranked<2, 8>(by_rank, s_idx, pos_rank_t, freq_rank, K, fuse_T + (int64_t)q * K);
+}
+
+static int select_sorted_impl(const char* name, qpg_ctx* ctx, void* stream, const float* Dm, int64_t ldD,
+                              const float* tile_min, const uint16_t* tile_mask, int64_t ldT, int Q, int64_t R,
+                              const int16_t* row_code, const int32_t* row_index, const int32_t* zero_row,
+                              const int32_t* code_tile, int K, float band, const float* qn, const float* xs, int Dd,
+                              float absent, float* out_dist, int32_t* out_idx, int16_t* out_rank, int32_t* out_nn,
+                              int32_t* stats, int32_t idx_base, int q_block, int64_t block_stride,
+                              const int16_t* pos_rank_t, const int16_t* freq_rank, int32_t* fuse_T) {
   QPG_REQUIRE(ctx && (Dm || tile_mask) && tile_min && row_code && row_index && code_tile && qn && xs && out_dist && out_idx,
               "%s: null pointer", name);
   QPG_REQUIRE(Q >= 0 && R > 0 && (R % 16) == 0 && R < 0x7fffffffll - 0x2000 && (!Dm || ldD >= R) && ldT >= R / 16 && K > 0 &&
@@ -193,11 +205,40 @@
                      idx_base, q_block, block_stride);
   QPG_LAUNCH_CHECK("percode_select_sorted_kernel");
   if (out_rank || out_nn) {
-    hipLaunchKernelGGL(sorted_finish_kernel, dim3(Q), dim3(256), 12 * (size_t)rank_sort_pow2(K) + 4 * (size_t)K, qpg_stream(stream),
-                       (const float*)out_dist, (const int32_t*)out_idx, K, out_rank, out_nn);
+    hipLaunchKernelGGL(sorted_finish_kernel, dim3(Q), dim3(256),
+                       12 * (size_t)rank_sort_pow2(K) + 4 * (size_t)K + (fuse_T ? 8 * (size_t)K : 0), qpg_stream(stream),
+                       (const float*)out_dist, (const int32_t*)out_idx, K, out_rank, out_nn, pos_rank_t, freq_rank, fuse_T);
     QPG_LAUNCH_CHECK("sorted_finish_kernel");
   }
   return QPG_OK;
+}
+
+extern "C" int qpg_percode_select_sorted_f32(qpg_ctx* ctx, void* stream, const float* Dm, int64_t ldD, const float* tile_min,
+                                             const uint16_t* tile_mask, int64_t ldT, int Q, int64_t R,
+                                             const int16_t* row_code,
+                                             const int32_t* row_index, const int32_t* zero_row, const int32_t* code_tile,
+                                             int K, float band, const float* qn, const float* xs, int Dd, float absent,
+                                             float* out_dist, int32_t* out_idx, int16_t* out_rank, int32_t* out_nn,
+                                             int32_t* stats, int32_t idx_base, int q_block, int64_t block_stride) {
+  return select_sorted_impl("qpg_percode_select_sorted_f32", ctx, stream, Dm, ldD, tile_min, tile_mask, ldT, Q, R, row_code,
+                            row_index, zero_row, code_tile, K, band, qn, xs, Dd, absent, out_dist, out_idx, out_rank, out_nn,
+                            stats, idx_base, q_block, block_stride, nullptr, nullptr, nullptr);
+}
+
+extern "C" int qpg_percode_select_sorted_fused_f32(qpg_ctx* ctx, void* stream, const float* Dm, int64_t ldD,
+                                                   const float* tile_min, const uint16_t* tile_mask, int64_t ldT, int Q,
+                                                   int64_t R, const int16_t* row_code, const int32_t* row_index,
+                                                   const int32_t* zero_row, const int32_t* code_tile, int K, float band,
+                                                   const float* qn, const float* xs, int Dd, float absent,
+                                                   float* out_dist, int32_t* out_idx, int16_t* out_rank, int32_t* out_nn,
+                                                   int32_t* stats, int32_t idx_base, const int16_t* pos_rank_t,
+                                                   const int16_t* freq_rank, int32_t* fuse_T) {
+  const char* name = "qpg_percode_select_sorted_fused_f32";
+  QPG_REQUIRE(out_rank && pos_rank_t && freq_rank && fuse_T && K > 0 && K <= 512,
+              "%s: needs out_rank, the rank tables, fuse_T and K <= 512", name);
+  return select_sorted_impl(name, ctx, stream, Dm, ldD, tile_min, tile_mask, ldT, Q, R, row_code, row_index, zero_row,
+                            code_tile, K, band, qn, xs, Dd, absent, out_dist, out_idx, out_rank, out_nn, stats, idx_base, 0, 0,
+                            pos_rank_t, freq_rank, fuse_T);
 }
 
 __global__ __launch_bounds__(256) void perm32_kernel(const float* __restrict__ x, int64_t n32, float* __restrict__ y) {
@@ -404,13 +445,12 @@
   }
 }
 
-extern "C" int qpg_percode_select_bycode_f32(qpg_ctx* ctx, void* stream, const float* tile_min_t, const uint16_t* tile_mask_t,
-                                             int64_t ldQ, int Q, int64_t R, const int16_t* row_code,
-                                             const int32_t* row_index, const int32_t* zero_row, const int32_t* code_tile,
-                                             int K, float band, const float* qn_perm, const float* xs_perm, int Dd,
-                                             float absent, float* out_dist, int32_t* out_idx, int16_t* out_rank,
-                                             int32_t* out_nn, int32_t* stats, int32_t idx_base) {
-  const char* name = "qpg_percode_select_bycode_f32";
+static int select_bycode_impl(const char* name, qpg_ctx* ctx, void* stream, const float* tile_min_t,
+                              const uint16_t* tile_mask_t, int64_t ldQ, int Q, int64_t R, const int16_t* row_code,
+                              const int32_t* row_index, const int32_t* zero_row, const int32_t* code_tile, int K, float band,
+                              const float* qn_perm, const float* xs_perm, int Dd, float absent, float* out_dist,
+                              int32_t* out_idx, int16_t* out_rank, int32_t* out_nn, int32_t* stats, int32_t idx_base,
+                              const int16_t* pos_rank_t, const int16_t* freq_rank, int32_t* fuse_T) {
   QPG_REQUIRE(ctx && tile_min_t && tile_mask_t && row_code && row_index && code_tile && qn_perm && xs_perm && out_dist && out_idx,
               "%s: null pointer", name);
   QPG_REQUIRE(Q >= 0 && ldQ >= Q && R > 0 && (R % 16) == 0 && R < 0x7fffffffll - 0x2000 && K > 0 && K <= 0x1fff && Dd > 0 &&
@@ -453,9 +493,37 @@
     QPG_LAUNCH_CHECK("percode_select_bycode_kernel");
   }
   if (out_rank || out_nn) {
-    hipLaunchKernelGGL(sorted_finish_kernel, dim3(Q), dim3(256), 12 * (size_t)rank_sort_pow2(K) + 4 * (size_t)K, qpg_stream(stream),
-                       (const float*)out_dist, (const int32_t*)out_idx, K, out_rank, out_nn);
+    hipLaunchKernelGGL(sorted_finish_kernel, dim3(Q), dim3(256),
+                       12 * (size_t)rank_sort_pow2(K) + 4 * (size_t)K + (fuse_T ? 8 * (size_t)K : 0), qpg_stream(stream),
+                       (const float*)out_dist, (const int32_t*)out_idx, K, out_rank, out_nn, pos_rank_t, freq_rank, fuse_T);
     QPG_LAUNCH_CHECK("sorted_finish_kernel");
   }
   return QPG_OK;
 }
+
+extern "C" int qpg_percode_select_bycode_f32(qpg_ctx* ctx, void* stream, const float* tile_min_t, const uint16_t* tile_mask_t,
+                                             int64_t ldQ, int Q, int64_t R, const int16_t* row_code,
+                                             const int32_t* row_index, const int32_t* zero_row, const int32_t* code_tile,
+                                             int K, float band, const float* qn_perm, const float* xs_perm, int Dd,
+                                             float absent, float* out_dist, int32_t* out_idx, int16_t* out_rank,
+                                             int32_t* out_nn, int32_t* stats, int32_t idx_base) {
+  return select_bycode_impl("qpg_percode_select_bycode_f32", ctx, stream, tile_min_t, tile_mask_t, ldQ, Q, R, row_code,
+                            row_index, zero_row, code_tile, K, band, qn_perm, xs_perm, Dd, absent, out_dist, out_idx, out_rank,
+                            out_nn, stats, idx_base, nullptr, nullptr, nullptr);
+}
+
+extern "C" int qpg_percode_select_bycode_fused_f32(qpg_ctx* ctx, void* stream, const float* tile_min_t,
+                                                   const uint16_t* tile_mask_t, int64_t ldQ, int Q, int64_t R,
+                                                   const int16_t* row_code, const int32_t* row_index,
+                                                   const int32_t* zero_row, const int32_t* code_tile, int K, float band,
+                                                   const float* qn_perm, const float* xs_perm, int Dd, float absent,
+                                                   float* out_dist, int32_t* out_idx, int16_t* out_rank, int32_t* out_nn,
+                                                   int32_t* stats, int32_t idx_base, const int16_t* pos_rank_t,
+                                                   const int16_t* freq_rank, int32_t* fuse_T) {
+  const char* name = "qpg_percode_select_bycode_fused_f32";
+  QPG_REQUIRE(out_rank && pos_rank_t && freq_rank && fuse_T && K > 0 && K <= 512,
+              "%s: needs out_rank, the rank tables, fuse_T and K <= 512", name);
+  return select_bycode_impl(name, ctx, stream, tile_min_t, tile_mask_t, ldQ, Q, R, row_code, row_index, zero_row, code_tile,
+                            K, band, qn_perm, xs_perm, Dd, absent, out_dist, out_idx, out_rank, out_nn, stats, idx_base,
+                            pos_rank_t, freq_rank, fuse_T);
+}
diff --git a/qpgesture_amd/csrc/qpg_tail.hip b/qpgesture_amd/csrc/qpg_tail.hip
--- a/qpgesture_amd/csrc/qpg_tail.hip
+++ b/qpgesture_amd/csrc/qpg_tail.hip
@@ -1,4 +1,5 @@
 #include "qpg_common.h"
+#include "qpg_fuse.h"
 #include <type_traits>
 
 __global__ __launch_bounds__(256) void l2_table_kernel(const float* __restrict__ sig, int K, int Dm,
@@ -41,13 +42,6 @@
   return lane4_sum(a, l);
 }
 
-struct ArgMin {
-  double v;
-  int i;
-};
-__device__ __forceinline__ ArgMin amin(ArgMin a, ArgMin b) {
-  return (b.v < a.v || (b.v == a.v && b.i < a.i)) ? b : a;
-}
 __device__ __forceinline__ ArgMin wave_argmin(ArgMin m) {
 #pragma unroll
   for (int o = 32; o > 0; o >>= 1) {
@@ -434,21 +428,36 @@
   int s_last, off_last;
 };
 
-__device__ __forceinline__ const float* cand_block(const TailArgs& A, int which, int ci, int* pay_base) {
+#define QPG_GRID_LDS 256
+__device__ __forceinline__ void grid_tables_to_lds(const TailArgs& A, int* lt) {
+  const int g = threadIdx.x;
+  if (g < A.G0) {
+    lt[g] = A.cidx0[g];
+    lt[128 + g] = A.pslot0[g];
+  }
+  if (g < A.G1) {
+    lt[64 + g] = A.cidx1[g];
+    lt[192 + g] = A.pslot1[g];
+  }
+}
+
+__device__ __forceinline__ const float* cand_block(const TailArgs& A, int which, int ci, int* pay_base,
+                                                   const int* lt = nullptr) {
   const int G = which ? A.G1 : A.G0;
   const int cc = ci < 0 ? 0 : ci;
   const int j = cc / G, g = cc - j * G;
-  const int ps = (which ? A.pslot1 : A.pslot0)[g];
-  *pay_base = j * A.code_ld + (which ? A.cidx1 : A.cidx0)[g];
+  const int ps = lt ? lt[128 + which * 64 + g] : (which ? A.pslot1 : A.pslot0)[g];
+  *pay_base = j * A.code_ld + (lt ? lt[which * 64 + g] : (which ? A.cidx1 : A.cidx0)[g]);
   return A.phase + ((int64_t)j * A.Tp + ps) * 16;
 }
 
-__device__ __forceinline__ unsigned int gate_eval(const TailArgs& A, int q, int p, const float* prev, int lane) {
+__device__ __forceinline__ unsigned int gate_eval(const TailArgs& A, int q, int p, const float* prev, int lane,
+                                                  const int* lt = nullptr) {
   const int K = A.K;
   const int k = (lane >> 2) & 1, l = lane & 3;
   const int ck = (k ? A.T1 : A.T0)[(int64_t)q * K + p];
   int pb_unused;
-  const float* head = cand_block(A, k, ck, &pb_unused);
+  const float* head = cand_block(A, k, ck, &pb_unused, lt);
   float xa[32], xb[32];
   float sa = 0.f, sb = 0.f;
 #pragma unroll
@@ -484,9 +493,10 @@
   return (unsigned int)((p << 1) | fi);
 }
 
-__device__ __forceinline__ const float* gate_prev(const TailArgs& A, const GateGeom& geo, int s, int kp, int ci, int* p) {
+__device__ __forceinline__ const float* gate_prev(const TailArgs& A, const GateGeom& geo, int s, int kp, int ci, int* p,
+                                                  const int* lt = nullptr) {
   int pb;
-  const float* prev = cand_block(A, kp, ci, &pb) + 384;
+  const float* prev = cand_block(A, kp, ci, &pb, lt) + 384;
   *p = A.code[pb + (s == 0 ? geo.off_last : A.step_codes - 1)];
   return prev;
 }
@@ -524,13 +534,16 @@
   __shared__ unsigned short val[GD_SLOTS];
   __shared__ unsigned short ulist[GD_SLOTS];
   __shared__ int n_u;
+  __shared__ int lt[QPG_GRID_LDS];
   const int K = A.K, Qc = A.M * A.steps, tid = threadIdx.x, lane = tid & 63;
   const int q = blockIdx.x, chain = q / Qc, s = q % A.steps;
   uint16_t* out = Gt + (int64_t)q * 2 * K;
+  grid_tables_to_lds(A, lt);
   if (q == chain * Qc) {
+    __syncthreads();
     if (tid < 8) {
       const int p = A.seed_codes ? A.seed_codes[chain] : A.seed_code;
-      const unsigned int g = gate_eval(A, q, p, A.seed_phase + (int64_t)chain * 128, lane);
+      const unsigned int g = gate_eval(A, q, p, A.seed_phase + (int64_t)chain * 128, lane, lt);
       if (tid == 0) out[0] = (uint16_t)g;
     }
     return;
@@ -566,8 +579,8 @@
   for (int u = tid >> 3; u < nu; u += GD_THREADS >> 3) {
     const int h = ulist[u], kv = key[h] - 1;
     int p;
-    const float* prev = gate_prev(A, geo, s, kv & 1, kv >> 1, &p);
-    const unsigned int g = gate_eval(A, q, p, prev, lane);
+    const float* prev = gate_prev(A, geo, s, kv & 1, kv >> 1, &p, lt);
+    const unsigned int g = gate_eval(A, q, p, prev, lane, lt);
     if ((lane & 7) == 0) val[h] = (unsigned short)g;
   }
   __syncthreads();
@@ -577,10 +590,11 @@
 }
 
 #define QPG_CHASE_QMAX 2048
-__global__ __launch_bounds__(1024) void gate_chase_kernel(TailArgs A, const uint16_t* __restrict__ Gt) {
+__global__ __launch_bounds__(1024) void gate_chase_kernel(TailArgs A, const uint16_t* __restrict__ Gt, int one_pass) {
   extern __shared__ __attribute__((aligned(16))) uint16_t gl[];
   __shared__ uint16_t sig[QPG_CHASE_QMAX];
   __shared__ int bad_s;
+  __shared__ int lt[QPG_GRID_LDS];
   const int K = A.K, Q = A.M * A.steps, tid = threadIdx.x, nt = blockDim.x;
   const int per_w = A.steps * 2 * K;
   const int chain = blockIdx.x;
@@ -593,31 +607,58 @@
   A.out_codes += (int64_t)chain * A.M * A.codes_per_window;
   A.out_status += (int64_t)chain * A.status_stride;
   if (tid == 0) bad_s = 0;
+  grid_tables_to_lds(A, lt);
   int sigma = 0;
-  auto stage = [&](int w, int first, int step) {
-    const int4* src = reinterpret_cast<const int4*>(Gt + (int64_t)w * per_w);
-    int4* dst = reinterpret_cast<int4*>(gl + (size_t)(w & 1) * per_w);
-    for (int v = first; v < per_w / 8; v += step) dst[v] = src[v];
-  };
-  stage(0, tid, nt);
-  __syncthreads();
-  for (int w = 0; w < A.M; ++w) {
-    if (tid >= 64 && w + 1 < A.M) stage(w + 1, tid - 64, nt - 64);
+  if (one_pass) {
+    const int n16 = A.M * (per_w / 8);
+    const int4* src = reinterpret_cast<const int4*>(Gt);
+    int4* dst = reinterpret_cast<int4*>(gl);
+    auto piece = [&](int v) { return src[v < n16 ? v : n16 - 1]; };
+    auto put = [&](int v, const int4& x) {
+      if (v < n16) dst[v] = x;
+    };
+    for (int v0 = tid; v0 < n16; v0 += 8 * nt) {
+      const int4 r0 = piece(v0), r1 = piece(v0 + nt), r2 = piece(v0 + 2 * nt), r3 = piece(v0 + 3 * nt);
+      const int4 r4 = piece(v0 + 4 * nt), r5 = piece(v0 + 5 * nt), r6 = piece(v0 + 6 * nt), r7 = piece(v0 + 7 * nt);
+      put(v0, r0); put(v0 + nt, r1); put(v0 + 2 * nt, r2); put(v0 + 3 * nt, r3);
+      put(v0 + 4 * nt, r4); put(v0 + 5 * nt, r5); put(v0 + 6 * nt, r6); put(v0 + 7 * nt, r7);
+    }
+    __syncthreads();
     if (tid == 0) {
-      const uint16_t* g = gl + (size_t)(w & 1) * per_w;
-      for (int s = 0; s < A.steps; ++s) {
-        sigma = (w == 0 && s == 0) ? g[0] : g[s * 2 * K + sigma];
-        sig[w * A.steps + s] = (uint16_t)sigma;
+      sigma = gl[0];
+      sig[0] = (uint16_t)sigma;
+      for (int q = 1; q < Q; ++q) {
+        sigma = gl[(size_t)q * 2 * K + sigma];
+        sig[q] = (uint16_t)sigma;
       }
     }
     __syncthreads();
+  } else {
+    auto stage = [&](int w, int first, int step) {
+      const int4* src = reinterpret_cast<const int4*>(Gt + (int64_t)w * per_w);
+      int4* dst = reinterpret_cast<int4*>(gl + (size_t)(w & 1) * per_w);
+      for (int v = first; v < per_w / 8; v += step) dst[v] = src[v];
+    };
+    stage(0, tid, nt);
+    __syncthreads();
+    for (int w = 0; w < A.M; ++w) {
+      if (tid >= 64 && w + 1 < A.M) stage(w + 1, tid - 64, nt - 64);
+      if (tid == 0) {
+        const uint16_t* g = gl + (size_t)(w & 1) * per_w;
+        for (int s = 0; s < A.steps; ++s) {
+          sigma = (w == 0 && s == 0) ? g[0] : g[s * 2 * K + sigma];
+          sig[w * A.steps + s] = (uint16_t)sigma;
+        }
+      }
+      __syncthreads();
+    }
   }
   for (int i = tid; i < Q * 32; i += nt) {
     const int q = i >> 5, v = i & 31;
     const int sg = sig[q], p = sg >> 1, fi = sg & 1;
     const int ci = (fi ? A.T1 : A.T0)[(int64_t)q * K + p];
     int pb;
-    const float* blk = cand_block(A, fi, ci, &pb) + 384;
+    const float* blk = cand_block(A, fi, ci, &pb, lt) + 384;
     reinterpret_cast<f32x4*>(A.out_phase + (int64_t)q * 128)[v] = reinterpret_cast<const f32x4*>(blk)[v];
     if (v == 0) {
       A.out_vote[q] = fi;
@@ -630,7 +671,7 @@
     const int sg = sig[q], p = sg >> 1, fi = sg & 1;
     const int ci = (fi ? A.T1 : A.T0)[(int64_t)q * K + p];
     int pb;
-    cand_block(A, fi, ci, &pb);
+    cand_block(A, fi, ci, &pb, lt);
     A.out_codes[i] = A.code[pb + c % A.step_codes];
   }
   __threadfence_system();
@@ -860,7 +901,25 @@
     }
     return QPG_OK;
   }
-  hipLaunchKernelGGL(gate_chase_kernel, dim3(n_chains), dim3(1024), lds_g, qpg_stream(stream), A, (const uint16_t*)gtab);
+  if (ctx->chase_lds_max == 0) {
+    int dev_lds = 0;
+    hipFuncAttributes fa;
+    if (hipDeviceGetAttribute(&dev_lds, hipDeviceAttributeMaxSharedMemoryPerBlock, ctx->device) != hipSuccess ||
+        hipFuncGetAttributes(&fa, reinterpret_cast<const void*>(gate_chase_kernel)) != hipSuccess) {
+      qpg_set_error("qpg_match_steps: cannot read the workgroup's LDS limit");
+      return QPG_EHIP;
+    }
+    int64_t room = (int64_t)dev_lds - (int64_t)fa.sharedSizeBytes;
+    if (room > 64 * 1024 &&
+        hipFuncSetAttribute(reinterpret_cast<const void*>(gate_chase_kernel), hipFuncAttributeMaxDynamicSharedMemorySize,
+                            (int)room) != hipSuccess)
+      room = 64 * 1024;
+    ctx->chase_lds_max = room > 0 ? room : -1;
+  }
+  const size_t lds_all = (size_t)M * steps * 2 * K * sizeof(uint16_t);
+  const bool one_pass = ctx->opt[QPG_OPT_CHASE_ONE_PASS] != 0 && (int64_t)lds_all <= ctx->chase_lds_max;
+  hipLaunchKernelGGL(gate_chase_kernel, dim3(n_chains), dim3(1024), one_pass ? lds_all : lds_g, qpg_stream(stream), A,
+                     (const uint16_t*)gtab, one_pass ? 1 : 0);
   QPG_LAUNCH_CHECK("gate_chase_kernel");
   return QPG_OK;
 }
diff --git a/qpgesture_amd/sorted_rows.py b/qpgesture_amd/sorted_rows.py
--- a/qpgesture_amd/sorted_rows.py
+++ b/qpgesture_amd/sorted_rows.py
@@ -87,7 +87,7 @@
     def uses_by_code(self, Q, q_block=0):
         return bool(self.by_code and Q >= self.by_code_min_q and self.d % 128 == 0 and q_block == 0 and self.use_masks)
 
-    def _select_by_code(self, qn, absent, stats, dist, idx, nn, rank, idx_base, sc, cols_packed, raw=None):
+    def _select_by_code(self, qn, absent, stats, dist, idx, nn, rank, idx_base, sc, cols_packed, raw=None, fuse=None):
         dev = self.device
         Q = (raw if qn is None else qn).shape[0]
         nt, ldq = self.R // 16, (Q + 15) // 16 * 16
@@ -104,9 +104,10 @@
             _lib.call("qpg_perm32_rows_f32", dev, qn, Q, self.d, sc["qperm"])
         _lib.call("qpg_hl_gemm_tilemin_h", dev, self.image, self.R, self.d, sc["cols"], Q, self.band_h, sc["tmin_t"],
                   sc["tmask_t"], ldq)
-        _lib.call("qpg_percode_select_bycode_f32", dev, sc["tmin_t"], sc["tmask_t"], ldq, Q, self.R, self.row_code,
-                  self.row_index, self.zero_row, self.code_tile, self.K, self.band_h, sc["qperm"], self.xs_perm(), self.d,
-                  absent, dist, idx, rank, nn, stats, int(idx_base))
+        _lib.call("qpg_percode_select_bycode_fused_f32" if fuse else "qpg_percode_select_bycode_f32", dev, sc["tmin_t"],
+                  sc["tmask_t"], ldq, Q, self.R, self.row_code, self.row_index, self.zero_row, self.code_tile, self.K,
+                  self.band_h, sc["qperm"], self.xs_perm(), self.d, absent, dist, idx, rank, nn, stats, int(idx_base),
+                  *(fuse or ()))
         return dist, idx, nn
 
     @staticmethod
@@ -151,7 +152,7 @@
         return self._select_by_code(None, absent, stats, dist, idx, nn, rank, idx_base, sc, False, raw=q.contiguous())
 
     def select(self, qn, absent, stats, dist=None, idx=None, nn=None, rank=None, idx_base=0, q_block=0, block_stride=0,
-               scratch=None, cols_packed=False):
+               scratch=None, cols_packed=False, fuse=None):
         dev, Q = self.device, qn.shape[0]
         lib = _lib.load()
         nb = int(lib.qpg_hl_cols_bytes(Q, self.d))
@@ -163,7 +164,7 @@
             if dist is None:
                 dist = torch.empty((Q, self.K), dtype=torch.float32, device=dev)
                 idx = torch.empty((Q, self.K), dtype=torch.int32, device=dev)
-            return self._select_by_code(qn, absent, stats, dist, idx, nn, rank, idx_base, sc, cols_packed)
+            return self._select_by_code(qn, absent, stats, dist, idx, nn, rank, idx_base, sc, cols_packed, fuse=fuse)
         if sc.get("tmin") is None or sc["tmin"].shape[0] < Q or sc["tmin"].shape[1] != nt:
             sc["tmin"] = torch.empty((Q, nt), dtype=torch.float32, device=dev)
             sc["tmask"] = torch.empty((Q, nt), dtype=torch.int16, device=dev)
@@ -182,6 +183,13 @@
                 sc["Dm"] = torch.empty((Q, self.R), dtype=torch.float32, device=dev)
             Dm = sc["Dm"]
             _lib.call("qpg_hl_gemm_distance", dev, self.image, self.R, self.d, cols, Q, Dm, self.R, tmin, nt)
+        if fuse:
+            if q_block:
+                raise ValueError("select: the folded rank fusion takes no exchange layout")
+            _lib.call("qpg_percode_select_sorted_fused_f32", dev, Dm, self.R, tmin, tmask if self.use_masks else None, nt,
+                      Q, self.R, self.row_code, self.row_index, self.zero_row, self.code_tile, self.K, self.band, qn,
+                      self.xs, self.d, absent, dist, idx, rank, nn, stats, int(idx_base), *fuse)
+            return dist, idx, nn
         _lib.call("qpg_percode_select_sorted_f32", dev, Dm, self.R, tmin, tmask if self.use_masks else None, nt, Q, self.R,
                   self.row_code, self.row_index, self.zero_row, self.code_tile, self.K, self.band, qn, self.xs, self.d,
                   absent, dist, idx, rank, nn, stats, int(idx_base), int(q_block), int(block_stride))
```
